# kngwyu/rogue-gym

Measured on AMD Instinct MI355X. Metric: env-steps/sec (whole node) at 65 536 envs, 32x16 mini-dungeon, higher is better.
Workload: dtype u8/u16 integer state, f32 observation; 1 GPU; config-mini.json 32x16, 65536 envs per GPU (65536 total), gray-image obs [N,1,16,32] f32, max_steps 1000, auto-reset; envs_per_gpu=65536, parallelism=env-sharded x1, no data-path collective

## Files before the change

### rogue-gym_amd/csrc/rg_api.cpp

```cpp
#include <hip/hip_runtime.h>
#include <dlfcn.h>

#include <cstdio>
#include <cstdlib>
#include <cstring>
#include <mutex>
#include <random>
#include <string>
#include <vector>

#include "../../include/rogue_gym_hip.h"
#include "rg_state.h"
#include "rg_state_io.h"

extern "C" {
typedef struct ncclComm *ncclComm_t;
typedef struct { char internal[128]; } ncclUniqueId;
typedef int ncclResult_t;
typedef int ncclDataType_t;
}
static const ncclResult_t ncclSuccess = 0;
static const ncclDataType_t ncclUint8 = 1;

extern "C" {
void rgk_build(const RgState *S, const RgConfig *c, hipStream_t st);
int rgk_step(const RgState *S, const RgState *SP_dev, const RgConfig *c, const uint8_t *keys, int use_spares, int parity, hipStream_t st, hipEvent_t ev0, hipEvent_t ev1);
void rgk_probe_clock(unsigned long long *out, int spin, hipStream_t st);
void rgk_regen(const RgState *SP, const RgConfig *c, int bulk, int spares, const uint32_t *mark, uint32_t target, uint32_t *err_any, hipStream_t st, hipEvent_t ev0, hipEvent_t ev1);
void rgk_regen_gate(const uint32_t *mark, uint32_t target, uint32_t *err_any, hipStream_t st);
void rgk_export(const RgState *S, uint32_t *err_any, void *o_screen, void *o_hist, void *o_status, void *o_flags, uint32_t *o_err, hipStream_t st);
int rgk_regen_lanes_supported(const RgConfig *c, int maze_cap);
int rgk_step_bound_capable(const RgConfig *c);
int rgk_regen_lanes(const RgState *SP, const RgConfig *c, uint32_t *q, int32_t *list, int bulk, int waves, int slots, hipStream_t st, hipEvent_t ev0, hipEvent_t ev1);
void rgk_debug_descend(const RgState *S, const RgConfig *c, hipStream_t st);
void rgk_render(const RgState *S, const RgConfig *c, hipStream_t st);
void rgk_encode(const uint8_t *screen, const uint8_t *hist, const int32_t *status, uint32_t *flags, uint32_t *err_any, int n, int hw, size_t rs, size_t rst,
                int symbols, int planes_sym, uint32_t sflag, int with_hist, int kind, float *out, const int32_t *ext, hipStream_t st);
void rgk_pack(const RgState *S, int with_hist, uint8_t *out, hipStream_t st);
void rgk_scatter_rows(const void *src, void *dst, const int32_t *ext, int n, int row_bytes, hipStream_t st);
void rgk_gather_keys(const uint8_t *keys, const int32_t *ext, uint8_t *dst, int n, hipStream_t st);
int rgk_obs(const RgState *S, const RgConfig *c, uint32_t sflag, int with_hist, int kind, float *out, uint32_t *err_any, int planes_sym, int bound, hipStream_t st, hipEvent_t ev0, hipEvent_t ev1);
int rgk_redraw(const RgState *S, const RgConfig *c, hipStream_t st);
int rgk_obs_typed(const RgState *S, const RgConfig *c, int kind, int dtype, uint32_t sflag, int with_hist, int planes_sym, void *out, uint32_t *err_any, hipStream_t st, hipEvent_t ev0,
                  hipEvent_t ev1);
int rgk_obs_crop(const RgState *S, const RgConfig *c, int kind, int ry, int rx, uint32_t sflag, int with_hist, int planes_sym, float *out, int32_t *centers,
                 uint32_t *err_any, hipStream_t st);
void rgk_state_save(const RgState *S, const RgIoLayout *L, const uint64_t *desc, const uint32_t *guard, const int32_t *ids, int k, uint8_t *out, hipStream_t st);
void rgk_state_load(const RgState *S, const RgIoLayout *L, const uint64_t *desc, const uint32_t *guard, const int32_t *ids, int k, const uint8_t *recs, uint32_t rec_bytes, uint8_t *ok,
                    uint8_t *mark, hipStream_t st);
}

#define RG_TIMED_KERNELS 5
struct rg_handle {
    RgParsed parsed;
    RgConfig cfg;
    RgState S;
    RgState SP;
    bool spares = false;
    uint32_t *lane_q = nullptr; int32_t *lane_list = nullptr;
    hipStream_t side3 = nullptr;
    hipStream_t side2 = nullptr;
    int lane_flip = 0;
    uint64_t lane_last = 0;
    uint8_t *pin_keys = nullptr;
    uint32_t *pin_err = nullptr;
    bool lane_regen = false;
    uint64_t step_count = 0;
    hipStream_t side = nullptr;
    int regen_idle_after = -1;
    int regen_bulk = 0;
    int device = 0;
    hipStream_t stream = nullptr;
    std::vector<void *> allocs;
    uint32_t *d_err = nullptr;
    uint8_t *d_keys = nullptr;
    bool render_pending = false;
    float *bound_out = nullptr; int bound_kind = 0; bool bound_valid = false;
    int32_t *obs_list_mem = nullptr; uint32_t *obs_cnt_mem = nullptr; float *gray_lut_mem = nullptr;
    int bound_steps = 0;
    int stair_gen = 0;
    float *obs_scratch = nullptr;
    size_t obs_scratch_cap = 0;
    std::vector<uint64_t> seed_lo, seed_hi;
    std::vector<uint8_t> reseed;
    std::vector<uint64_t> range_lo, range_span;
    unsigned long long *d_probe = nullptr;
    std::vector<rg_handle *> sub;
    std::vector<int> g_of, l_of;
    int32_t *d_ext = nullptr;
    std::vector<int32_t> ext;
    uint8_t *d_keys_sub = nullptr;
    int planes_sym = 0;
    bool screens_stale = true;
    bool mixed = false;
    std::vector<size_t> ragged_off;
    size_t stat_rows = 0;
    RgState *d_SP = nullptr;
    ncclComm_t comm = nullptr;
    int comm_rank = 0, comm_world = 1;
    std::string err;
    bool timing = false;
    std::vector<hipEvent_t> ev[RG_TIMED_KERNELS];
    size_t ev_used[RG_TIMED_KERNELS] = {0, 0, 0, 0, 0};
    uint64_t timing_seq[RG_TIMED_KERNELS] = {0, 0, 0, 0, 0};
    uint64_t timing_stride = 1;
    uint64_t state_fp = 0;
    uint64_t *io_desc = nullptr;
    uint32_t *io_guard = nullptr;
    uint32_t io_words = 0;
    int32_t *io_ids = nullptr; size_t io_ids_cap = 0;
    uint8_t *io_ok = nullptr; size_t io_ok_cap = 0;
    uint8_t *io_mark = nullptr;
};

#define RG_TIMING_MAX 4096
struct TimedLaunch {
    rg_handle *h; int k; bool on, ext_;
    TimedLaunch(rg_handle *h_, int k_, bool ext = false) : h(h_), k(k_), on(false), ext_(ext) {
        if (h->timing && (h->timing_seq[k]++ % h->timing_stride) == h->timing_stride / 2 && h->ev_used[k] + 2 <= h->ev[k].size()) {
            on = true;
            if (!ext_) (void)hipEventRecord(h->ev[k][h->ev_used[k]], h->stream);
        }
    }
    hipEvent_t start_ev() const { return on && ext_ ? h->ev[k][h->ev_used[k]] : nullptr; }
    hipEvent_t stop_ev() const { return on && ext_ ? h->ev[k][h->ev_used[k] + 1] : nullptr; }
    void cancel() { on = false; }
    void stop() { if (on) { if (!ext_) (void)hipEventRecord(h->ev[k][h->ev_used[k] + 1], h->stream); h->ev_used[k] += 2; on = false; } }
    ~TimedLaunch() { stop(); }
};

static thread_local std::string g_create_err;

#ifdef RG_DEV_KNOBS
#define RG_DEV_ENV(name) getenv(name)
#else
#define RG_DEV_ENV(name) ((const char *)nullptr)
#endif

#define HIPCHK(h, call)                                                                                  \
    do {                                                                                                 \
        hipError_t e_ = (call);                                                                          \
        if (e_ != hipSuccess) {                                                                          \
            (h)->err = std::string(#call) + ": " + hipGetErrorString(e_);                                \
            return 1;                                                                                    \
        }                                                                                                \
    } while (0)

template <typename T>
static bool dev_alloc(rg_handle *h, T **p, size_t count) {
    void *q = nullptr;
    size_t bytes = count * sizeof(T);
    if (bytes == 0) bytes = 16;
    if (hipMalloc(&q, bytes) != hipSuccess) { h->err = "hipMalloc failed (" + std::to_string(bytes) + " bytes)"; return false; }
    if (hipMemset(q, 0, bytes) != hipSuccess) { h->err = "hipMemset failed"; return false; }
    h->allocs.push_back(q);
    *p = (T *)q;
    return true;
}

static void free_all(rg_handle *h) {
    for (void *p : h->allocs) (void)hipFree(p);
    h->allocs.clear();
}

static int flush_render(rg_handle *h) {
    if (h->render_pending) {
        { TimedLaunch t(h, 1); rgk_render(&h->S, &h->cfg, h->stream); }
        HIPCHK(h, hipGetLastError());
        h->render_pending = false;
        h->bound_valid = false;
    }
    return 0;
}

static int upload_seeds(rg_handle *h, size_t n) {
    HIPCHK(h, hipMemcpyAsync(h->S.seed_lo, h->seed_lo.data(), n * 8, hipMemcpyHostToDevice, h->stream));
    HIPCHK(h, hipMemcpyAsync(h->S.seed_hi, h->seed_hi.data(), n * 8, hipMemcpyHostToDevice, h->stream));
    HIPCHK(h, hipMemcpyAsync(h->S.reseed, h->reseed.data(), n, hipMemcpyHostToDevice, h->stream));
    return 0;
}

extern "C" {

const char *rg_last_error(const rg_t *h) { return h ? h->err.c_str() : g_create_err.c_str(); }

#ifndef RG_BUILD_ID
#define RG_BUILD_ID "unstamped"
#endif
const char *rg_build_id(void) { static const char id[] = "RGBUILDID:" RG_BUILD_ID; return id + 10; }

static void destroy_handle(rg_handle *h);
struct EnvSeed { bool has_seed, has_range; uint64_t lo, hi; unsigned __int128 r0, r1; };

static int create_homog(const RgParsed &parsed, const EnvSeed *seeds, int n_env, uint64_t max_steps, int device, int auto_reset, rg_handle **out) {
    *out = nullptr;
    rg_handle *h = new rg_handle();
    std::random_device rd;
    std::mt19937_64 gen(((uint64_t)rd() << 32) ^ rd());
    h->seed_lo.resize(n_env); h->seed_hi.resize(n_env); h->reseed.resize(n_env);
    h->parsed = parsed;
    for (int i = 0; i < n_env; i++) {
        const EnvSeed &p = seeds[i];
        if (p.has_seed) { h->seed_lo[i] = p.lo; h->seed_hi[i] = p.hi; h->reseed[i] = 0; }
        else { h->seed_lo[i] = gen(); h->seed_hi[i] = gen(); h->reseed[i] = 1; }
        if (p.has_range) {
            if (!(p.r1 > p.r0)) {
                if (!p.has_seed) { g_create_err = "Invalid Setting: seed_range must satisfy start < end"; delete h; return 1; }
                continue;
            }
            if (h->range_lo.empty()) { h->range_lo.assign(2 * (size_t)n_env, 0); h->range_span.assign(2 * (size_t)n_env, 0); }
            const unsigned __int128 span = p.r1 - p.r0;
            h->range_lo[i] = (uint64_t)p.r0; h->range_lo[n_env + i] = (uint64_t)(p.r0 >> 64);
            h->range_span[i] = (uint64_t)span; h->range_span[n_env + i] = (uint64_t)(span >> 64);
            if (!p.has_seed) h->reseed[i] = 2;
        }
    }
    h->cfg = h->parsed.cfg;
    {
        RgParsed q = h->parsed;
        q.has_seed_range = false;
        const std::string js = rg_dump_config_json(q, 0, 0, false);
        uint64_t f = 0xcbf29ce484222325ull;
        for (unsigned char ch : js) { f ^= ch; f *= 0x100000001b3ull; }
        h->state_fp = f;
    }
    h->planes_sym = h->cfg.symbols;
    h->cfg.max_steps = max_steps > 0xfffffff0ull ? 0xfffffff0u : (uint32_t)max_steps;
    h->cfg.auto_reset = auto_reset ? 1 : 0;
    h->device = device;
    int ndev = 0;
    if (hipGetDeviceCount(&ndev) != hipSuccess || ndev <= 0) {
        g_create_err = "no HIP device available (librogue_gym_hip has no CPU fallback)"; delete h; return 1;
    }
    if (device < 0 || device >= ndev || hipSetDevice(device) != hipSuccess) { g_create_err = "invalid HIP device " + std::to_string(device); delete h; return 1; }

    RgState &S = h->S;
    memset(&S, 0, sizeof S);
    const size_t n = (size_t)n_env, hw = (size_t)h->cfg.width * h->cfg.height;
    S.n = n_env; S.hw = (int)hw; S.n_keys = n_env;
    const int maze_cap = ((h->cfg.width / h->cfg.room_num_x + 1) / 2) * ((h->cfg.height / h->cfg.room_num_y + 1) / 2) + 1;
    S.maze_cap = maze_cap;
    const size_t nr = (size_t)h->cfg.room_num_x * h->cfg.room_num_y, ne = 2 * nr;
    h->stat_rows = 2048 + (n + 15) / 16;
    bool ok = dev_alloc(h, &S.cell, n * hw) && dev_alloc(h, &S.screen, n * hw) && dev_alloc(h, &S.hist, n * hw) &&
              dev_alloc(h, &S.p_pos, n) && dev_alloc(h, &S.p_hp, n) && dev_alloc(h, &S.p_hpmax, n) && dev_alloc(h, &S.p_lvl, n) &&
              dev_alloc(h, &S.p_exp, n) && dev_alloc(h, &S.food, n) && dev_alloc(h, &S.quiet, n) && dev_alloc(h, &S.pack_gold, n) &&
              dev_alloc(h, &S.dlevel, n) && dev_alloc(h, &S.steps, n) && dev_alloc(h, &S.flags, n) && dev_alloc(h, &S.reward, n) && dev_alloc(h, &S.done, n) &&
              dev_alloc(h, &S.rng, 12 * n) && dev_alloc(h, &S.seed_lo, n) && dev_alloc(h, &S.seed_hi, n) && dev_alloc(h, &S.reseed, n) &&
              dev_alloc(h, &S.room_rect, nr * n) && dev_alloc(h, &S.room_meta, nr * n) &&
              dev_alloc(h, &S.mon_w0, nr * n) && dev_alloc(h, &S.mon_hp, nr * n) && dev_alloc(h, &S.mon_exp, nr * n) &&
              dev_alloc(h, &S.mon_cnt, n) && dev_alloc(h, &S.gold_pos, nr * n) && dev_alloc(h, &S.gold_amt, nr * n) &&
              dev_alloc(h, &S.edge_a, ne * n) && dev_alloc(h, &S.edge_b, ne * n) &&
              dev_alloc(h, &S.maze_stack, (size_t)maze_cap * n) && dev_alloc(h, &S.build_ctr, n) && dev_alloc(h, &S.stats, RG_STAT_COLS * h->stat_rows) && dev_alloc(h, &S.stair_list, 2 * n) && dev_alloc(h, &S.stair_cnt, 8) && dev_alloc(h, &S.stair_mark, 2 * n) &&
              dev_alloc(h, &S.dc_map, h->cfg.n_enemies > 0 ? n * RG_DIST_SLOTS * hw : 16) && dev_alloc(h, &S.dc_key, RG_DIST_SLOTS * n) &&
              dev_alloc(h, &S.dc_head, n) && dev_alloc(h, &S.dc_len, n) && dev_alloc(h, &S.dc_part, n) && dev_alloc(h, &S.dc_own, n) && dev_alloc(h, &S.status, n * 10) &&
              dev_alloc(h, &h->d_err, 4) && dev_alloc(h, &h->d_keys, n);
    if (ok && nr <= RG_OBS_MAX_ROOMS) ok = dev_alloc(h, &S.obs_rec, n * (size_t)RG_OBS_REC_WORDS(nr));
    if (ok && nr <= RG_OVL_MAX && getenv("ROGUE_GYM_HIP_NO_MIRROR_UPDATE") == nullptr)
        ok = dev_alloc(h, &S.ovl, (nr + 1) * n) && hipMemset(S.ovl, 0xff, (nr + 1) * n * 2) == hipSuccess;
    h->spares = auto_reset != 0 && getenv("ROGUE_GYM_HIP_NO_SPARES") == nullptr;
    h->lane_regen = h->spares && getenv("ROGUE_GYM_HIP_WAVE_REGEN") == nullptr && rgk_regen_lanes_supported(&h->cfg, maze_cap) > 0;
    const char *slots_env = getenv("ROGUE_GYM_HIP_SP_SLOTS");
    S.sp_slots = h->lane_regen ? (slots_env ? atoi(slots_env) : 4) : 1;
    if (S.sp_slots < 1 || S.sp_slots > 8) S.sp_slots = 4;
    const size_t ns = n * (size_t)S.sp_slots;
    ok = ok && dev_alloc(h, &S.sp_ready, ns) && dev_alloc(h, &h->d_probe, 4) && dev_alloc(h, &S.launch_mark, 4);
    if (ok && h->cfg.n_enemies > 0 && RG_PARTIAL_MAPS(h->cfg.width, h->cfg.height, (int)nr))
        ok = dev_alloc(h, &S.dc_walk, n * RG_DIST_SLOTS * h->cfg.height * RG_WALK_WORDS(h->cfg.width));
    S.full_bfs = getenv("ROGUE_GYM_HIP_FULL_BFS") != nullptr;
    S.keep_spares = getenv("ROGUE_GYM_HIP_KEEP_SPARES") != nullptr;
    S.err_any = h->d_err;
    if (ok && !h->range_lo.empty()) {
        ok = dev_alloc(h, &S.range_lo, 2 * n) && dev_alloc(h, &S.range_span, 2 * n) &&
             hipMemcpy(S.range_lo, h->range_lo.data(), 2 * n * 8, hipMemcpyHostToDevice) == hipSuccess &&
             hipMemcpy(S.range_span, h->range_span.data(), 2 * n * 8, hipMemcpyHostToDevice) == hipSuccess;
        if (!ok && h->err.empty()) h->err = "hipMemcpy failed";
    }
    if (ok && !h->parsed.init_draws.empty()) {
        uint32_t *d = nullptr;
        ok = dev_alloc(h, &d, h->parsed.init_draws.size()) &&
             hipMemcpy(d, h->parsed.init_draws.data(), h->parsed.init_draws.size() * 4, hipMemcpyHostToDevice) == hipSuccess;
        if (!ok && h->err.empty()) h->err = "hipMemcpy failed";
        S.init_draws = d;
    }
    if (ok && h->spares && nr <= 64 && getenv("ROGUE_GYM_HIP_NO_NEXT_LEVELS") == nullptr) {
        RgNext nx;
        memset(&nx, 0, sizeof nx);
        RgNext *d_nx = nullptr;
        ok = dev_alloc(h, &nx.cell, n * hw) && dev_alloc(h, &nx.room_rect, nr * n) && dev_alloc(h, &nx.room_meta, nr * n) &&
             dev_alloc(h, &nx.gold_pos, nr * n) && dev_alloc(h, &nx.gold_amt, nr * n) && dev_alloc(h, &nx.level, n) &&
             dev_alloc(h, &S.nx_rng, 12 * n) && dev_alloc(h, &S.nx_state, n) && dev_alloc(h, &d_nx, 1);
        ok = ok && hipMemcpy(d_nx, &nx, sizeof nx, hipMemcpyHostToDevice) == hipSuccess;
        S.nx = d_nx;
    }
    h->SP = S;
    if (ok && h->spares) {
        RgState &P = h->SP;
        ok = dev_alloc(h, &P.cell, ns * hw) && dev_alloc(h, &P.p_pos, ns) && dev_alloc(h, &P.p_hp, ns) && dev_alloc(h, &P.p_hpmax, ns) && dev_alloc(h, &P.p_lvl, ns) &&
             dev_alloc(h, &P.p_exp, ns) && dev_alloc(h, &P.food, ns) && dev_alloc(h, &P.quiet, ns) && dev_alloc(h, &P.pack_gold, ns) && dev_alloc(h, &P.dlevel, ns) &&
             dev_alloc(h, &P.rng, 12 * ns) && dev_alloc(h, &P.room_rect, nr * ns) && dev_alloc(h, &P.room_meta, nr * ns) &&
             dev_alloc(h, &P.mon_w0, nr * ns) && dev_alloc(h, &P.mon_hp, nr * ns) && dev_alloc(h, &P.mon_exp, nr * ns) &&
             dev_alloc(h, &P.mon_cnt, ns) && dev_alloc(h, &P.gold_pos, nr * ns) && dev_alloc(h, &P.gold_amt, nr * ns) &&
             dev_alloc(h, &P.edge_a, ne * n) && dev_alloc(h, &P.edge_b, ne * n) && dev_alloc(h, &P.maze_stack, (size_t)maze_cap * n) &&
             dev_alloc(h, &P.on_stairs, ns);
        P.prof = nullptr;
        int lo = 0, hi = 0;
        if (ok && (hipDeviceGetStreamPriorityRange(&lo, &hi) != hipSuccess || hipStreamCreateWithPriority(&h->side, hipStreamNonBlocking, RG_DEV_ENV("ROGUE_GYM_HIP_SIDE_HIPRIO") ? hi : lo) != hipSuccess)) {
            h->err = "failed to create the background generation stream"; ok = false;
        }
        static const bool lanes_low = RG_DEV_ENV("ROGUE_GYM_HIP_LANES_LOWPRIO") != nullptr;
        if (ok && (hipStreamCreateWithPriority(&h->side2, hipStreamNonBlocking, lanes_low ? lo : (lo + hi) / 2) != hipSuccess || hipStreamCreateWithPriority(&h->side3, hipStreamNonBlocking, lanes_low ? lo : (lo + hi) / 2) != hipSuccess)) { h->err = "failed to create the background generation stream"; ok = false; }
    }
    ok = ok && dev_alloc(h, &h->d_SP, 1) && hipMemcpy(h->d_SP, &h->SP, sizeof(RgState), hipMemcpyHostToDevice) == hipSuccess;
    if (!ok) { g_create_err = h->err.empty() ? "device allocation failed" : h->err; destroy_handle(h); return 1; }
    if (hipMemset(S.screen, ' ', n * hw) != hipSuccess) { g_create_err = "hipMemset failed"; destroy_handle(h); return 1; }
    if (upload_seeds(h, n)) { g_create_err = h->err; destroy_handle(h); return 1; }
    h->S.stair_gen = h->stair_gen++;
    rgk_build(&h->S, &h->cfg, h->stream);
    hipError_t e = hipGetLastError();
    if (e == hipSuccess) e = hipStreamSynchronize(h->stream);
    if (e != hipSuccess) { g_create_err = std::string("k_build: ") + hipGetErrorString(e); destroy_handle(h); return 1; }
    h->render_pending = true;
    if (h->spares) {
        if (h->lane_regen && !(dev_alloc(h, &h->lane_q, 8) && dev_alloc(h, &h->lane_list, 2 * ns))) { g_create_err = h->err; destroy_handle(h); return 1; }
        if (h->lane_regen) (void)rgk_regen_lanes(&h->SP, &h->cfg, h->lane_q, h->lane_list, 1, 0, h->S.sp_slots, h->side2, nullptr, nullptr);
        else rgk_regen(&h->SP, &h->cfg, 1, 1, nullptr, 0, h->d_err, h->side, nullptr, nullptr);
        e = hipGetLastError();
        if (e == hipSuccess && !RG_DEV_ENV("ROGUE_GYM_HIP_ASYNC_FIRST_SPARES")) { e = hipStreamSynchronize(h->side); if (e == hipSuccess) e = hipStreamSynchronize(h->side2); if (e == hipSuccess) e = hipStreamSynchronize(h->side3); }
        if (e != hipSuccess) { g_create_err = std::string("k_regen: ") + hipGetErrorString(e); destroy_handle(h); return 1; }
        h->regen_bulk = 1;
        bool all_fixed = true;
        for (uint8_t m : h->reseed) all_fixed = all_fixed && m == 0;
        if (h->S.keep_spares && all_fixed && !h->S.nx_state) h->regen_idle_after = 1;
    }
    *out = h;
    return 0;
}

#define SUBCHK(h, sh, call) do { if (call) { (h)->err = (sh)->err; return 1; } } while (0)

static void destroy_handle(rg_handle *h);
static int comm_release(rg_handle *h, bool teardown);

static int assemble_small(rg_handle *h) {
    for (rg_handle *sh : h->sub) {
        const int m = sh->S.n;
        rgk_scatter_rows(sh->S.status, h->S.status, sh->d_ext, m, 40, h->stream);
        rgk_scatter_rows(sh->S.reward, h->S.reward, sh->d_ext, m, 4, h->stream);
        rgk_scatter_rows(sh->S.done, h->S.done, sh->d_ext, m, 1, h->stream);
        rgk_scatter_rows(sh->S.flags, h->S.flags, sh->d_ext, m, 4, h->stream);
    }
    HIPCHK(h, hipGetLastError());
    return 0;
}
static int assemble_screens(rg_handle *h) {
    if (!h->screens_stale) return 0;
    for (rg_handle *sh : h->sub) {
        SUBCHK(h, sh, flush_render(sh));
        const int m = sh->S.n;
        if (!h->mixed) {
            rgk_scatter_rows(sh->S.screen, h->S.screen, sh->d_ext, m, h->S.hw, h->stream);
            rgk_scatter_rows(sh->S.hist, h->S.hist, sh->d_ext, m, h->S.hw, h->stream);
        }
        rgk_scatter_rows(sh->S.flags, h->S.flags, sh->d_ext, m, 4, h->stream);
    }
    HIPCHK(h, hipGetLastError());
    h->screens_stale = false;
    return 0;
}

int rg_create(const char *const *cfg_json, int n_env, uint64_t max_steps, int device, int auto_reset, rg_t **out) {
    if (!out || n_env <= 0) { g_create_err = "rg_create: invalid arguments"; return 1; }
    *out = nullptr;
    std::vector<RgParsed> reps;
    std::vector<EnvSeed> seeds(n_env);
    std::vector<int> g_of(n_env), l_of(n_env);
    std::vector<std::vector<int>> members;
    {
        const char *prev = nullptr; int prev_g = -1;
        RgParsed p;
        for (int i = 0; i < n_env; i++) {
            const char *js = cfg_json ? cfg_json[i] : nullptr;
            const bool same_text = i > 0 && ((js == nullptr && prev == nullptr) || (js && prev && strcmp(js, prev) == 0));
            int g = prev_g;
            if (!same_text) {
                std::string e = rg_parse_config(js, &p);
                if (!e.empty()) { g_create_err = "Failed to parse config: " + e; return 1; }
                g = -1;
                for (size_t k = 0; k < reps.size(); k++) if (rg_config_equal(reps[k], p)) { g = (int)k; break; }
                if (g < 0) { g = (int)reps.size(); reps.push_back(p); members.emplace_back(); }
                prev = js; prev_g = g;
            }
            seeds[i] = EnvSeed{p.has_seed, p.has_seed_range, p.seed_lo, p.seed_hi, p.seed_range[0], p.seed_range[1]};
            g_of[i] = g; l_of[i] = (int)members[g].size(); members[g].push_back(i);
        }
    }
    if (reps.size() == 1) return create_homog(reps[0], seeds.data(), n_env, max_steps, device, auto_reset, out);
    bool mixed = false;
    for (size_t k = 1; k < reps.size(); k++) mixed = mixed || reps[k].cfg.width != reps[0].cfg.width || reps[k].cfg.height != reps[0].cfg.height;
    rg_handle *h = new rg_handle();
    h->device = device;
    h->mixed = mixed;
    h->g_of = g_of; h->l_of = l_of;
    for (size_t k = 0; k < reps.size(); k++) {
        std::vector<EnvSeed> gs(members[k].size());
        for (size_t j = 0; j < members[k].size(); j++) gs[j] = seeds[members[k][j]];
        rg_handle *sh = nullptr;
        if (create_homog(reps[k], gs.data(), (int)gs.size(), max_steps, device, auto_reset, &sh)) { destroy_handle(h); return 1; }
        h->sub.push_back(sh);
        sh->ext.assign(members[k].begin(), members[k].end());
        bool ok = dev_alloc(sh, &sh->d_ext, gs.size()) && dev_alloc(sh, &sh->d_keys_sub, gs.size()) &&
                  hipMemcpy(sh->d_ext, sh->ext.data(), gs.size() * 4, hipMemcpyHostToDevice) == hipSuccess;
        if (!ok) { g_create_err = "device allocation failed"; destroy_handle(h); return 1; }
        sh->S.ext = sh->d_ext;
    }
    if (mixed) {
        h->ragged_off.assign((size_t)n_env + 1, 0);
        for (int i = 0; i < n_env; i++) h->ragged_off[i + 1] = h->ragged_off[i] + (size_t)reps[g_of[i]].cfg.width * reps[g_of[i]].cfg.height;
    }
    rg_handle *first = h->sub[g_of[0]];
    h->parsed = first->parsed; h->cfg = first->cfg;
    h->planes_sym = first->cfg.symbols;
    for (rg_handle *sh : h->sub) sh->planes_sym = h->planes_sym;
    RgState &S = h->S;
    memset(&S, 0, sizeof S);
    const size_t n = (size_t)n_env, hw = (size_t)h->cfg.width * h->cfg.height;
    S.n = n_env; S.hw = (int)hw; S.n_keys = n_env;
    bool ok = (mixed || (dev_alloc(h, &S.screen, n * hw) && dev_alloc(h, &S.hist, n * hw))) && dev_alloc(h, &S.status, n * 10) && dev_alloc(h, &S.flags, n) &&
              dev_alloc(h, &S.reward, n) && dev_alloc(h, &S.done, n) && dev_alloc(h, &h->d_err, 4) && dev_alloc(h, &h->d_probe, 4);
    if (!ok) { g_create_err = h->err; destroy_handle(h); return 1; }
    S.err_any = h->d_err;
    if (assemble_small(h) || hipStreamSynchronize(h->stream) != hipSuccess) { g_create_err = h->err.empty() ? "assemble failed" : h->err; destroy_handle(h); return 1; }
    *out = h;
    return 0;
}

static void destroy_handle(rg_handle *h) {
    if (!h) return;
    (void)hipSetDevice(h->device);
    for (rg_handle *sh : h->sub) destroy_handle(sh);
    h->sub.clear();
    (void)hipStreamSynchronize(h->stream);
    if (h->comm) (void)comm_release(h, true);
    if (h->side) { (void)hipStreamSynchronize(h->side); (void)hipStreamDestroy(h->side); }
    if (h->side2) { (void)hipStreamSynchronize(h->side2); (void)hipStreamDestroy(h->side2); }
    if (h->side3) { (void)hipStreamSynchronize(h->side3); (void)hipStreamDestroy(h->side3); }
    for (int k = 0; k < RG_TIMED_KERNELS; k++) for (auto &e : h->ev[k]) (void)hipEventDestroy(e);
    if (h->obs_scratch) (void)hipFree(h->obs_scratch);
    if (h->pin_keys) (void)hipHostFree(h->pin_keys);
    if (h->pin_err) (void)hipHostFree(h->pin_err);
    free_all(h);
    delete h;
}

void rg_destroy(rg_t *h) { destroy_handle(h); }

int rg_dims(const rg_t *h, int *height, int *width, int *symbols, int *n_env) {
    if (height) *height = h->cfg.height;
    if (width) *width = h->cfg.width;
    if (symbols) *symbols = h->planes_sym;
    if (n_env) *n_env = h->S.n;
    return 0;
}

int rg_env_dims(const rg_t *h, int32_t *heights, int32_t *widths) {
    for (int i = 0; i < h->S.n; i++) {
        const RgConfig &c = h->sub.empty() ? h->cfg : h->sub[h->g_of[i]]->cfg;
        if (heights) heights[i] = c.height;
        if (widths) widths[i] = c.width;
    }
    return 0;
}
static bool refuse_mixed(rg_handle *h, const char *what) {
    if (!h->mixed) return false;
    h->err = std::string(what) + ": the envs of this batch differ in width / height, so there is no [n_env][H][W] tensor (per-env sizes: rg_env_dims; "
             "ragged host copies: rg_fetch_states; or one handle per size)";
    return true;
}

int rg_env_symbols(const rg_t *h, int32_t *out_host) {
    if (h->sub.empty()) { for (int i = 0; i < h->S.n; i++) out_host[i] = h->cfg.symbols; return 0; }
    for (int i = 0; i < h->S.n; i++) out_host[i] = h->sub[h->g_of[i]]->cfg.symbols;
    return 0;
}

int rg_set_stream(rg_t *h, void *hip_stream) {
    for (rg_handle *sh : h->sub) SUBCHK(h, sh, rg_set_stream(sh, hip_stream));
    HIPCHK(h, hipStreamSynchronize(h->stream));
    if (h->side) { HIPCHK(h, hipStreamSynchronize(h->side)); HIPCHK(h, hipStreamSynchronize(h->side2)); HIPCHK(h, hipStreamSynchronize(h->side3)); }
    h->stream = (hipStream_t)hip_stream;
    return 0;
}

int rg_seed(rg_t *h, const uint64_t *seed_lo, const uint64_t *seed_hi, int n) {
    if (n > h->S.n) n = h->S.n;
    if (n <= 0) return 0;
    HIPCHK(h, hipSetDevice(h->device));
    if (!h->sub.empty()) {
        for (rg_handle *sh : h->sub) {
            std::vector<uint64_t> lo, hi;
            for (int l = 0; l < sh->S.n && sh->ext[l] < n; l++) { lo.push_back(seed_lo[sh->ext[l]]); hi.push_back(seed_hi ? seed_hi[sh->ext[l]] : 0); }
            if (!lo.empty()) SUBCHK(h, sh, rg_seed(sh, lo.data(), hi.data(), (int)lo.size()));
        }
        return 0;
    }
    for (int i = 0; i < n; i++) { h->seed_lo[i] = seed_lo[i]; h->seed_hi[i] = seed_hi ? seed_hi[i] : 0; h->reseed[i] = 0; }
    if (h->spares) {
        HIPCHK(h, hipStreamSynchronize(h->side));
        HIPCHK(h, hipStreamSynchronize(h->side2));
        HIPCHK(h, hipStreamSynchronize(h->side3));
        for (int sl = 0; sl < h->S.sp_slots; sl++) HIPCHK(h, hipMemsetAsync(h->S.sp_ready + (size_t)sl * h->S.n, 0, (size_t)n * 4, h->stream));
        if (h->regen_idle_after >= 0) h->regen_idle_after = 2;
        h->regen_bulk = 2;
    }
    return upload_seeds(h, (size_t)n);
}

int rg_reset(rg_t *h) {
    HIPCHK(h, hipSetDevice(h->device));
    if (!h->sub.empty()) {
        for (rg_handle *sh : h->sub) SUBCHK(h, sh, rg_reset(sh));
        h->screens_stale = true;
        return assemble_small(h);
    }
    h->S.stair_gen = h->stair_gen++;
    { TimedLaunch t(h, 3); rgk_build(&h->S, &h->cfg, h->stream); }
    HIPCHK(h, hipGetLastError());
    h->render_pending = true;
    h->bound_valid = false;
    return 0;
}

static int obs_common(rg_t *h, uint32_t status_flag, int with_hist, int kind, float *out_dev);
int rg_step(rg_t *h, const uint8_t *keys, int keys_on_device) { return rg_step_prefix(h, keys, h->S.n, keys_on_device); }
int rg_step_obs_gray(rg_t *h, const uint8_t *keys, int keys_on_device, uint32_t status_flag, int with_hist, float *out_dev) {
    return rg_step_prefix(h, keys, h->S.n, keys_on_device) ? 1 : obs_common(h, status_flag, with_hist, 0, out_dev);
}

int rg_step_prefix(rg_t *h, const uint8_t *keys, int n_keys, int keys_on_device) {
    HIPCHK(h, hipSetDevice(h->device));
    if (n_keys < 0) { h->err = "rg_step_prefix: negative key count"; return 1; }
    if (n_keys > h->S.n) n_keys = h->S.n;
    if (!h->sub.empty()) {
        const uint8_t *dkeys = keys;
        if (!keys_on_device) {
            if (!h->d_keys && !dev_alloc(h, &h->d_keys, (size_t)h->S.n)) return 1;
            HIPCHK(h, hipMemcpyAsync(h->d_keys, keys, (size_t)n_keys, hipMemcpyHostToDevice, h->stream));
            dkeys = h->d_keys;
        }
        for (rg_handle *sh : h->sub) {
            int m = 0;
            while (m < sh->S.n && sh->ext[m] < n_keys) m++;
            if (m) rgk_gather_keys(dkeys, sh->d_ext, sh->d_keys_sub, m, h->stream);
            SUBCHK(h, sh, rg_step_prefix(sh, sh->d_keys_sub, m, 1));
        }
        HIPCHK(h, hipGetLastError());
        h->screens_stale = true;
        return assemble_small(h);
    }
    if (flush_render(h)) return 1;
    const uint8_t *dk = keys;
    if (!keys_on_device) {
        HIPCHK(h, hipMemcpyAsync(h->d_keys, keys, (size_t)n_keys, hipMemcpyHostToDevice, h->stream));
        dk = h->d_keys;
    }
    h->S.n_keys = n_keys;
    static const int regen_every = RG_DEV_ENV("ROGUE_GYM_HIP_REGEN_EVERY") ? atoi(RG_DEV_ENV("ROGUE_GYM_HIP_REGEN_EVERY")) : 1;
    h->step_count++;
    bool regen = h->spares && (regen_every <= 1 || h->step_count % (uint64_t)regen_every == 0);
    if (regen && h->regen_idle_after >= 0) { if (h->regen_idle_after == 0) regen = false; else h->regen_idle_after--; }
    static const bool no_stair_waves = getenv("ROGUE_GYM_HIP_NO_STAIR_WAVES") != nullptr;
    {
        TimedLaunch t(h, 0, true);
        h->S.stair_gen = h->stair_gen++;
        h->S.obs_par = (int32_t)(h->step_count & 1); h->bound_steps++;
        (void)rgk_step(&h->S, h->d_SP, &h->cfg, dk, h->spares ? 1 : 0, no_stair_waves ? -1 : 0, h->stream, t.start_ev(), t.stop_ev());
    }
    HIPCHK(h, hipGetLastError());
    if (regen) {
        TimedLaunch t(h, 4, true);
        if (h->lane_regen) {
            static const int lane_waves = RG_DEV_ENV("ROGUE_GYM_HIP_LANE_WAVES") ? atoi(RG_DEV_ENV("ROGUE_GYM_HIP_LANE_WAVES")) : 256;
            static const int lane_every = RG_DEV_ENV("ROGUE_GYM_HIP_LANE_EVERY") ? atoi(RG_DEV_ENV("ROGUE_GYM_HIP_LANE_EVERY")) : 16;
            static const bool time_lanes = RG_DEV_ENV("ROGUE_GYM_HIP_TIME_LANES") != nullptr;
            const bool lanes_now = h->regen_bulk > 0 || h->step_count - h->lane_last >= (uint64_t)(lane_every > 0 ? lane_every : 1);
            static const int urgent_mode = RG_DEV_ENV("ROGUE_GYM_HIP_URGENT_AT0") ? 3 : 2;
            rgk_regen(&h->SP, &h->cfg, 0, urgent_mode, h->S.launch_mark, (uint32_t)h->S.stair_gen + 1u, h->d_err, h->side, time_lanes ? nullptr : t.start_ev(), time_lanes ? nullptr : t.stop_ev());
            if (time_lanes && !lanes_now) t.cancel();
            if (lanes_now) {
                h->lane_last = h->step_count;
                h->lane_flip ^= 1;
                rgk_regen_gate(h->S.launch_mark, (uint32_t)h->S.stair_gen + 1u, h->d_err, h->lane_flip ? h->side3 : h->side2);
                (void)rgk_regen_lanes(&h->SP, &h->cfg, h->lane_q + 4 * h->lane_flip, h->lane_list + (size_t)h->S.n * h->S.sp_slots * h->lane_flip, h->regen_bulk > 0 ? 1 : 0, lane_waves, h->S.sp_slots,
                                      h->lane_flip ? h->side3 : h->side2, time_lanes ? t.start_ev() : nullptr, time_lanes ? t.stop_ev() : nullptr);
            }
        } else rgk_regen(&h->SP, &h->cfg, h->regen_bulk > 0 ? 1 : 0, 1, h->S.launch_mark, (uint32_t)h->S.stair_gen + 1u, h->d_err, h->side, t.start_ev(), t.stop_ev());
        if (h->regen_bulk > 0) h->regen_bulk--;
    }
    HIPCHK(h, hipGetLastError());
    h->render_pending = true;
    return 0;
}

int rg_sync(rg_t *h) {
    HIPCHK(h, hipSetDevice(h->device));
    if (!h->sub.empty()) {
        int rc = 0;
        for (rg_handle *sh : h->sub)
            if (rg_sync(sh) && !rc) { rc = 1; h->err = sh->err; }
        if (rc) return rc;
    }
    uint32_t err = 0;
    HIPCHK(h, hipMemcpyAsync(&err, h->d_err, 4, hipMemcpyDeviceToHost, h->stream));
    HIPCHK(h, hipStreamSynchronize(h->stream));
    if (h->side) { HIPCHK(h, hipStreamSynchronize(h->side)); HIPCHK(h, hipStreamSynchronize(h->side2)); HIPCHK(h, hipStreamSynchronize(h->side3)); }
    if (err) {
        HIPCHK(h, hipMemsetAsync(h->d_err, 0, 4, h->stream));
        if (err & RG_FLAG_ERR_INTERNAL) h->err = "internal capacity guard of the HIP stepper tripped (please report the config)";
        else if (err & RG_FLAG_ERR_STATE) h->err = "state record refused: it does not fit this env (magic / version / config fingerprint / geometry), the env is unchanged";
        else if (err & RG_FLAG_ERR_KEY) h->err = "Invalid input (key is not in the ai keymap)";
        else if (err & RG_FLAG_ERR_DEAD) h->err = "Ignored input (action while the player is dead)";
        else h->err = "Invalid tile in symbol image (symbol >= symbols - 1)";
        return 1;
    }
    return 0;
}

static int flush_mirrors(rg_handle *h) { return h->sub.empty() ? flush_render(h) : assemble_screens(h); }
int rg_screen(rg_t *h, uint8_t **dev) { if (refuse_mixed(h, "rg_screen")) return 1; HIPCHK(h, hipSetDevice(h->device)); if (flush_mirrors(h)) return 1; *dev = h->S.screen; return 0; }
int rg_hist(rg_t *h, uint8_t **dev) { if (refuse_mixed(h, "rg_hist")) return 1; HIPCHK(h, hipSetDevice(h->device)); if (flush_mirrors(h)) return 1; *dev = h->S.hist; return 0; }
int rg_status(rg_t *h, int32_t **dev) { *dev = h->S.status; return 0; }
int rg_flags(rg_t *h, uint32_t **dev) { HIPCHK(h, hipSetDevice(h->device)); if (flush_mirrors(h)) return 1; *dev = h->S.flags; return 0; }
int rg_reward(rg_t *h, float **dev) { *dev = h->S.reward; return 0; }
int rg_done(rg_t *h, uint8_t **dev) { *dev = h->S.done; return 0; }
int rg_set_stair_reward(rg_t *h, float bonus) {
    if (!(bonus == bonus) || bonus < 0.f) { h->err = "rg_set_stair_reward: the bonus must be a number >= 0"; return 1; }
    h->S.stair_reward = bonus;
    for (rg_handle *sh : h->sub) sh->S.stair_reward = bonus;
    return 0;
}

int rg_obs_channels(const rg_t *h, int symbol, uint32_t status_flag, int with_hist) {
    return (symbol ? h->planes_sym : 1) + __builtin_popcount(status_flag & 0x1ffu) + (with_hist ? 1 : 0);
}

static int obs_common(rg_t *h, uint32_t status_flag, int with_hist, int kind, float *out_dev) {
    if (refuse_mixed(h, kind ? "rg_obs_symbol" : "rg_obs_gray")) return 1;
    HIPCHK(h, hipSetDevice(h->device));
    if (!h->sub.empty()) {
        for (rg_handle *sh : h->sub) {
            if (kind && sh->cfg.symbols > h->planes_sym) {
                h->err = "symbol image: a config of the batch has more symbols (" + std::to_string(sh->cfg.symbols) + ") than env 0's (" + std::to_string(h->planes_sym) +
                         "), which sets the channel count (python/src/lib.rs:281-285)";
                return 1;
            }
            SUBCHK(h, sh, obs_common(sh, status_flag, with_hist, kind, out_dev));
        }
        return 0;
    }
    {
        TimedLaunch t(h, 2, true);
        const bool bound = h->bound_out && out_dev == h->bound_out && kind == h->bound_kind && (status_flag & 0x1ffu) == 0 && !with_hist;
        if (rgk_obs(&h->S, &h->cfg, status_flag & 0x1ffu, with_hist ? 1 : 0, kind, out_dev, h->d_err, h->planes_sym, bound && h->S.obs_list && h->bound_valid && h->bound_steps == 1, h->stream, t.start_ev(), t.stop_ev())) {
            HIPCHK(h, hipGetLastError());
            h->render_pending = false;
            h->bound_valid = bound;
            h->bound_steps = 0;
            return 0;
        }
        t.cancel();
    }
    h->bound_valid = false;
    if (flush_render(h)) return 1;
    {
        TimedLaunch t(h, 2);
        rgk_encode(h->S.screen, h->S.hist, h->S.status, h->S.flags, h->d_err, h->S.n, h->S.hw, (size_t)h->S.hw, 10, h->cfg.symbols, h->planes_sym,
                   status_flag & 0x1ffu, with_hist ? 1 : 0, kind, out_dev, h->S.ext, h->stream);
    }
    HIPCHK(h, hipGetLastError());
    return 0;
}
static uint32_t host_tile_to_sym(uint32_t t) {
    switch (t) {
    case ' ': return 0; case '@': return 1; case '#': return 2; case '.': return 3; case '-': case '|': return 4;
    case '%': return 5; case '+': return 6; case '^': return 7; case '!': return 8; case '?': return 9; case ']': return 10;
    case ')': return 11; case '/': return 12; case '*': return 13; case ':': return 14; case '=': return 15; case ',': return 16;
    default: return (t >= 'A' && t <= 'Z') ? t - 'A' + 17 : 255u;
    }
}
int rg_obs_bind(rg_t *h, int kind, uint32_t status_flag, int with_hist, float *out_dev) {
    if (!h->sub.empty()) { h->err = "rg_obs_bind: not for a handle with config groups"; return 1; }
    if (out_dev && ((status_flag & 0x1ffu) || with_hist || (kind != 0 && kind != 1))) { h->err = "rg_obs_bind: gray or symbol image without status planes and history plane"; return 1; }
    HIPCHK(h, hipSetDevice(h->device));
    const bool capable = rgk_step_bound_capable(&h->cfg) != 0;
    if (!capable) { h->S.obs_list = nullptr; h->S.obs_cnt = nullptr; h->S.bound_gray = nullptr; h->bound_out = out_dev; h->bound_kind = kind; h->bound_valid = false; h->bound_steps = 0; return 0; }
    if (out_dev && !h->obs_list_mem) {
        if (!dev_alloc(h, &h->obs_list_mem, 2 * (size_t)h->S.n) || !dev_alloc(h, &h->obs_cnt_mem, 2)) return 1;
    }
    if (out_dev) HIPCHK(h, hipMemsetAsync(h->obs_cnt_mem, 0, 8, h->stream));
    h->S.obs_list = out_dev ? h->obs_list_mem : nullptr; h->S.obs_cnt = out_dev ? h->obs_cnt_mem : nullptr;
    h->S.bound_gray = (out_dev && kind == 0) ? out_dev : nullptr;
    if (h->S.bound_gray && !h->gray_lut_mem) {
        float lut[128];
        for (uint32_t g = 0; g < 128; g++) lut[g] = (float)(uint8_t)host_tile_to_sym(g) / (float)(uint8_t)h->cfg.symbols;
        if (!dev_alloc(h, &h->gray_lut_mem, 128)) return 1;
        HIPCHK(h, hipMemcpy(h->gray_lut_mem, lut, sizeof lut, hipMemcpyHostToDevice));
    }
    h->S.gray_lut = h->gray_lut_mem;
    h->bound_out = out_dev; h->bound_kind = kind; h->bound_valid = false; h->bound_steps = 0;
    return 0;
}
int rg_obs_crop(rg_t *h, int kind, int radius_y, int radius_x, uint32_t status_flag, int with_hist, float *out_dev, int32_t *centers_dev) {
    if (kind != 0 && kind != 1) { h->err = "rg_obs_crop: kind must be 0 (gray) or 1 (symbol), got " + std::to_string(kind); return 1; }
    if (radius_y < 0 || radius_y > RG_MAX_H - 1 || radius_x < 0 || radius_x > RG_MAX_W - 1) {
        h->err = "rg_obs_crop: radii must satisfy 0 <= radius_y <= " + std::to_string(RG_MAX_H - 1) + " and 0 <= radius_x <= " + std::to_string(RG_MAX_W - 1) +
                 ", got (" + std::to_string(radius_y) + ", " + std::to_string(radius_x) + ")";
        return 1;
    }
    if (!out_dev || ((uintptr_t)out_dev & 15)) { h->err = "rg_obs_crop: out_dev must be a non-null, 16-byte aligned device pointer"; return 1; }
    HIPCHK(h, hipSetDevice(h->device));
    if (!h->sub.empty()) {
        for (rg_handle *sh : h->sub)
            if (kind && sh->cfg.symbols > h->planes_sym) {
                h->err = "symbol image: a config of the batch has more symbols (" + std::to_string(sh->cfg.symbols) + ") than env 0's (" + std::to_string(h->planes_sym) +
                         "), which sets the channel count (python/src/lib.rs:281-285)";
                return 1;
            }
        for (rg_handle *sh : h->sub) SUBCHK(h, sh, rg_obs_crop(sh, kind, radius_y, radius_x, status_flag, with_hist, out_dev, centers_dev));
        return 0;
    }
    if (flush_render(h)) return 1;
    if (!rgk_obs_crop(&h->S, &h->cfg, kind, radius_y, radius_x, status_flag & 0x1ffu, with_hist ? 1 : 0, h->planes_sym, out_dev, centers_dev, h->d_err, h->stream)) {
        h->err = "rg_obs_crop: window too large";
        return 1;
    }
    HIPCHK(h, hipGetLastError());
    return 0;
}
int rg_obs_dtype_bytes(int dtype) { return dtype == RG_OBS_F32 ? 4 : (dtype == RG_OBS_F16 || dtype == RG_OBS_BF16) ? 2 : dtype == RG_OBS_U8 ? 1 : -1; }
static int typed_check(rg_t *h, const char *what, int kind, int dtype, uint32_t status_flag, const void *out_dev) {
    const std::string w = std::string(what) + ": ";
    if (kind < 0 || kind > 2) { h->err = w + "kind must be 0 (gray), 1 (symbol) or 2 (symbol ids), got " + std::to_string(kind); return 1; }
    if (rg_obs_dtype_bytes(dtype) < 0) { h->err = w + "dtype must be RG_OBS_F32 (0), RG_OBS_F16 (1), RG_OBS_BF16 (2) or RG_OBS_U8 (3), got " + std::to_string(dtype); return 1; }
    if (kind == 2 && dtype != RG_OBS_U8) { h->err = w + "kind 2 (symbol ids) takes dtype RG_OBS_U8 only, got dtype " + std::to_string(dtype); return 1; }
    if (kind != 2 && dtype == RG_OBS_U8) { h->err = w + "dtype RG_OBS_U8 is for kind 2 (symbol ids) only, got kind " + std::to_string(kind); return 1; }
    if (kind == 2 && (status_flag & 0x1ffu)) { h->err = w + "status_flag must be 0 for kind 2 (status values do not fit a byte; read the status mirror)"; return 1; }
    if (!out_dev || ((uintptr_t)out_dev & 15)) { h->err = w + "out_dev must be a non-null, 16-byte aligned device pointer"; return 1; }
    if (dtype == RG_OBS_F32) return 0;
    if (!h->sub.empty() || h->mixed) { h->err = w + "not for a handle with config groups or mixed sizes"; return 1; }
    const int cells = dtype == RG_OBS_U8 ? 16 : 8;
    if (h->S.hw % cells) {
        h->err = w + "H*W must be a multiple of " + std::to_string(cells) + " for this dtype (a lane writes whole 16-byte pieces of a plane), got " + std::to_string(h->cfg.height) +
                 " x " + std::to_string(h->cfg.width);
        return 1;
    }
    return 0;
}
static int obs_typed_checked(rg_t *h, int kind, int dtype, uint32_t status_flag, int with_hist, void *out_dev) {
    if (dtype == RG_OBS_F32) return obs_common(h, status_flag, with_hist, kind, static_cast<float *>(out_dev));
    HIPCHK(h, hipSetDevice(h->device));
    if (h->render_pending) {
        bool swept;
        { TimedLaunch t(h, 1); swept = rgk_redraw(&h->S, &h->cfg, h->stream) != 0; if (!swept) t.cancel(); }
        if (swept) {
            HIPCHK(h, hipGetLastError());
            h->render_pending = false;
            h->bound_valid = false;
        } else if (flush_render(h)) return 1;
    }
    {
        TimedLaunch t(h, 2, true);
        if (!rgk_obs_typed(&h->S, &h->cfg, kind, dtype, status_flag & 0x1ffu, with_hist ? 1 : 0, h->planes_sym, out_dev, h->d_err, h->stream, t.start_ev(), t.stop_ev())) {
            t.cancel();
            h->err = "rg_obs_typed: grid not supported";
            return 1;
        }
    }
    HIPCHK(h, hipGetLastError());
    return 0;
}
int rg_obs_typed(rg_t *h, int kind, int dtype, uint32_t status_flag, int with_hist, void *out_dev) {
    return typed_check(h, "rg_obs_typed", kind, dtype, status_flag, out_dev) ? 1 : obs_typed_checked(h, kind, dtype, status_flag, with_hist, out_dev);
}
int rg_step_obs_typed(rg_t *h, const uint8_t *keys, int keys_on_device, int kind, int dtype, uint32_t status_flag, int with_hist, void *out_dev) {
    if (typed_check(h, "rg_step_obs_typed", kind, dtype, status_flag, out_dev)) return 1;
    return rg_step_prefix(h, keys, h->S.n, keys_on_device) ? 1 : obs_typed_checked(h, kind, dtype, status_flag, with_hist, out_dev);
}
int rg_obs_gray(rg_t *h, uint32_t status_flag, int with_hist, float *out_dev) { return obs_common(h, status_flag, with_hist, 0, out_dev); }
int rg_obs_symbol(rg_t *h, uint32_t status_flag, int with_hist, float *out_dev) { return obs_common(h, status_flag, with_hist, 1, out_dev); }

int rg_fetch_states(rg_t *h, uint8_t *screen, uint8_t *hist, int32_t *status, uint32_t *flags) {
    HIPCHK(h, hipSetDevice(h->device));
    if (flush_mirrors(h)) return 1;
    size_t n = (size_t)h->S.n, hw = (size_t)h->S.hw;
    if (h->mixed) {
        std::vector<uint8_t> tmp;
        for (rg_handle *sh : h->sub) {
            const size_t m = (size_t)sh->S.n, ghw = (size_t)sh->S.hw;
            for (int which = 0; which < 2; which++) {
                uint8_t *dst = which ? hist : screen;
                if (!dst) continue;
                tmp.resize(m * ghw);
                HIPCHK(h, hipMemcpyAsync(tmp.data(), which ? sh->S.hist : sh->S.screen, m * ghw, hipMemcpyDeviceToHost, h->stream));
                HIPCHK(h, hipStreamSynchronize(h->stream));
                for (size_t l = 0; l < m; l++) memcpy(dst + h->ragged_off[sh->ext[l]], tmp.data() + l * ghw, ghw);
            }
        }
        screen = hist = nullptr;
    }
    if (screen) HIPCHK(h, hipMemcpyAsync(screen, h->S.screen, n * hw, hipMemcpyDeviceToHost, h->stream));
    if (hist) HIPCHK(h, hipMemcpyAsync(hist, h->S.hist, n * hw, hipMemcpyDeviceToHost, h->stream));
    if (status) HIPCHK(h, hipMemcpyAsync(status, h->S.status, n * 40, hipMemcpyDeviceToHost, h->stream));
    if (flags) HIPCHK(h, hipMemcpyAsync(flags, h->S.flags, n * 4, hipMemcpyDeviceToHost, h->stream));
    HIPCHK(h, hipStreamSynchronize(h->stream));
    return 0;
}

int rg_step_fetch(rg_t *h, const uint8_t *keys_host, int n_keys, uint8_t *screen, uint8_t *hist, int32_t *status, uint32_t *flags) {
    if (refuse_mixed(h, "rg_step_fetch")) return 1;
    if (!h->sub.empty()) { h->err = "rg_step_fetch: not for a handle with config groups (rg_step_prefix + rg_fetch_states)"; return 1; }
    if (!status || !flags || (screen == nullptr) != (hist == nullptr)) { h->err = "rg_step_fetch: status and flags are required, screen and hist come together"; return 1; }
    if (h->S.hw & 3) { h->err = "rg_step_fetch needs H*W divisible by 4"; return 1; }
    HIPCHK(h, hipSetDevice(h->device));
    if (n_keys < 0) { h->err = "rg_step_fetch: negative key count"; return 1; }
    if (n_keys > h->S.n) n_keys = h->S.n;
    if (!h->pin_keys) HIPCHK(h, hipHostMalloc((void **)&h->pin_keys, (size_t)h->S.n + 16, hipHostMallocDefault));
    if (!h->pin_err) HIPCHK(h, hipHostMalloc((void **)&h->pin_err, 16, hipHostMallocDefault));
    memcpy(h->pin_keys, keys_host, (size_t)n_keys);
    if (rg_step_prefix(h, h->pin_keys, n_keys, 1)) return 1;
    if (flush_render(h)) return 1;
    rgk_export(&h->S, h->d_err, screen, hist, status, flags, h->pin_err, h->stream);
    HIPCHK(h, hipGetLastError());
    HIPCHK(h, hipStreamSynchronize(h->stream));
    const uint32_t err = h->pin_err[0];
    if (err) {
        if (err & RG_FLAG_ERR_INTERNAL) h->err = "internal capacity guard of the HIP stepper tripped (please report the config)";
        else if (err & RG_FLAG_ERR_STATE) h->err = "state record refused: it does not fit this env (magic / version / config fingerprint / geometry), the env is unchanged";
        else if (err & RG_FLAG_ERR_KEY) h->err = "Invalid input (key is not in the ai keymap)";
        else if (err & RG_FLAG_ERR_DEAD) h->err = "Ignored input (action while the player is dead)";
        else h->err = "Invalid tile in symbol image (symbol >= symbols - 1)";
        return 1;
    }
    return 0;
}

int rg_dev_alloc(int device, size_t bytes, void **out) {
    if (hipSetDevice(device) != hipSuccess || hipMalloc(out, bytes ? bytes : 16) != hipSuccess) { g_create_err = "hipMalloc failed (" + std::to_string(bytes) + " bytes)"; return 1; }
    return 0;
}
void rg_dev_free(int device, void *p) { if (p && hipSetDevice(device) == hipSuccess) (void)hipFree(p); }
int rg_snapshot_take(rg_t *h, void *dev) {
    if (refuse_mixed(h, "rg_snapshot_take")) return 1;
    HIPCHK(h, hipSetDevice(h->device));
    if (flush_mirrors(h)) return 1;
    const size_t bytes = (size_t)h->S.n * (size_t)h->S.hw;
    HIPCHK(h, hipMemcpyAsync(dev, h->S.screen, bytes, hipMemcpyDeviceToDevice, h->stream));
    HIPCHK(h, hipMemcpyAsync(static_cast<uint8_t *>(dev) + bytes, h->S.hist, bytes, hipMemcpyDeviceToDevice, h->stream));
    return 0;
}
int rg_dev_read_rows(rg_t *h, const void *dev_src, size_t src_pitch, void *host_dst, size_t row_bytes, int rows) {
    HIPCHK(h, hipSetDevice(h->device));
// ... 664 lines not shown
```

### rogue-gym_amd/csrc/rg_kernels.hip

```cpp


#include "rg_device.h"


#include "rg_gen.h"


#ifdef RG_FINE_PROF
#define PFM(id) pf.mark(id)
#else
#define PFM(id) ((void)0)
#endif
struct Prof {
    unsigned long long *p; unsigned long long t, t0, r0; int k;
    __device__ __forceinline__ void start(unsigned long long *pp) { p = pp ? pp + (size_t)blockIdx.x * 64 : nullptr; k = 0; if (p) { r0 = __builtin_amdgcn_s_memrealtime(); t = t0 = __builtin_amdgcn_s_memtime(); } }
    __device__ __forceinline__ void rec(int phase, unsigned long long v) {
        if (p && threadIdx.x == 0 && k < 61) p[1 + k++] = ((unsigned long long)phase << 48) | (v & 0xffffffffffffull);
    }
    __device__ __forceinline__ void mark(int phase) {
        if (!p) return;
        unsigned long long now = __builtin_amdgcn_s_memtime();
        rec(phase, now - t);
        t = now;
    }
    __device__ __forceinline__ void finish() {
        if (p && threadIdx.x == 0) { p[0] = (unsigned long long)k; p[63] = __builtin_amdgcn_s_memtime() - t0; p[62] = (r0 << 32) | (__builtin_amdgcn_s_memrealtime() & 0xffffffffull); }
    }
};

typedef __attribute__((address_space(3))) uint16_t lds_u16;
typedef __attribute__((address_space(3))) uint32_t lds_u32;
struct Env {
    int e;
    int n;
    uint16_t *cell;
    uint16_t *gcell;
    Rng rd, ri, re;
    int px, py;
    int hp, hpmax, plvl;
    uint32_t exp, food, quiet, gold, dlevel;
    uint32_t mon_alive, mon_active;
    lds_u16 *lc;
    uint16_t *stk_lds;
    lds_u32 *mc;
    uint32_t err;
    uint32_t on_stairs;
#ifdef RG_FINE_PROF
    Prof *pfp;
#endif
    uint32_t g_rect, g_meta;
    uint32_t g_ea, g_eb;
};
template <int GM> __device__ __forceinline__ uint32_t gen_rect(const RgState &S, const Env &E, int i) { return GM < 2 ? lane_get(E.g_rect, i) : uni(S.room_rect[i]); }
template <int GM> __device__ __forceinline__ uint32_t gen_meta(const RgState &S, const Env &E, int i) { return GM < 2 ? lane_get(E.g_meta, i) : uni((uint32_t)S.room_meta[i]); }
template <int GM> __device__ __forceinline__ void gen_set_rect(const RgState &S, Env &E, int i, uint32_t v) {
    if (GM < 2) E.g_rect = (int)threadIdx.x == i ? v : E.g_rect; else S.room_rect[i] = v;
}
template <int GM> __device__ __forceinline__ void gen_set_meta(const RgState &S, Env &E, int i, uint32_t v) {
    if (GM < 2) E.g_meta = (int)threadIdx.x == i ? v : E.g_meta; else S.room_meta[i] = (uint8_t)v;
}

template <bool MC> __device__ __forceinline__ uint32_t mon_rd(const RgState &S, const Env &E, int s) { return MC ? E.mc[s * WAVE] : uni(S.mon_w0[s * E.n + E.e]); }
template <bool MC> __device__ __forceinline__ void mon_wr(const RgState &S, const Env &E, int s, uint32_t w) {
    S.mon_w0[s * E.n + E.e] = w;
    if (MC) E.mc[s * WAVE] = w;
}

__device__ __forceinline__ int mon_find(const RgState &S, const Env &E, int nrooms, uint32_t pos) {
    if (E.mon_alive == 0) return -1;
    int found = -1;
    for (int s = 0; s < nrooms; s++) {
        uint32_t w = mon_rd<true>(S, E, s);
        uint32_t fl = w >> 24;
        if ((fl & MF_ALIVE) && (w & 0xffff) == pos) found = s;
    }
    return found;
}

template <bool MC>
__device__ __forceinline__ void activate_room(const RgState &S, const RgConfig &c, Env &E, int rid) {
    if (E.mon_alive == E.mon_active) return;
    int nrooms = c.room_num_x * c.room_num_y;
    for (int s = 0; s < nrooms; s++) {
        uint32_t w = mon_rd<MC>(S, E, s);
        uint32_t fl = w >> 24;
        if (!(fl & MF_ALIVE) || (fl & MF_ACTIVE)) continue;
        if (!(c.mon[(w >> 16) & 0xff].attr & EA_MEAN)) continue;
        if (room_id_of(c, POS_X(w), POS_Y(w)) != rid) continue;
        mon_wr<MC>(S, E, s, w | (MF_ACTIVE << 24));
        E.mon_active++;
    }
}

template <int GM>
__device__ __forceinline__ void player_in_init(const RgState &S, const RgConfig &c, Env &E, int x, int y) {
    lds_u16 *cell = E.lc;
    int W = c.width;
    int rid = room_id_of(c, x, y);
    if (rid >= 0) {
        uint32_t meta = gen_meta<GM>(S, E, rid);
        if (!(meta & RM_VISITED)) {
            gen_set_meta<GM>(S, E, rid, meta | RM_VISITED);
            if ((meta & RM_KIND_MASK) == RK_NORMAL && !(meta & RM_DARK)) {
                int x0, y0, x1, y1;
                unpack_rect(gen_rect<GM>(S, E, rid), x0, y0, x1, y1);
                const int rw = x1 - x0, area = rw * (y1 - y0);
                for (int t = threadIdx.x; t < area; t += WAVE) {
                    const int yy = small_div(t, rw), xx = t - yy * rw;
                    cell[(y0 + yy) * W + x0 + xx] |= C_DRAWN | C_VISIBLE;
                }
                __builtin_amdgcn_fence(__ATOMIC_RELEASE, "workgroup");
                __builtin_amdgcn_wave_barrier();
            }
        }
        activate_room<false>(S, c, E, rid);
    }
    cell[y * W + x] |= C_VISITED;
    for (int d = 0; d < 9; d++) {
        int cx = x + dir_dx(d), cy = y + dir_dy(d);
        if (!in_bounds(c, cx, cy)) continue;
        uint32_t v = uni(cell[cy * W + cx]);
        bool diag = d >= 4 && d < 8;
        if (diag && (v & C_SURF_MASK) == S_PASSAGE) continue;
        if (v & C_HIDDEN) continue;
        cell[cy * W + cx] = (uint16_t)(v | C_DRAWN | C_VISIBLE);
    }
}

__device__ __forceinline__ uint64_t rect_ballot(const RgConfig &c, const Env &E, int x0, int y0, int rw, int area, int base, uint32_t bits, uint32_t excl) {
    const int t = base + (int)threadIdx.x;
    bool in = false;
    if (t < area) {
        const int yy = small_div(t, rw), xx = t - yy * rw;
        in = (E.lc[(y0 + yy) * c.width + x0 + xx] & bits) && POS(x0 + xx, y0 + yy) != excl;
    }
    return __ballot(in);
}
__device__ __forceinline__ int nth_set64(uint64_t m, int nth) {
    const int lane = threadIdx.x;
    const bool mine = ((m >> lane) & 1ull) && lanes_below(m) == nth;
    return __ffsll((long long)__ballot(mine)) - 1;
}
__device__ __forceinline__ uint32_t rect_nth(const RgConfig &c, const Env &E, int x0, int y0, int rw, int area, uint32_t bits, uint32_t excl, int nth) {
    for (int base = 0; base < area; base += WAVE) {
        const uint64_t m = rect_ballot(c, E, x0, y0, rw, area, base, bits, excl);
        const int cnt = __popcll(m);
        if (nth < cnt) {
            const int t = base + nth_set64(m, nth);
            const int yy = small_div(t, rw);
            return POS(x0 + t - yy * rw, y0 + yy);
        }
        nth -= cnt;
    }
    return POS(x0, y0);
}
// ... 1901 lines not shown
    const __attribute__((address_space(3))) uint8_t *mt = (const __attribute__((address_space(3))) uint8_t *)(ovl_l - ln + (RG_OVL_MAX + 6) * WAVE);
    uint32_t actp = 0;
    bool far = false;
#pragma nounroll
    for (int s0 = 0; s0 < nrooms; s0++) {
        const uint32_t p = ovl_l[(1 + s0) * WAVE], m = mc[s0 * WAVE];
        const bool alive = (m >> 24) & MF_ALIVE, had = p != OVL_NONE;
        const uint32_t pp = p & 0xff3fu, pn = m & 0xffffu;
        bool show = false;
        if (alive) {
            const int x = POS_X(pn), y = POS_Y(pn), dx = px - x, dy = py - y;
            show = dx * dx + dy * dy <= 2;
            if (!show && rid >= 0 && room_id_of(c, x, y) == rid) {
                if ((r_meta & RM_KIND_MASK) == RK_EMPTY) show = true;
                else {
                    int x0, y0, x1, y1;
                    unpack_rect(r_rect, x0, y0, x1, y1);
                    const bool ina = px >= x0 && px < x1 && py >= y0 && py < y1, inb = x >= x0 && x < x1 && y >= y0 && y < y1;
                    show = ina == inb;
                }
            }
        }
        const bool unknown = had && (p & OVL_UNKNOWN), showed = had && (p & OVL_SHOW);
        const bool same = had && alive && pp == pn && !unknown && !dirty_at(POS_X(pn), POS_Y(pn));
        uint32_t a = 0;
        if (same) { if (showed && !show) a = 1u; else if (!showed && show) a = 2u; }
        else { if (had && (showed || unknown)) a |= 1u; if (show) a |= 2u; }
        a |= show ? 4u : 0u;
        actp |= a << (3 * s0);
        if (((a & 1u) && !in_win(POS_X(pp), POS_Y(pp))) || ((a & 2u) && !in_win(POS_X(pn), POS_Y(pn)))) far = true;
        const uint32_t now = alive ? (pn | (show ? OVL_SHOW : 0u)) : OVL_NONE;
        if (now != p) S.ovl[(size_t)s0 * n + e] = (uint16_t)now;
    }
    const uint32_t pl = ovl_l[(1 + nrooms) * WAVE];
    const uint32_t plp = pl & 0xff3fu;
    const bool pl_moved = pl == OVL_NONE || (pl & OVL_UNKNOWN) || plp != POS(px, py) || dirty_at(px, py);
    if (pl_moved) S.ovl[(size_t)nrooms * n + e] = (uint16_t)POS(px, py);
    if (far || (pl_moved && pl != OVL_NONE && !in_win(POS_X(plp), POS_Y(plp)))) return false;
    for (uint32_t d = ds; d;) {
        const int k = __ffs((int)d) - 1;
        d &= d - 1;
        const int j = k / 5, i = k - j * 5, x = w.ox + i - 2, y = w.oy + j - 2;
        put(y * W + x, base_glyph(c, WV(w, k), y) & 0x7fu);
    }
    if (react & R_HIST_CHANGED) S.hist[(size_t)e * S.hw + py * W + px] = 1;
    if (pl_moved && pl != OVL_NONE) {
        const int x = POS_X(plp), y = POS_Y(plp);
        put(y * W + x, base_glyph(c, WV(w, WIN_K(x - w.ox, y - w.oy)), y) & 0x7fu);
    }
#pragma nounroll
    for (int s0 = 0; s0 < nrooms; s0++)
        if ((actp >> (3 * s0)) & 1u) {
            const uint32_t pp = ovl_l[(1 + s0) * WAVE] & 0xff3fu;
            const int x = POS_X(pp), y = POS_Y(pp);
            put(y * W + x, base_glyph(c, WV(w, WIN_K(x - w.ox, y - w.oy)), y) & 0x7fu);
        }
#pragma nounroll
    for (int s0 = 0; s0 < nrooms; s0++)
        if ((actp >> (3 * s0)) & 2u) {
            const uint32_t m = mc[s0 * WAVE];
            const int x = POS_X(m), y = POS_Y(m);
            const uint32_t under = base_glyph(c, WV(w, WIN_K(x - w.ox, y - w.oy)), y);
            if ((under & 0x80u) && under != (0x80u | '*')) put(y * W + x, mt[(m >> 16) & 0xff]);
        }
    if (pl_moved && (base_glyph(c, WV(w, WIN_K(px - w.ox, py - w.oy)), py) & 0x80u)) put(py * W + px, '@');
    return true;
}

__device__ __forceinline__ void take_spares(const RgState &S, const RgState *__restrict__ SPd, const RgConfig &c, int lane, int e, bool taken, bool &on_stairs) {
    const uint64_t tm = __ballot(taken);
    if (!tm) return;
    const RgState &SP = *SPd;
    const int HW = S.hw, n = S.n, nrooms = c.room_num_x * c.room_num_y;
    const size_t ns = (size_t)n * S.sp_slots;
    int es = e;
    if (taken)
        for (int sl = S.sp_slots - 1; sl >= 0; sl--)
            if (__hip_atomic_load(&S.sp_ready[(size_t)sl * n + e], __ATOMIC_RELAXED, __HIP_MEMORY_SCOPE_AGENT) == 1u) es = sl * n + e;
    __builtin_amdgcn_fence(__ATOMIC_ACQUIRE, "agent");
    if ((HW & 7) == 0) {
        const int q = HW / 8;
        uint64_t mm = tm;
        while (mm) {
            const int s0 = __ffsll((long long)mm) - 1; mm &= mm - 1;
            const int s1 = mm ? __ffsll((long long)mm) - 1 : -1; if (mm) mm &= mm - 1;
            const int s2 = mm ? __ffsll((long long)mm) - 1 : -1; if (mm) mm &= mm - 1;
            const int s3 = mm ? __ffsll((long long)mm) - 1 : -1; if (mm) mm &= mm - 1;
            const int e0 = __shfl(e, s0), e1 = __shfl(e, s1 >= 0 ? s1 : s0), e2 = __shfl(e, s2 >= 0 ? s2 : s0), e3 = __shfl(e, s3 >= 0 ? s3 : s0);
            const int q0 = __shfl(es, s0), q1 = __shfl(es, s1 >= 0 ? s1 : s0), q2 = __shfl(es, s2 >= 0 ? s2 : s0), q3 = __shfl(es, s3 >= 0 ? s3 : s0);
            const uint4 *a0 = reinterpret_cast<const uint4 *>(SP.cell + (size_t)q0 * HW), *a1 = reinterpret_cast<const uint4 *>(SP.cell + (size_t)q1 * HW);
            const uint4 *a2 = reinterpret_cast<const uint4 *>(SP.cell + (size_t)q2 * HW), *a3 = reinterpret_cast<const uint4 *>(SP.cell + (size_t)q3 * HW);
            uint4 *d0 = reinterpret_cast<uint4 *>(S.cell + (size_t)e0 * HW), *d1 = reinterpret_cast<uint4 *>(S.cell + (size_t)e1 * HW);
            uint4 *d2 = reinterpret_cast<uint4 *>(S.cell + (size_t)e2 * HW), *d3 = reinterpret_cast<uint4 *>(S.cell + (size_t)e3 * HW);
            for (int i = lane; i < q; i += WAVE) {
                const uint4 v0 = a0[i];
                uint4 v1 = v0, v2 = v0, v3 = v0;
                if (s1 >= 0) v1 = a1[i];
                if (s2 >= 0) v2 = a2[i];
                if (s3 >= 0) v3 = a3[i];
                d0[i] = v0;
                if (s1 >= 0) d1[i] = v1;
                if (s2 >= 0) d2[i] = v2;
                if (s3 >= 0) d3[i] = v3;
            }
        }
    } else {
        uint64_t mm = tm;
        while (mm) {
            const int src = __ffsll((long long)mm) - 1; mm &= mm - 1;
            const int env_s = __shfl(e, src);
            const uint16_t *sp = SP.cell + (size_t)__shfl(es, src) * HW;
            uint16_t *dp = S.cell + (size_t)env_s * HW;
            for (int i = lane; i < HW; i += WAVE) dp[i] = sp[i];
        }
    }
    if (taken) {
        uint32_t r[12];
#pragma unroll
        for (int k = 0; k < 12; k++) r[k] = SP.rng[k * ns + es];
        const uint16_t pp = SP.p_pos[es];
        const int32_t hp = SP.p_hp[es], hpm = SP.p_hpmax[es], lv = SP.p_lvl[es];
        const uint32_t ex = SP.p_exp[es], fd = SP.food[es], qu = SP.quiet[es], pg = SP.pack_gold[es], dl = SP.dlevel[es], mc = SP.mon_cnt[es];
        on_stairs = SP.on_stairs[es] != 0;
#pragma unroll
        for (int k = 0; k < 12; k++) S.rng[k * n + e] = r[k];
        S.p_pos[e] = pp; S.p_hp[e] = hp; S.p_hpmax[e] = hpm; S.p_lvl[e] = lv;
        if (S.obs_rec) S.obs_rec[(size_t)e * RG_OBS_REC_WORDS(nrooms) + nrooms] = pp;
        if (S.ovl) S.ovl[(size_t)nrooms * n + e] = (uint16_t)(pp | 0x40u);
        S.p_exp[e] = ex; S.food[e] = fd; S.quiet[e] = qu; S.pack_gold[e] = pg; S.dlevel[e] = dl; S.mon_cnt[e] = mc;
        for (int s0 = 0; s0 < nrooms; s0 += 4) {
            uint32_t rr[4], mw[4], me[4], gp[4], ga[4]; int32_t mh[4]; uint8_t rm[4];
#pragma unroll
            for (int k = 0; k < 4; k++) {
                const size_t g = (size_t)(s0 + k < nrooms ? s0 + k : s0) * ns + es;
                rr[k] = SP.room_rect[g]; rm[k] = SP.room_meta[g]; mw[k] = SP.mon_w0[g]; mh[k] = SP.mon_hp[g]; me[k] = SP.mon_exp[g]; gp[k] = SP.gold_pos[g]; ga[k] = SP.gold_amt[g];
            }
#pragma unroll
            for (int k = 0; k < 4; k++)
                if (s0 + k < nrooms) {
                    const size_t g = (size_t)(s0 + k) * n + e;
                    S.room_rect[g] = rr[k]; S.room_meta[g] = rm[k]; S.mon_w0[g] = mw[k]; S.mon_hp[g] = mh[k]; S.mon_exp[g] = me[k]; S.gold_pos[g] = gp[k]; S.gold_amt[g] = ga[k];
                    if (S.obs_rec) {
                        uint32_t *rec = S.obs_rec + (size_t)e * RG_OBS_REC_WORDS(nrooms);
                        rec[s0 + k] = mw[k]; rec[nrooms + 1 + s0 + k] = rr[k]; reinterpret_cast<uint8_t *>(&rec[2 * nrooms + 1])[s0 + k] = rm[k];
                    }
                    if (S.ovl) S.ovl[(size_t)(s0 + k) * n + e] = (uint16_t)(((mw[k] >> 24) & MF_ALIVE) ? ((mw[k] & 0xffffu) | 0x40u) : 0xffffu);
                }
        }
    }
    __syncthreads();
    if (taken && !(S.keep_spares && S.reseed[e] == 0)) __hip_atomic_store(&S.sp_ready[es], 0u, __ATOMIC_RELAXED, __HIP_MEMORY_SCOPE_AGENT);
}

template <int BW, int GM, bool BND = false>
__device__ __forceinline__ void step_wave(const RgState &S, const RgState *__restrict__ SPd, const RgConfig &c, const uint8_t *__restrict__ keys, int use_spares, int stage_off,
                                          const int e, const bool valid_in, const int stair_role) {
    uint16_t *lds_grid = reinterpret_cast<uint16_t *>(g_smem + stage_off);
    const int lane = threadIdx.x;
    Prof pf; pf.start(S.prof);
    Env E;
    E.err = 0; E.on_stairs = 0;
    uint32_t react = 0, err = 0, old_flags = 0, steps = 0, flags = 0;
    int act = ACT_NOOP, dir = 0;
    int gold0 = 0;
    bool live = false;
    bool ui_dead = false, terminal = false;
    bool inc_done = false;
    bool taken = false;
    uint32_t n_bfs = 0, n_inline = 0, n_taken = 0, n_cont = 0;
    uint32_t key = 0, nxs = RG_NX_NONE;
    bool listed = false;
    const int nrooms_k = c.room_num_x * c.room_num_y;
    E.mc = (lds_u32 *)(g_smem + STEP_LDS_MC) + lane;
    const uint32_t glyph_r = S.ovl ? c.mon[lane & 31].tile : 0u;
    if (valid_in) {
        listed = S.stair_mark[(size_t)(S.stair_gen & 1) * S.n + e] != 0;
        uint32_t nxk = 0;
        if (S.nx_state) {
            nxs = __hip_atomic_load(&S.nx_state[e], __ATOMIC_RELAXED, __HIP_MEMORY_SCOPE_AGENT);
            nxk = __hip_atomic_load(&S.nx_rng[(size_t)3 * S.n + e], __ATOMIC_RELAXED, __HIP_MEMORY_SCOPE_AGENT);
        }
        old_flags = S.flags[e];
        steps = S.steps[e];
        gold0 = S.status[(size_t)e * 10 + 1];
        if (e < S.n_keys) key = keys[e];
        load_env(S, E, e);
        if (nxs == RG_NX_READY && nxk != E.rd.w) nxs = RG_NX_STALE;
        for (int s0 = 0; s0 < nrooms_k; s0 += 4) {
            uint32_t m4[4];
#pragma unroll
            for (int k = 0; k < 4; k++) m4[k] = S.mon_w0[(size_t)(s0 + k < nrooms_k ? s0 + k : s0) * S.n + e];
#pragma unroll
            for (int k = 0; k < 4; k++)
                if (s0 + k < nrooms_k) E.mc[(s0 + k) * WAVE] = m4[k];
        }
    }
    const bool to_stair_wave = listed && key == '>';
    const bool valid = valid_in && (stair_role == 0 || (stair_role == 1) == to_stair_wave);
    const bool has_key = valid && e < S.n_keys;
    if (valid) {
        if (has_key && !(steps > c.max_steps)) {
            act = decode_key(key, dir);
            if (act == ACT_INVALID) err = RG_FLAG_ERR_KEY;
            else {
                klog_push(S, e, key);
                if (old_flags & RG_FLAG_DEAD) err = RG_FLAG_ERR_DEAD;
                else live = true;
            }
        }
    }
    pf.mark(0);
    bool need_gen = false, descends = false;
    Win w;
    w.v = (lds_u16 *)(g_smem + STEP_LDS_WIN) + lane;
    lds_u32 *ovl_l = (lds_u32 *)(g_smem + STEP_LDS_OVL) + lane;
    ovl_l[0] = 0;
    if (BND && S.bound_gray) {
        typedef const __attribute__((address_space(1))) void *gptr;
        typedef __attribute__((address_space(3))) void *lptr;
        __builtin_amdgcn_global_load_lds((gptr)(S.gray_lut + lane), (lptr)(g_smem + STEP_LDS_LUT), 4, 0, 0);
        __builtin_amdgcn_global_load_lds((gptr)(S.gray_lut + 64 + lane), (lptr)(g_smem + STEP_LDS_LUT + 256), 4, 0, 0);
    }
    if (S.ovl && lane < RG_MAX_ENEMY_KINDS + 6)
        ((__attribute__((address_space(3))) uint8_t *)(g_smem + STEP_LDS_OVL + (RG_OVL_MAX + 6) * WAVE * 4))[lane] = (uint8_t)glyph_r;
    if (S.ovl) {
        typedef const __attribute__((address_space(1))) void *gptr;
        typedef __attribute__((address_space(3))) void *lptr;
        lds_u32 *base = (lds_u32 *)(g_smem + STEP_LDS_OVL);
        const size_t es = valid_in ? (size_t)e : 0;
#pragma unroll
        for (int s0 = 0; s0 <= RG_OVL_MAX; s0++)
            __builtin_amdgcn_global_load_lds((gptr)(S.ovl + (size_t)(s0 <= nrooms_k ? s0 : 0) * S.n + es), (lptr)(base + (1 + s0) * WAVE), 2, 0, 0);
    }
    w.inb = 0;
    if (S.ovl) {
        typedef const __attribute__((address_space(1))) void *gptr;
        typedef __attribute__((address_space(3))) void *lptr;
        lds_u32 *base = (lds_u32 *)(g_smem + STEP_LDS_OVL);
        const size_t es = valid_in ? (size_t)e : 0;
        const bool mv = live && (act == ACT_MOVE || act == ACT_MOVE_UNTIL);
        const int ra = room_id_of(c, E.px, E.py), rb = mv ? room_id_of(c, E.px + dir_dx(dir), E.py + dir_dy(dir)) : ra;
        const size_t aa = (size_t)(ra >= 0 ? ra : 0) * S.n + es, ab = (size_t)(rb >= 0 ? rb : 0) * S.n + es;
        __builtin_amdgcn_global_load_lds((gptr)(S.room_rect + aa), (lptr)(base + (RG_OVL_MAX + 2) * WAVE), 4, 0, 0);
        __builtin_amdgcn_global_load_lds((gptr)(S.room_meta + aa), (lptr)(base + (RG_OVL_MAX + 3) * WAVE), 1, 0, 0);
        __builtin_amdgcn_global_load_lds((gptr)(S.room_rect + ab), (lptr)(base + (RG_OVL_MAX + 4) * WAVE), 4, 0, 0);
        __builtin_amdgcn_global_load_lds((gptr)(S.room_meta + ab), (lptr)(base + (RG_OVL_MAX + 5) * WAVE), 1, 0, 0);
    }
    if (live && stair_role != 1) win_load(c, E.cell, w, E.px, E.py);
    else { w.inb = 0; w.dirty = 0; w.ox = w.oy = 0; }
    pf.mark(26);
    if (live && act == ACT_DOWNSTAIR) {
        if (stair_role == 1 || (WV(w, WIN_K(0, 0)) & C_SURF_MASK) == S_STAIR) {
            need_gen = descends = true;
            react |= R_REDRAW | R_STATUS | R_HIST_STALE;
        } else react |= MSG_NO_DOWNSTAIR;
    }
    if (S.nx_state) {
        if (descends && nxs == RG_NX_READY) {
            const uint32_t *q = S.nx_rng + e;
            const size_t n = (size_t)S.n;
            const uint32_t k0 = q[0], k1 = q[n], k2 = q[2 * n], kl = S.nx->level[e];
            if (k0 == E.rd.x && k1 == E.rd.y && k2 == E.rd.z && kl == E.dlevel) nxs = RG_NX_HIT;
        }
        if (__any(nxs == RG_NX_HIT)) __builtin_amdgcn_fence(__ATOMIC_ACQUIRE, "agent");
    }
    {
        uint64_t lag = __ballot(descends && ((old_flags & RG_FLAG_HIST_LAG) || ((old_flags & RG_FLAG_REDRAW) && (old_flags & RG_FLAG_HIST_STALE))));
        while (lag) {
            const int src = __ffsll((long long)lag) - 1;
            lag &= lag - 1;
            const int env_s = __shfl(e, src);
            const uint16_t *cp = S.cell + (size_t)env_s * S.hw;
            uint8_t *hp = S.hist + (size_t)env_s * S.hw;
            for (int i = lane; i < S.hw; i += WAVE) hp[i] = (cp[i] & C_VISITED) ? 1 : 0;
        }
    }
#pragma nounroll
    for (int pass = 0; pass < 2; ++pass) {
        pf.mark(1);
        if (pass == 1 && use_spares) {
            if (need_gen) {
                bool rdy = false;
                for (int sl = 0; sl < S.sp_slots; sl++) rdy = rdy || __hip_atomic_load(&S.sp_ready[(size_t)sl * S.n + e], __ATOMIC_RELAXED, __HIP_MEMORY_SCOPE_AGENT) == 1u;
                if (rdy) { taken = true; need_gen = false; n_taken++; }
            }
        }
        const bool regenerated = descends && pass == 0;
        if constexpr (BW == 1 || BW == 2) { if (pass == 0 && S.dc_walk) snapshot_walk_service(S, c, lane, e, descends); }
        const uint64_t nx_now = pass == 0 ? __ballot(need_gen && nxs == RG_NX_HIT) : 0ull;
        if (need_gen) n_inline++;
        gen_service<GM>(S, c, E, lane, e, need_gen, pass == 1, lds_grid, pf, nx_now);
        (void)regenerated;
        pf.mark(2);
        need_gen = false;
        if (pass == 1) break;

        bool running = live && act != ACT_NOOP;
        int iter = 0;
        while (__any(running)) {
            bool do_turn = false, need_bfs = false, opened = false, own_req = false;
            int map_slot = -1;
            FillReq fr; fr.leave = fr.enter = 0;
            if (running) {
                switch (act) {
                case ACT_DOWNSTAIR:
                    do_turn = true; running = false;
                    break;
                case ACT_MOVE:
                case ACT_MOVE_UNTIL: {
                    bool done = move_player(S, c, E, w, dir, react, fr, (S.ovl && iter == 0) ? (const lds_u32 *)ovl_l : nullptr);
                    if (act == ACT_MOVE) { do_turn = true; running = false; break; }
                    uint32_t v = win_get(w, WIN_K(E.px - w.ox, E.py - w.oy));
                    uint32_t tile = (v & C_VISIBLE) ? glyph_of(v) : ' ';
                    if (done || (tile != '.' && tile != '#')) running = false;
                    else do_turn = true;
                    break;
                }
                case ACT_SEARCH:
                    opened = do_search(c, E, w, react);
                    do_turn = true; running = false;
                    break;
                }
            }
            if constexpr (BW == 1 || BW == 2) { if (__any(opened) && S.dc_walk) snapshot_walk_service(S, c, lane, e, opened); }
            pf.mark(28);
            if (do_turn) turn_passed(c, E, react);
            pf.mark(29);
            bool need_map = false;
            if (do_turn && E.mon_active > 0) need_map = monsters_prepass(S, c, E);
            pf.mark(30);
            if (need_map) {
                uint32_t part_bits = 0, own_bits = 0;
                if constexpr (BW == 1 || BW == 2) { part_bits = S.dc_part[e]; own_bits = S.dc_own[e]; }
                need_bfs = !dist_cache_lookup(S, E, POS(E.px, E.py), map_slot);
                if constexpr (BW == 1 || BW == 2) {
                    if (!need_bfs && ((part_bits >> map_slot) & 1u) && !dist_map_sufficient(S, c, E, map_slot)) {
                        need_bfs = true;
                        own_req = (own_bits >> map_slot) & 1u;
                        if (own_req) n_cont++;
                    }
                }
            }
            pf.mark(3);
            if (iter == 0) ovl_l[0] = w.dirty | ((fr.leave | fr.enter) ? 0x80000000u : 0u);
            fill_service(S, c, lane, e, fr);
            win_flush(c, E.cell, w);
            pf.mark(27);
#ifdef RG_EXP_NO_BFS
            need_bfs = false;
#endif
            uint64_t m = __ballot(need_bfs);
            if (need_bfs) n_bfs++;
            if (m) {
                unsigned long long tb0 = pf.p ? __builtin_amdgcn_s_memtime() : 0;
                const bool complete = bfs_service<BW>(S, c, reinterpret_cast<uint64_t *>(lds_grid), m, e, E.px, E.py, map_slot, lane, E.mc - lane, __ballot(own_req));
                if constexpr (BW == 1 || BW == 2) {
                    if (need_bfs) {
                        const uint32_t bit = 1u << map_slot;
                        const uint32_t part = S.dc_part[e], own = S.dc_own[e];
                        S.dc_part[e] = (uint16_t)(complete ? part & ~bit : part | bit);
                        S.dc_own[e] = (uint16_t)((own_req && !complete) ? own : own & ~bit);
                    }
                } else (void)complete;
                if (pf.p) { pf.rec(24, __builtin_amdgcn_s_memtime() - tb0); pf.rec(25, (unsigned long long)__popcll(m)); }
            }
            pf.mark(4);
            if (do_turn && E.mon_active > 0) ui_dead = monsters_move(S, c, E, map_slot, react);
            else if (do_turn) ui_dead = false;
            pf.mark(5);
            if (++iter > RG_MAX_W + RG_MAX_H && running) { running = false; E.err |= RG_FLAG_ERR_INTERNAL; }
            if (running) win_load(c, E.cell, w, E.px, E.py);
        }
        if (live) {
            flags = (react & 0x7f00u);
            if (react & R_REDRAW) flags |= RG_FLAG_REDRAW | ((react & R_HIST_STALE) ? RG_FLAG_HIST_STALE : 0);
            else flags |= old_flags & (RG_FLAG_REDRAW | RG_FLAG_HIST_STALE);
            flags |= old_flags & (RG_FLAG_HIST_LAG | RG_FLAG_HIST_DIRTY | (BND ? RG_FLAG_SCR_CHANGED : 0u));
            if ((react & R_HIST_CHANGED) || descends) flags |= RG_FLAG_HIST_DIRTY;
            if (react & R_STATUS) write_status(S, c, E);
            if (ui_dead) flags |= RG_FLAG_DEAD;
            steps += 1;
            terminal = (react & R_GRAVE) || steps >= c.max_steps;
            need_gen = terminal && c.auto_reset;
            if (S.ovl && (react & R_REDRAW) && !descends && !need_gen && act != ACT_MOVE_UNTIL &&
                !(old_flags & (RG_FLAG_REDRAW | RG_FLAG_HIST_STALE | RG_FLAG_HIST_LAG | RG_FLAG_HIST_DIRTY)) && !(ovl_l[0] >> 31)) {
                if (mirror_update<BND>(S, c, E, w, react, room_id_of(c, w.ox, w.oy))) flags = (flags & ~(RG_FLAG_REDRAW | RG_FLAG_HIST_DIRTY)) | ((!BND || S.bound_gray) ? 0u : RG_FLAG_SCR_CHANGED);
                inc_done = true;
            }
        }
    }
    pf.mark(6);
    int et = e;
    asm volatile("" : "+v"(et));
    E.e = et;
    bool pend = false; uint64_t pm = 0; uint32_t lbase = 0;
    if (BND && S.obs_list) {
        const uint32_t fw = (live ? ((terminal && c.auto_reset) ? RG_FLAG_REDRAW : flags) : old_flags);
        pend = valid && (fw & (RG_FLAG_REDRAW | RG_FLAG_SCR_CHANGED));
        pm = __ballot(pend);
        if (pm && lane == 0) lbase = atomicAdd(&S.obs_cnt[S.obs_par], (uint32_t)__popcll(pm));
    }
    if (S.stats) {
        const uint32_t cnt[8] = {(uint32_t)__popcll(__ballot(live && terminal && c.auto_reset)), (uint32_t)__popcll(__ballot(descends)),
                                 wave_sum(n_bfs), wave_sum(n_inline), wave_sum(n_taken), (uint32_t)__popcll(__ballot(live && (react & R_REDRAW))),
                                 (uint32_t)__popcll(__ballot(live)), (BW == 1 || BW == 2) ? wave_sum(n_cont) : 0u};
        const uint32_t n_nx = (uint32_t)__popcll(__ballot(descends && nxs == RG_NX_HIT));
        int ln = threadIdx.x;
        asm volatile("" : "+v"(ln));
        if (ln < RG_STAT_COLS) {
            uint32_t mine = ln == 8 ? n_nx : 0u;
#pragma unroll
            for (int k = 0; k < 8; k++) mine = ln == k ? cnt[k] : mine;
            if (mine) atomicAdd(&S.stats[(size_t)blockIdx.x * RG_STAT_COLS + ln], (unsigned long long)mine);
        }
    }
    if (valid && err) {
        S.flags[et] = (old_flags & ~RG_FLAG_ERR_MASK) | err;
        S.reward[et] = 0.f;
        S.done[et] = (old_flags & RG_FLAG_TERMINAL) ? 1 : 0;
        atomicOr(S.err_any, err);
    } else if (valid && !live) {
        S.reward[et] = 0.f; S.done[et] = (old_flags & RG_FLAG_TERMINAL) ? 1 : 0;
    } else if (valid) {
        if (terminal && c.auto_reset) {
            if (taken) {
                E.dlevel = 1; E.gold = c.init_gold; E.hp = E.hpmax = c.init_hp; E.plvl = 1; E.exp = 0; E.food = c.hunger_time;
            }
            write_status(S, c, E);
            S.dc_len[et] = 0; S.dc_head[et] = 0; S.dc_part[et] = 0; S.dc_own[et] = 0;
            steps = 0;
            flags = RG_FLAG_REDRAW | RG_FLAG_HIST_DIRTY;
            klog_new_episode(S, et);
        }
        if (E.err) { flags |= E.err; atomicOr(S.err_any, E.err); }
        if (terminal) flags |= RG_FLAG_TERMINAL;
        if (!taken) store_env(S, E);
        S.steps[et] = steps;
        S.flags[et] = flags;
        S.done[et] = terminal ? 1 : 0;
        if (S.ovl && !taken && !inc_done && ((react & R_REDRAW) || descends || (terminal && c.auto_reset))) {
            for (int s0 = 0; s0 < nrooms_k; s0++) {
                const uint32_t mw = E.mc[s0 * WAVE];
                S.ovl[(size_t)s0 * S.n + et] = (uint16_t)(((mw >> 24) & MF_ALIVE) ? ((mw & 0xffffu) | OVL_UNKNOWN) : OVL_NONE);
            }
            S.ovl[(size_t)nrooms_k * S.n + et] = (uint16_t)(POS(E.px, E.py) | OVL_UNKNOWN);
        }
        if (S.obs_rec && (flags & RG_FLAG_REDRAW) && !taken) {
            uint32_t *rec = S.obs_rec + (size_t)et * RG_OBS_REC_WORDS(nrooms_k);
            for (int s0 = 0; s0 < nrooms_k; s0 += 4) {
                uint32_t m4[4];
#pragma unroll
                for (int k = 0; k < 4; k++) m4[k] = E.mc[(s0 + k < nrooms_k ? s0 + k : s0) * WAVE];
                if (s0 + 4 <= nrooms_k) *reinterpret_cast<uint4 *>(rec + s0) = make_uint4(m4[0], m4[1], m4[2], m4[3]);
                else
                    for (int k = 0; k < 4 && s0 + k < nrooms_k; k++) rec[s0 + k] = m4[k];
            }
            rec[nrooms_k] = POS(E.px, E.py);
        }
        const int gold_before = gold0;
        const int gold_after = ((terminal && c.auto_reset) || (react & R_STATUS)) ? (int)E.gold : gold_before;
        const float bonus = (descends && !(terminal && c.auto_reset)) ? S.stair_reward : 0.f;
        S.reward[et] = (float)(gold_after - gold_before > 0 ? gold_after - gold_before : 0) + bonus;
    }
    bool on_next = false;
    if (valid && !live) on_next = S.stair_mark[(size_t)(S.stair_gen & 1) * S.n + et] != 0;
    if (live) on_next = ((descends || (terminal && c.auto_reset && !taken)) ? E.on_stairs != 0
                                                                              : (win_get(w, WIN_K(E.px - w.ox, E.py - w.oy)) & C_SURF_MASK) == S_STAIR);
    if (S.nx_state) {
        const bool fresh = live && (descends || (terminal && c.auto_reset));
        const bool ask = live && !fresh && (w.inb & WIN_STAIR) && (nxs == RG_NX_NONE || nxs == RG_NX_STALE);
        if (fresh && nxs != RG_NX_NONE) (void)__hip_atomic_fetch_and(&S.nx_state[et], RG_NX_DROP, __ATOMIC_RELAXED, __HIP_MEMORY_SCOPE_AGENT);
        if (__any(ask)) {
            if (ask) {
                uint32_t *q = S.nx_rng + et;
                const size_t n = (size_t)S.n;
                st_pub<true>(&q[0], E.rd.x); st_pub<true>(&q[n], E.rd.y); st_pub<true>(&q[2 * n], E.rd.z); st_pub<true>(&q[3 * n], E.rd.w);
                st_pub<true>(&q[8 * n], E.ri.x); st_pub<true>(&q[9 * n], E.ri.y); st_pub<true>(&q[10 * n], E.ri.z); st_pub<true>(&q[11 * n], E.ri.w);
                st_pub<true>(&S.nx->level[et], E.dlevel);
            }
            asm volatile("s_waitcnt vmcnt(0)" ::: "memory");
            if (ask) __hip_atomic_store(&S.nx_state[et], RG_NX_ASKED, __ATOMIC_RELAXED, __HIP_MEMORY_SCOPE_AGENT);
        }
    }
    if (BND && pm) {
        const uint32_t lb = uni(lbase);
        if (pend) S.obs_list[(size_t)S.obs_par * S.n + lb + lanes_below(pm)] = et;
    }
    take_spares(S, SPd, c, lane, et, taken, on_next);
    stair_publish(S, lane, et, valid, on_next);
    pf.mark(7);
    pf.finish();
}

#define STAIR_BLOCKS 256

#define RG_STEP_BLOCK_BODY(BWV, GMV, BNDV) \
    __builtin_amdgcn_s_setprio(3); \
    const int lane = threadIdx.x; \
    if (blockIdx.x == 0 && lane == 0) { \
        stair_recycle(S); \
        if (BNDV && S.obs_cnt) S.obs_cnt[S.obs_par ^ 1] = 0;   \
        __hip_atomic_store(S.launch_mark, (uint32_t)S.stair_gen + 1u, __ATOMIC_RELAXED, __HIP_MEMORY_SCOPE_AGENT);   \
    } \
    const bool stair = parity >= 0 && (int)blockIdx.x < STAIR_BLOCKS; \
    const int32_t *list = S.stair_list + (size_t)(S.stair_gen & 1) * S.n; \
    const int items = stair ? (int)S.stair_cnt[S.stair_gen % 3] : S.n; \
    const int first = stair ? (int)blockIdx.x : ((int)blockIdx.x - (parity >= 0 ? STAIR_BLOCKS : 0)) * epw; \
    uint32_t *next = S.stair_cnt + 4 + S.stair_gen % 3; \
    for (int i0 = first; i0 < items;) { \
        bool v; int e; \
        if (stair) { e = list[i0]; v = lane == 0 && e < S.n_keys && keys[e] == '>'; } \
        else { v = lane < epw && i0 + lane < items; e = v ? i0 + lane : 0; } \
        if (!stair || __any(v)) step_wave<BWV, GMV, BNDV>(S, SPd, c, keys, use_spares, stage_off, e, v, parity >= 0 ? (stair ? 1 : 2) : 0); \
        if (!stair || items <= STAIR_BLOCKS) break; \
        __syncthreads(); \
        uint32_t t = 0; \
        if (lane == 0) t = atomicAdd(next, 1u); \
        i0 = STAIR_BLOCKS + (int)uni(t); \
    }
template <int BW, bool BND = false>
__global__ void __launch_bounds__(WAVE) k_step(RgState S, const RgState *__restrict__ SPd, RgConfig c, const uint8_t *__restrict__ keys, int use_spares, int stage_off, int epw,
                                               int parity) {
    RG_STEP_BLOCK_BODY(BW, (BW != 0 ? 1 : 0), BND)
}
template <bool BND>
__global__ void __launch_bounds__(WAVE) __attribute__((amdgpu_waves_per_eu(2, 2)))
k_step_w32(RgState S, const RgState *__restrict__ SPd, RgConfig c, const uint8_t *__restrict__ keys, int use_spares, int stage_off, int epw, int parity) {
    RG_STEP_BLOCK_BODY(0, 0, BND)
}
__global__ void __launch_bounds__(WAVE) k_step_huge(RgState S, const RgState *__restrict__ SPd, RgConfig c, const uint8_t *__restrict__ keys, int use_spares, int stage_off,
                                                    int epw, int parity) {
    RG_STEP_BLOCK_BODY(4, 2, false)
}
#undef RG_STEP_BLOCK_BODY

static int gen_mode_of(const RgConfig *c) { const int nr = c->room_num_x * c->room_num_y; return nr <= 32 ? 0 : (nr <= 64 ? 1 : 2); }
extern "C" {
void rgk_build(const RgState *S, const RgConfig *c, hipStream_t st) {
    int hw = c->width * c->height;
    size_t smem = GEN_SLOT_BYTES(hw, c->room_num_x * c->room_num_y);
    const dim3 grid((S->n + BUILD_EPB - 1) / BUILD_EPB);
    switch (gen_mode_of(c)) {
    case 0: hipLaunchKernelGGL(k_build<0>, grid, dim3(WAVE), smem, st, *S, *c); break;
    case 1: hipLaunchKernelGGL(k_build<1>, grid, dim3(WAVE), smem, st, *S, *c); break;
    default: hipLaunchKernelGGL(k_build<2>, grid, dim3(WAVE), smem, st, *S, *c);
    }
}
int rgk_step_epw(int n, int slots_per_simd) {
    static const int epw_env = getenv("ROGUE_GYM_HIP_EPW") ? atoi(getenv("ROGUE_GYM_HIP_EPW")) : 0;
    int epw = WAVE;
    while (epw > 16 && (n + epw - 1) / epw < 1024) epw >>= 1;
    if (slots_per_simd < 2 && epw < WAVE && (n + epw - 1) / epw > 1008) { epw = (n + 1007) / 1008; if (epw > WAVE) epw = WAVE; }
    if (epw_env >= 16 && epw_env <= 64) epw = epw_env;
    return epw;
}
static size_t step_lds(const RgConfig *c, int *stage_off_out) {
    const int hw = c->width * c->height;
    size_t stage = GEN_SLOT_BYTES(hw, c->room_num_x * c->room_num_y);
    const bool n32 = c->width <= 96 && hw <= 4096;
    const size_t bfs_hi = n32 ? 0 : (size_t)10 * ((c->width + 63) / 64) * WAVE * 8;
    if (bfs_hi > stage) stage = bfs_hi;
    stage = (stage + 15) & ~(size_t)15;
    const int stage_off = STEP_LDS_MC + c->room_num_x * c->room_num_y * WAVE * 4;
    if (stage_off_out) *stage_off_out = stage_off;
    return (size_t)stage_off + stage;
}
size_t rgk_step_lds_per_cu(const RgConfig *c) { return step_lds(c, nullptr) * ((c->width <= 32 && gen_mode_of(c) == 0) ? 8 : 4); }
int rgk_step_bound_capable(const RgConfig *c) {
    const int hw = c->width * c->height;
    if (gen_mode_of(c) == 2) return 0;
    if (c->width <= 32 && gen_mode_of(c) == 0) return 1;
    return (c->width <= 96 && hw <= 4096 && c->width > 64) ? 1 : 0;
}
int rgk_step(const RgState *S, const RgState *SP_dev, const RgConfig *c, const uint8_t *keys, int use_spares, int parity, hipStream_t st, hipEvent_t ev0, hipEvent_t ev1) {
    const bool bnd = S->obs_list != nullptr && rgk_step_bound_capable(c);
    int hw = c->width * c->height;
    const bool n32 = c->width <= 96 && hw <= 4096;
    int stage_off = 0;
    const size_t smem = step_lds(c, &stage_off);
    const int epw = rgk_step_epw(S->n, (c->width <= 32 && gen_mode_of(c) == 0) ? 2 : 1);
    const int nb = (S->n + epw - 1) / epw;
    const dim3 grid(parity >= 0 ? STAIR_BLOCKS + nb : nb), block(WAVE);
#define RG_LAUNCH_STEP(K) do { if (ev0 || ev1) hipExtLaunchKernelGGL(K, grid, block, (uint32_t)smem, st, ev0, ev1, 0, *S, SP_dev, *c, keys, use_spares, stage_off, epw, parity); \
                               else hipLaunchKernelGGL(K, grid, block, smem, st, *S, SP_dev, *c, keys, use_spares, stage_off, epw, parity); } while (0)
    if (gen_mode_of(c) == 2) {
        static size_t raised[64] = {0};
        int dev = 0;
        (void)hipGetDevice(&dev);
        if (dev < 0 || dev >= 64 || smem > raised[dev]) {
            if (hipFuncSetAttribute(reinterpret_cast<const void *>(k_step_huge), hipFuncAttributeMaxDynamicSharedMemorySize, (int)smem) == hipSuccess && dev >= 0 && dev < 64) raised[dev] = smem;
        }
        RG_LAUNCH_STEP(k_step_huge);
    } else if (c->width <= 32 && gen_mode_of(c) == 0) { if (bnd) RG_LAUNCH_STEP(k_step_w32<true>); else RG_LAUNCH_STEP(k_step_w32<false>); }
    else if (n32 && c->width <= 64) RG_LAUNCH_STEP(k_step<1>);
    else if (n32) { if (bnd) RG_LAUNCH_STEP((k_step<2, true>)); else RG_LAUNCH_STEP(k_step<2>); }
    else if (c->width <= 128) RG_LAUNCH_STEP(k_step<3>);
    else RG_LAUNCH_STEP(k_step<4>);
#undef RG_LAUNCH_STEP
    return (int)grid.x;
}
void rgk_debug_descend(const RgState *S, const RgConfig *c, hipStream_t st) {
    int hw = c->width * c->height;
    const size_t smem = GEN_SLOT_BYTES(hw, c->room_num_x * c->room_num_y);
    const dim3 grid((S->n + BUILD_EPB - 1) / BUILD_EPB);
    switch (gen_mode_of(c)) {
    case 0: hipLaunchKernelGGL(k_debug_descend<0>, grid, dim3(WAVE), smem, st, *S, *c); break;
    case 1: hipLaunchKernelGGL(k_debug_descend<1>, grid, dim3(WAVE), smem, st, *S, *c); break;
    default: hipLaunchKernelGGL(k_debug_descend<2>, grid, dim3(WAVE), smem, st, *S, *c);
    }
}
void rgk_regen_gate(const uint32_t *mark, uint32_t target, uint32_t *err_any, hipStream_t st) { hipLaunchKernelGGL(k_regen_gate, dim3(1), dim3(WAVE), 0, st, mark, target, err_any); }
void rgk_regen(const RgState *SP, const RgConfig *c, int bulk, int spares, const uint32_t *mark, uint32_t target, uint32_t *err_any, hipStream_t st, hipEvent_t ev0, hipEvent_t ev1) {
    if (mark) rgk_regen_gate(mark, target, err_any, st);
    int hw = c->width * c->height;
    size_t smem = GEN_SLOT_BYTES(hw, c->room_num_x * c->room_num_y);
#ifdef RG_DEV_KNOBS
    static const int epb_env = getenv("ROGUE_GYM_HIP_REGEN_EPB") ? atoi(getenv("ROGUE_GYM_HIP_REGEN_EPB")) : 0;
    const int epb = (epb_env >= 4 && epb_env <= WAVE) ? epb_env : (spares == 1 ? 8 : WAVE);
    static const int claims_env = getenv("ROGUE_GYM_HIP_REGEN_CLAIMS") ? atoi(getenv("ROGUE_GYM_HIP_REGEN_CLAIMS")) : 1;
    const int max_claims = bulk ? WAVE : claims_env;
#else
    const int epb = spares == 1 ? 8 : WAVE, max_claims = bulk ? WAVE : 1;
#endif
    const dim3 grid((SP->n + epb - 1) / epb);
#define RG_LAUNCH_REGEN(K) do { if (ev0 || ev1) hipExtLaunchKernelGGL(K, grid, dim3(WAVE), (uint32_t)smem, st, ev0, ev1, 0, *SP, *c, epb, max_claims, spares); \
                                else hipLaunchKernelGGL(K, grid, dim3(WAVE), smem, st, *SP, *c, epb, max_claims, spares); } while (0)
    switch (gen_mode_of(c)) {
    case 0: RG_LAUNCH_REGEN(k_regen<0>); break;
    case 1: RG_LAUNCH_REGEN(k_regen<1>); break;
    default: RG_LAUNCH_REGEN(k_regen_huge);
    }
#undef RG_LAUNCH_REGEN
}
}
```

### rogue-gym_amd/csrc/rg_obs.hip

```cpp
#include <cstdlib>
#include "rg_device.h"

#define RENDER_THREADS 256
__device__ __forceinline__ bool in_same_room(const RgState &S, const RgConfig &c, int e, int ax, int ay, int bx, int by) {
    int id = room_id_of(c, ax, ay);
    if (id < 0 || room_id_of(c, bx, by) != id) return false;
    uint8_t meta = S.room_meta[id * S.n + e];
    if ((meta & RM_KIND_MASK) == RK_EMPTY) return true;
    int x0, y0, x1, y1;
    unpack_rect(S.room_rect[id * S.n + e], x0, y0, x1, y1);
    bool ina = ax >= x0 && ax < x1 && ay >= y0 && ay < y1, inb = bx >= x0 && bx < x1 && by >= y0 && by < y1;
    return ina == inb;
}

__global__ void __launch_bounds__(RENDER_THREADS) k_render(RgState S, RgConfig c) {
    __shared__ uint8_t s_scr[RG_MAX_W * RG_MAX_H];
    const int tid = threadIdx.x, W = c.width, H = c.height, HW = W * H, n = S.n;
    const int nrooms = c.room_num_x * c.room_num_y;
    for (int e = blockIdx.x; e < n; e += gridDim.x) {
        const uint32_t fl = S.flags[e];
        if (!(fl & RG_FLAG_REDRAW)) continue;
        const uint16_t *cell = S.cell + (size_t)e * HW;
        const bool upd_hist = !(fl & RG_FLAG_HIST_STALE);
        uint8_t *hist = S.hist + (size_t)e * HW;
        for (int i = tid; i < HW; i += RENDER_THREADS) {
            uint32_t v = cell[i];
            int y = i / W;
            uint8_t g = ' ';
            if (y >= 1 && y < H - 1 && (v & C_VISIBLE)) g = glyph_of(v);
            s_scr[i] = g;
            if (upd_hist) hist[i] = (v & C_VISITED) ? 1 : 0;
        }
        __syncthreads();
        const uint32_t ppos = S.p_pos[e];
        const int px = POS_X(ppos), py = POS_Y(ppos);
        for (int r = tid; r < nrooms; r += RENDER_THREADS) {
            uint32_t w = S.mon_w0[r * n + e];
            if ((w >> 24) & MF_ALIVE) {
                int x = POS_X(w), y = POS_Y(w);
                uint32_t v = cell[y * W + x];
                int dx = px - x, dy = py - y;
                if ((v & (C_VISIBLE | C_DRAWN)) && y >= 1 && y < H - 1 && (dx * dx + dy * dy <= 2 || in_same_room(S, c, e, px, py, x, y)))
                    s_scr[y * W + x] = c.mon[(w >> 16) & 0xff].tile;
            }
        }
        __syncthreads();
        for (int r = tid; r < nrooms; r += RENDER_THREADS) {
            uint32_t g = S.gold_pos[r * n + e];
            if (g & 0x10000u) {
                int x = POS_X(g), y = POS_Y(g);
                if ((cell[y * W + x] & (C_VISIBLE | C_DRAWN)) && y >= 1 && y < H - 1) s_scr[y * W + x] = '*';
            }
        }
        __syncthreads();
        if (tid == 0 && (cell[py * W + px] & (C_VISIBLE | C_DRAWN)) && py >= 1 && py < H - 1) s_scr[py * W + px] = '@';
        __syncthreads();
        uint8_t *scr = S.screen + (size_t)e * HW;
        if ((HW & 3) == 0) {
            uint32_t *d4 = reinterpret_cast<uint32_t *>(scr);
            const uint32_t *s4 = reinterpret_cast<const uint32_t *>(s_scr);
            for (int i = tid; i < HW / 4; i += RENDER_THREADS) d4[i] = s4[i];
        } else
            for (int i = tid; i < HW; i += RENDER_THREADS) scr[i] = s_scr[i];
        if (tid == 0)
            S.flags[e] = (fl & ~(RG_FLAG_REDRAW | RG_FLAG_HIST_STALE | RG_FLAG_HIST_LAG | (upd_hist ? RG_FLAG_HIST_DIRTY : 0u))) | ((fl & RG_FLAG_HIST_STALE) ? RG_FLAG_HIST_LAG : 0u);
        __syncthreads();
    }
}

__device__ __constant__ uint8_t kStatusIdx[9] = {0, 2, 3, 4, 5, 6, 7, 8, 9};

__global__ void __launch_bounds__(256) k_gray(const uint8_t *__restrict__ screen, const uint8_t *__restrict__ hist, const int32_t *__restrict__ status,
                                              int n, int hw, size_t rs, size_t rst, int symbols, uint32_t sflag, int with_hist, float *__restrict__ out,
                                              const int32_t *__restrict__ ext) {
    const int q = hw >> 2;
    const size_t total = (size_t)n * q;
    const int nplanes = 1 + __popc(sflag) + (with_hist ? 1 : 0);
    const float fsym = (float)(uint8_t)symbols;
    for (size_t g = (size_t)blockIdx.x * blockDim.x + threadIdx.x; g < total; g += (size_t)gridDim.x * blockDim.x) {
        int e = (int)(g / q), i = (int)(g - (size_t)e * q);
        uint32_t s4 = reinterpret_cast<const uint32_t *>(screen + (size_t)e * rs)[i];
        float4 v;
        v.x = (float)(uint8_t)tile_to_sym(s4 & 0xff) / fsym;
        v.y = (float)(uint8_t)tile_to_sym((s4 >> 8) & 0xff) / fsym;
        v.z = (float)(uint8_t)tile_to_sym((s4 >> 16) & 0xff) / fsym;
        v.w = (float)(uint8_t)tile_to_sym(s4 >> 24) / fsym;
        float4 *o = reinterpret_cast<float4 *>(out + (size_t)(ext ? ext[e] : e) * nplanes * hw) + i;
        o[0] = v;
        int p = 1;
        for (int b = 0; b < 9; b++)
            if (sflag & (1u << b)) {
                float f = (float)status[(size_t)e * rst + kStatusIdx[b]];
                float4 sv; sv.x = sv.y = sv.z = sv.w = f;
                o[(size_t)p * q] = sv;
                p++;
            }
        if (with_hist) {
            uint32_t h4 = reinterpret_cast<const uint32_t *>(hist + (size_t)e * rs)[i];
            float4 hv;
            hv.x = (h4 & 0xff) ? 1.f : 0.f; hv.y = (h4 & 0xff00) ? 1.f : 0.f; hv.z = (h4 & 0xff0000) ? 1.f : 0.f; hv.w = (h4 >> 24) ? 1.f : 0.f;
            o[(size_t)p * q] = hv;
        }
    }
}

__global__ void __launch_bounds__(256) k_symbol(const uint8_t *__restrict__ screen, const uint8_t *__restrict__ hist, const int32_t *__restrict__ status,
                                                uint32_t *__restrict__ flags, uint32_t *__restrict__ err_any,
                                                int n, int hw, size_t rs, size_t rst, int symbols, int planes_sym, uint32_t sflag, int with_hist, float *__restrict__ out,
                                                const int32_t *__restrict__ ext) {
    const int q = hw >> 2;
    const size_t total = (size_t)n * q;
    const int nplanes = planes_sym + __popc(sflag) + (with_hist ? 1 : 0);
    const uint32_t symbol_max = (uint32_t)symbols - 1;
    for (size_t g = (size_t)blockIdx.x * blockDim.x + threadIdx.x; g < total; g += (size_t)gridDim.x * blockDim.x) {
        int e = (int)(g / q), i = (int)(g - (size_t)e * q);
        uint32_t s4 = reinterpret_cast<const uint32_t *>(screen + (size_t)e * rs)[i];
        uint32_t a = tile_to_sym(s4 & 0xff), b = tile_to_sym((s4 >> 8) & 0xff), cc = tile_to_sym((s4 >> 16) & 0xff), d = tile_to_sym(s4 >> 24);
        if (a >= symbol_max || b >= symbol_max || cc >= symbol_max || d >= symbol_max) {
            if (flags) atomicOr(&flags[e], RG_FLAG_ERR_TILE);
            atomicOr(err_any, RG_FLAG_ERR_TILE);
        }
        float4 *o = reinterpret_cast<float4 *>(out + (size_t)(ext ? ext[e] : e) * nplanes * hw) + i;
        for (uint32_t ch = 0; ch < (uint32_t)planes_sym; ch++) {
            float4 v;
            v.x = a == ch ? 1.f : 0.f; v.y = b == ch ? 1.f : 0.f; v.z = cc == ch ? 1.f : 0.f; v.w = d == ch ? 1.f : 0.f;
            if (ch >= symbol_max) v.x = v.y = v.z = v.w = 0.f;
            o[(size_t)ch * q] = v;
        }
        int p = planes_sym;
        for (int bb = 0; bb < 9; bb++)
            if (sflag & (1u << bb)) {
                float f = (float)status[(size_t)e * rst + kStatusIdx[bb]];
                float4 sv; sv.x = sv.y = sv.z = sv.w = f;
                o[(size_t)p * q] = sv;
                p++;
            }
        if (with_hist) {
            uint32_t h4 = reinterpret_cast<const uint32_t *>(hist + (size_t)e * rs)[i];
            float4 hv;
            hv.x = (h4 & 0xff) ? 1.f : 0.f; hv.y = (h4 & 0xff00) ? 1.f : 0.f; hv.z = (h4 & 0xff0000) ? 1.f : 0.f; hv.w = (h4 >> 24) ? 1.f : 0.f;
            o[(size_t)p * q] = hv;
        }
    }
}

#define OBS_THREADS 256
__device__ __forceinline__ void store_obs(float4 *p, float4 v) {
    typedef float f4v __attribute__((ext_vector_type(4)));
    f4v nv = {v.x, v.y, v.z, v.w};
#ifdef RG_EXP_OBS_PLAIN_STORES
    *reinterpret_cast<f4v *>(p) = nv;
#else
    __builtin_nontemporal_store(nv, reinterpret_cast<f4v *>(p));
#endif
}
struct ObsTabs { uint32_t w[RG_OBS_REC_WORDS(RG_OBS_MAX_ROOMS)]; };
#define OBS_ENV_BYTES(hw) ((((size_t)(hw) + sizeof(ObsTabs)) + 15) & ~(size_t)15)

__device__ __forceinline__ void draw_cells8(uint4 v, int i, int W, int HW, uint32_t g[2], uint32_t hb[2]) {
    const uint32_t q[4] = {v.x, v.y, v.z, v.w};
    g[0] = g[1] = hb[0] = hb[1] = 0;
#pragma unroll
    for (int t = 0; t < 8; t++) {
        uint32_t cw = (q[t >> 1] >> ((t & 1) * 16)) & 0xffff;
        int idx = i * 8 + t;
        bool inner = idx >= W && idx < HW - W;
        uint32_t gl = ' ';
        if (inner && (cw & C_VISIBLE)) gl = glyph_of(cw);
        if (inner && (cw & (C_VISIBLE | C_DRAWN))) gl = ((cw & C_GOLD) ? (uint32_t)'*' : gl) | 0x80u;
        g[t >> 2] |= gl << ((t & 3) * 8);
        hb[t >> 2] |= ((cw & C_VISITED) ? 1u : 0u) << ((t & 3) * 8);
    }
}
__device__ __forceinline__ bool monster_shown(const RgConfig &c, const ObsTabs *tb, int nrooms, int px, int py, int x, int y) {
    int dx = px - x, dy = py - y;
    bool show = dx * dx + dy * dy <= 2;
    if (!show) {
        int id = room_id_of(c, px, py);
        if (id >= 0 && room_id_of(c, x, y) == id) {
            if ((reinterpret_cast<const uint8_t *>(&tb->w[2 * nrooms + 1])[id] & RM_KIND_MASK) == RK_EMPTY) show = true;
            else {
                int x0, y0, x1, y1;
                unpack_rect(tb->w[nrooms + 1 + id], x0, y0, x1, y1);
                bool ina = px >= x0 && px < x1 && py >= y0 && py < y1, inb = x >= x0 && x < x1 && y >= y0 && y < y1;
                show = ina == inb;
            }
        }
    }
    return show;
}

__device__ __forceinline__ void lds_barrier() { asm volatile("s_waitcnt lgkmcnt(0)\n\ts_barrier" ::: "memory"); }

template <int KIND, bool GROUPS, bool BOUND = false>
__global__ void __launch_bounds__(OBS_THREADS) k_obs(RgState S, RgConfig c, uint32_t sflag, int with_hist, float *__restrict__ out,
                                                    uint32_t *__restrict__ err_any, int tpe, int epb, int planes_sym, int hi_prio) {
    if (hi_prio) __builtin_amdgcn_s_setprio(3);
    extern __shared__ __align__(16) uint8_t smem[];
    float *lutf = reinterpret_cast<float *>(smem);
    uint8_t *luts = smem + 512;
    uint8_t *mtile = smem + 512 + 128;
    uint8_t *envs = smem + 512 + 128 + 64;
    const int tid = threadIdx.x, W = c.width, H = c.height, HW = W * H, Q8 = HW >> 3;
    const int32_t *list = BOUND ? S.obs_list + (size_t)S.obs_par * S.n : nullptr;
    const int n = BOUND ? (int)S.obs_cnt[S.obs_par] : S.n;
    const int nrooms = c.room_num_x * c.room_num_y;
    const int symbols = c.symbols;
    for (int g = tid; g < 128; g += blockDim.x) {
        uint32_t sy = tile_to_sym((uint32_t)g);
        luts[g] = (uint8_t)sy;
        lutf[g] = (float)(uint8_t)sy / (float)(uint8_t)symbols;
    }
    for (int g = tid; g < RG_MAX_ENEMY_KINDS + 6; g += blockDim.x) mtile[g] = c.mon[g].tile;
    const int le = tid / tpe, lt = tid - le * tpe;
    const int base_planes = KIND ? (GROUPS ? planes_sym : symbols) : 1;
    const int nplanes = base_planes + __popc(sflag) + (with_hist ? 1 : 0);
    uint8_t *scr = envs + (size_t)le * OBS_ENV_BYTES(HW);
    ObsTabs *tb = reinterpret_cast<ObsTabs *>(scr + HW);
    struct Pre { uint4 v0; uint32_t rec; };
    const int rec_words = RG_OBS_REC_WORDS(nrooms);
    const uint32_t *rec_all = S.obs_rec;
    const int stride = gridDim.x * epb;
    const int Q4 = HW >> 2;
    const bool one_wave = blockDim.x == WAVE;
    const bool fast_ok = (epb == 1 || one_wave) && Q4 <= 4 * tpe && sflag == 0 && !with_hist;
    auto load_env = [&](int base) -> int {
        const int i = base + le;
        if (!BOUND) return i;
        return (le < epb && i < n) ? list[i] : 0;
    };
    auto load_flag = [&](int base, int e) -> uint32_t {
        return (le < epb && base + le < n) ? S.flags[e] : 0u;
    };
    auto prefetch = [&](int base, int e, uint32_t fl) {
        Pre p; p.v0 = make_uint4(0, 0, 0, 0); p.rec = 0;
        if (le < epb && base + le < n) {
            if (fl & RG_FLAG_REDRAW) {
                if (lt < Q8) p.v0 = reinterpret_cast<const uint4 *>(S.cell + (size_t)e * HW)[lt];
                if (lt < rec_words) p.rec = rec_all[(size_t)e * rec_words + lt];
            } else if (fast_ok) {
                const uint32_t *m4 = reinterpret_cast<const uint32_t *>(S.screen + (size_t)e * HW);
                if (lt < Q4) p.v0.x = m4[lt];
                if (lt + tpe < Q4) p.v0.y = m4[lt + tpe];
                if (lt + 2 * tpe < Q4) p.v0.z = m4[lt + 2 * tpe];
                if (lt + 3 * tpe < Q4) p.v0.w = m4[lt + 3 * tpe];
            } else if (lt < Q8) {
                const uint2 m = reinterpret_cast<const uint2 *>(S.screen + (size_t)e * HW)[lt];
                p.v0.x = m.x; p.v0.y = m.y;
            }
        }
        return p;
    };
    const uint32_t smax = (uint32_t)symbols - 1;
    auto emit_glyphs = [&](float4 *o, int q, uint32_t g, bool &bad) {
        const int q4 = Q4;
        const uint32_t b0 = g & 0x7f, b1 = (g >> 8) & 0x7f, b2 = (g >> 16) & 0x7f, b3 = g >> 24;
        if (KIND == 0) {
            float4 v; v.x = lutf[b0]; v.y = lutf[b1]; v.z = lutf[b2]; v.w = lutf[b3];
            store_obs(&o[q], v);
        } else {
            const uint32_t s0 = luts[b0], s1 = luts[b1], s2 = luts[b2], s3 = luts[b3];
            bad = bad || s0 >= smax || s1 >= smax || s2 >= smax || s3 >= smax;
            for (uint32_t ch = 0; ch < smax; ch++) {
                float4 v;
                v.x = s0 == ch ? 1.f : 0.f; v.y = s1 == ch ? 1.f : 0.f; v.z = s2 == ch ? 1.f : 0.f; v.w = s3 == ch ? 1.f : 0.f;
                store_obs(&o[(size_t)ch * q4 + q], v);
            }
            float4 z; z.x = z.y = z.z = z.w = 0.f;
            for (uint32_t ch = smax; ch < (uint32_t)base_planes; ch++) store_obs(&o[(size_t)ch * q4 + q], z);
        }
    };
    auto emit = [&](float4 *o, int q, uint32_t g, const float *stf, int nst, const uint32_t *hist4, bool &bad) {
        const int q4 = Q4;
        emit_glyphs(o, q, g, bad);
        int p = base_planes;
        for (int b = 0; b < nst; b++, p++) {
            float4 sv; sv.x = sv.y = sv.z = sv.w = stf[b];
            store_obs(&o[(size_t)p * q4 + q], sv);
        }
        if (with_hist) {
            const uint32_t h4 = hist4[q];
            float4 a;
            a.x = (h4 & 0xff) ? 1.f : 0.f; a.y = (h4 & 0xff00) ? 1.f : 0.f; a.z = (h4 & 0xff0000) ? 1.f : 0.f; a.w = (h4 >> 24) ? 1.f : 0.f;
            store_obs(&o[(size_t)p * q4 + q], a);
        }
    };
    lds_barrier();
    const int base0 = blockIdx.x * epb;
    int e_cur = load_env(base0), e_nxt = load_env(base0 + stride), e_nn = load_env(base0 + 2 * stride);
    uint32_t fl_cur = load_flag(base0, e_cur), fl_nxt = load_flag(base0 + stride, e_nxt);
    Pre nxt = prefetch(base0, e_cur, fl_cur);
    for (int base = base0; base < n; base += stride) {
        const int e = e_cur;
        const bool valid = le < epb && base + le < n;
        const Pre cur = nxt;
        const uint32_t fl = fl_cur;
        e_cur = e_nxt; e_nxt = e_nn;
        fl_cur = fl_nxt;
        fl_nxt = load_flag(base + 2 * stride, e_nxt);
        e_nn = load_env(base + 3 * stride);
        if (base + stride < n) nxt = prefetch(base + stride, e_cur, fl_cur);
        const uint4 *cell4 = reinterpret_cast<const uint4 *>(S.cell + (size_t)e * HW);
        const uint4 v0 = cur.v0;
        const uint32_t t_rec = cur.rec;
        const bool my_fast = fast_ok && valid && !(fl & RG_FLAG_REDRAW);
        if (my_fast) {
            const int xe = GROUPS ? __builtin_amdgcn_readfirstlane(S.ext[e]) : e;
            float4 *o = reinterpret_cast<float4 *>(out + (size_t)xe * nplanes * HW);
            bool bad = false;
            if (lt < Q4) emit_glyphs(o, lt, v0.x & 0x7f7f7f7fu, bad);
            if (lt + tpe < Q4) emit_glyphs(o, lt + tpe, v0.y & 0x7f7f7f7fu, bad);
            if (lt + 2 * tpe < Q4) emit_glyphs(o, lt + 2 * tpe, v0.z & 0x7f7f7f7fu, bad);
            if (lt + 3 * tpe < Q4) emit_glyphs(o, lt + 3 * tpe, v0.w & 0x7f7f7f7fu, bad);
            if (KIND == 1 && bad) { atomicOr(&S.flags[e], RG_FLAG_ERR_TILE); atomicOr(err_any, RG_FLAG_ERR_TILE); }
            if (BOUND && lt == 0) atomicAnd(&S.flags[e], ~RG_FLAG_SCR_CHANGED);
        }
        const bool staged = valid && !my_fast;
        if (fast_ok && !(one_wave ? __any(staged) : staged)) continue;
        const bool redraw = staged && (fl & RG_FLAG_REDRAW);
        lds_barrier();
        if (staged) {
            if (redraw) {
                if (lt < rec_words) tb->w[lt] = t_rec;
                const bool upd_hist = !(fl & RG_FLAG_HIST_STALE) && (fl & RG_FLAG_HIST_DIRTY);
                uint2 *hist8 = reinterpret_cast<uint2 *>(S.hist + (size_t)e * HW);
                for (int i = lt; i < Q8; i += tpe) {
                    uint4 v = i == lt ? v0 : cell4[i];
                    uint32_t g[2], hb[2];
                    draw_cells8(v, i, W, HW, g, hb);
                    reinterpret_cast<uint2 *>(scr)[i] = make_uint2(g[0], g[1]);
                    if (upd_hist) hist8[i] = make_uint2(hb[0], hb[1]);
                }
            } else {
                const uint2 *m8 = reinterpret_cast<const uint2 *>(S.screen + (size_t)e * HW);
                for (int i = lt; i < Q8; i += tpe) reinterpret_cast<uint2 *>(scr)[i] = i == lt ? make_uint2(v0.x, v0.y) : m8[i];
            }
        }
        lds_barrier();
        const uint32_t ppos = redraw ? tb->w[nrooms] : 0;
        const int px = POS_X(ppos), py = POS_Y(ppos);
        if (redraw && lt < nrooms) {
            uint32_t w = tb->w[lt];
            if ((w >> 24) & MF_ALIVE) {
                int x = POS_X(w), y = POS_Y(w);
                const bool show = monster_shown(c, tb, nrooms, px, py, x, y);
                const uint32_t under = scr[y * W + x];
                if (show && (under & 0x80u) && under != (0x80u | '*')) scr[y * W + x] = (uint8_t)(0x80u | mtile[(w >> 16) & 0xff]);
            }
        }
        lds_barrier();
        if (redraw && lt == 0 && (scr[py * W + px] & 0x80u)) scr[py * W + px] = (uint8_t)(0x80u | '@');
        lds_barrier();
        if (with_hist) __syncthreads();
        if (staged) {
            uint32_t *m4 = reinterpret_cast<uint32_t *>(S.screen + (size_t)e * HW);
            const uint32_t *scr4 = reinterpret_cast<const uint32_t *>(scr);
            const uint32_t *hist4 = reinterpret_cast<const uint32_t *>(S.hist + (size_t)e * HW);
            const int xe = GROUPS ? __builtin_amdgcn_readfirstlane(S.ext[e]) : e;
            float4 *o = reinterpret_cast<float4 *>(out + (size_t)xe * nplanes * HW);
            float stf[9];
            int nst = 0;
            for (int b = 0; b < 9; b++)
                if (sflag & (1u << b)) stf[nst++] = (float)S.status[(size_t)e * 10 + kStatusIdx[b]];
            bool bad = false;
            for (int q = lt; q < Q4; q += tpe) {
                const uint32_t g = scr4[q] & 0x7f7f7f7fu;
                if (redraw) m4[q] = g;
                emit(o, q, g, stf, nst, hist4, bad);
            }
            if (KIND == 1 && bad) { atomicOr(&S.flags[e], RG_FLAG_ERR_TILE); atomicOr(err_any, RG_FLAG_ERR_TILE); }
            const uint32_t seen = BOUND ? RG_FLAG_SCR_CHANGED : 0u;
            if (redraw && lt == 0) {
                const uint32_t clr = seen | RG_FLAG_REDRAW | RG_FLAG_HIST_STALE | RG_FLAG_HIST_LAG | ((fl & RG_FLAG_HIST_STALE) ? 0u : RG_FLAG_HIST_DIRTY);
                const uint32_t set = (fl & RG_FLAG_HIST_STALE) ? RG_FLAG_HIST_LAG : 0u;
                if (KIND == 1) {
                    atomicAnd(&S.flags[e], ~clr);
                    if (set) atomicOr(&S.flags[e], set);
                } else S.flags[e] = (fl & ~clr) | set;
            } else if (BOUND && !redraw && lt == 0) atomicAnd(&S.flags[e], ~RG_FLAG_SCR_CHANGED);
        }
    }
}

#ifndef OBS_RUN
#define OBS_RUN 4
#endif
#ifndef OBS_STREAM_WAVES
#define OBS_STREAM_WAVES 16384
#endif
__global__ void __launch_bounds__(WAVE) k_obs_stream(RgState S, RgConfig c, float *__restrict__ out, int hi_prio) {
    if (hi_prio) __builtin_amdgcn_s_setprio(3);
    __shared__ float lutf[128];
    __shared__ uint8_t mtile[RG_MAX_ENEMY_KINDS + 6];
    __shared__ __align__(16) uint8_t scr[512];
    __shared__ ObsTabs tb;
    const int lane = threadIdx.x, W = c.width, HW = W * c.height, Q4 = HW >> 2, Q8 = HW >> 3, n = S.n;
    const int nrooms = c.room_num_x * c.room_num_y, rec_words = RG_OBS_REC_WORDS(nrooms);
    for (int g = lane; g < 128; g += WAVE) lutf[g] = (float)(uint8_t)tile_to_sym((uint32_t)g) / (float)(uint8_t)c.symbols;
    for (int g = lane; g < RG_MAX_ENEMY_KINDS + 6; g += WAVE) mtile[g] = c.mon[g].tile;
    lds_barrier();
    auto gray4 = [&](uint32_t w) {
        w &= 0x7f7f7f7fu;
        float4 v; v.x = lutf[w & 0xff]; v.y = lutf[(w >> 8) & 0xff]; v.z = lutf[(w >> 16) & 0xff]; v.w = lutf[w >> 24];
        return v;
    };
    struct Run { uint32_t fl, w0[OBS_RUN], w1[OBS_RUN]; };
    auto load_run = [&](int r, Run &R) {
        const int base = r * OBS_RUN, cnt = n - base;
        R.fl = lane < cnt && lane < OBS_RUN ? S.flags[base + lane] : 0u;
        const uint32_t *m = reinterpret_cast<const uint32_t *>(S.screen) + (size_t)base * Q4;
#pragma unroll
        for (int i = 0; i < OBS_RUN; i++) {
            R.w0[i] = i < cnt && lane < Q4 ? m[i * Q4 + lane] : 0u;
            R.w1[i] = i < cnt && lane + WAVE < Q4 ? m[i * Q4 + lane + WAVE] : 0u;
        }
    };
    const int nruns = (n + OBS_RUN - 1) / OBS_RUN;
    Run cur;
    load_run(blockIdx.x, cur);
    for (int r = blockIdx.x; r < nruns; r += gridDim.x) {
        const int base = r * OBS_RUN, cnt = n - base < OBS_RUN ? n - base : OBS_RUN;
        Run nxt;
        load_run(r + gridDim.x, nxt);
        const uint32_t fl = cur.fl;
#ifdef RG_EXP_OBS_STREAM_BOUND
        uint64_t rmask = 0;
#else
        uint64_t rmask = __ballot(fl & RG_FLAG_REDRAW);
#endif
        auto load_tiles = [&](int e, uint4 &v, uint32_t &rec) {
            v = lane < Q8 ? reinterpret_cast<const uint4 *>(S.cell + (size_t)e * HW)[lane] : make_uint4(0, 0, 0, 0);
            rec = lane < rec_words ? S.obs_rec[(size_t)e * rec_words + lane] : 0u;
        };
        uint4 tv = make_uint4(0, 0, 0, 0);
        uint32_t trec = 0;
        if (rmask) load_tiles(base + __builtin_ctzll(rmask), tv, trec);
        float4 *o = reinterpret_cast<float4 *>(out) + (size_t)base * Q4;
#pragma unroll
        for (int i = 0; i < OBS_RUN; i++) {
            if (i >= cnt || ((rmask >> i) & 1)) continue;
            if (lane < Q4) store_obs(&o[i * Q4 + lane], gray4(cur.w0[i]));
            if (lane + WAVE < Q4) store_obs(&o[i * Q4 + lane + WAVE], gray4(cur.w1[i]));
        }
        while (rmask) {
            const int i = __builtin_ctzll(rmask);
            rmask &= rmask - 1;
            const int e = base + i;
            const uint32_t fle = __builtin_amdgcn_readlane(fl, i);
            const uint4 v = tv;
            const uint32_t t_rec = trec;
            if (rmask) load_tiles(base + __builtin_ctzll(rmask), tv, trec);
            lds_barrier();
            if (lane < rec_words) tb.w[lane] = t_rec;
            const bool upd_hist = !(fle & RG_FLAG_HIST_STALE) && (fle & RG_FLAG_HIST_DIRTY);
            if (lane < Q8) {
                uint32_t g[2], hb[2];
                draw_cells8(v, lane, W, HW, g, hb);
                reinterpret_cast<uint2 *>(scr)[lane] = make_uint2(g[0], g[1]);
                if (upd_hist) reinterpret_cast<uint2 *>(S.hist + (size_t)e * HW)[lane] = make_uint2(hb[0], hb[1]);
            }
            lds_barrier();
            const uint32_t ppos = tb.w[nrooms];
            const int px = POS_X(ppos), py = POS_Y(ppos);
            if (lane < nrooms) {
                const uint32_t mw = tb.w[lane];
                if ((mw >> 24) & MF_ALIVE) {
                    const int x = POS_X(mw), y = POS_Y(mw);
                    const uint32_t under = scr[y * W + x];
                    if (monster_shown(c, &tb, nrooms, px, py, x, y) && (under & 0x80u) && under != (0x80u | '*')) scr[y * W + x] = (uint8_t)(0x80u | mtile[(mw >> 16) & 0xff]);
                }
            }
            lds_barrier();
            if (lane == 0 && (scr[py * W + px] & 0x80u)) scr[py * W + px] = (uint8_t)(0x80u | '@');
            lds_barrier();
            uint32_t *m4 = reinterpret_cast<uint32_t *>(S.screen + (size_t)e * HW);
            float4 *oe = reinterpret_cast<float4 *>(out) + (size_t)e * Q4;
            for (int q = lane; q < Q4; q += WAVE) {
                const uint32_t g = reinterpret_cast<const uint32_t *>(scr)[q] & 0x7f7f7f7fu;
                m4[q] = g;
                store_obs(&oe[q], gray4(g));
            }
            if (lane == 0)
                S.flags[e] = (fle & ~(RG_FLAG_REDRAW | RG_FLAG_HIST_STALE | RG_FLAG_HIST_LAG | ((fle & RG_FLAG_HIST_STALE) ? 0u : RG_FLAG_HIST_DIRTY))) |
                             ((fle & RG_FLAG_HIST_STALE) ? RG_FLAG_HIST_LAG : 0u);
        }
        cur = nxt;
    }
}

#define RG_PUBLIC_FLAGS (RG_FLAG_TERMINAL | RG_FLAG_DEAD | RG_FLAG_MSG_MASK | RG_FLAG_ERR_MASK)
__global__ void __launch_bounds__(256) k_pack(const uint8_t *__restrict__ screen, const uint8_t *__restrict__ hist, const int32_t *__restrict__ status,
                                              const float *__restrict__ reward, const uint32_t *__restrict__ flags, int n, int hw, int with_hist, uint32_t *__restrict__ out) {
    const int qs = hw >> 2, qr = qs + 12 + (with_hist ? qs : 0);
    const size_t total = (size_t)n * qr;
    for (size_t g = (size_t)blockIdx.x * blockDim.x + threadIdx.x; g < total; g += (size_t)gridDim.x * blockDim.x) {
        const int e = (int)(g / qr), i = (int)(g - (size_t)e * qr);
        uint32_t v;
        if (i < qs) v = reinterpret_cast<const uint32_t *>(screen + (size_t)e * hw)[i];
        else if (i < qs + 10) v = (uint32_t)status[(size_t)e * 10 + (i - qs)];
        else if (i == qs + 10) v = __float_as_uint(reward[e]);
        else if (i == qs + 11) v = flags[e] & RG_PUBLIC_FLAGS;
        else v = reinterpret_cast<const uint32_t *>(hist + (size_t)e * hw)[i - qs - 12];
        out[g] = v;
    }
}

__global__ void __launch_bounds__(256) k_export(const uint32_t *__restrict__ screen, const uint32_t *__restrict__ hist, const uint32_t *__restrict__ status,
                                                const uint32_t *__restrict__ flags, uint32_t *__restrict__ err_any, size_t w_scr, size_t w_status, size_t w_flags,
                                                uint32_t *__restrict__ o_screen, uint32_t *__restrict__ o_hist, uint32_t *__restrict__ o_status,
                                                uint32_t *__restrict__ o_flags, uint32_t *__restrict__ o_err) {
    const size_t total = (o_screen ? 2 * w_scr : 0) + w_status + w_flags;
    const size_t base = o_screen ? 2 * w_scr : 0;
    for (size_t g = (size_t)blockIdx.x * blockDim.x + threadIdx.x; g < total; g += (size_t)gridDim.x * blockDim.x) {
        if (g < base) { if (g < w_scr) o_screen[g] = screen[g]; else o_hist[g - w_scr] = hist[g - w_scr]; }
        else if (g < base + w_status) o_status[g - base] = status[g - base];
        else o_flags[g - base - w_status] = flags[g - base - w_status];
    }
    if (blockIdx.x == 0 && threadIdx.x == 0) {
        const uint32_t e = atomicExch(err_any, 0u);
        *o_err = e;
    }
}
__global__ void __launch_bounds__(256) k_scatter_rows(const uint8_t *__restrict__ src, uint8_t *__restrict__ dst, const int32_t *__restrict__ ext, int n, int row_bytes) {
    if ((row_bytes & 3) == 0) {
        const int rw = row_bytes >> 2;
        const size_t total = (size_t)n * rw;
        for (size_t g = (size_t)blockIdx.x * blockDim.x + threadIdx.x; g < total; g += (size_t)gridDim.x * blockDim.x) {
            const int e = (int)(g / rw), i = (int)(g - (size_t)e * rw);
            reinterpret_cast<uint32_t *>(dst)[(size_t)ext[e] * rw + i] = reinterpret_cast<const uint32_t *>(src)[g];
        }
    } else {
        const size_t total = (size_t)n * row_bytes;
        for (size_t g = (size_t)blockIdx.x * blockDim.x + threadIdx.x; g < total; g += (size_t)gridDim.x * blockDim.x) {
            const int e = (int)(g / row_bytes), i = (int)(g - (size_t)e * row_bytes);
            dst[(size_t)ext[e] * row_bytes + i] = src[g];
        }
    }
}
__global__ void __launch_bounds__(256) k_gather_keys(const uint8_t *__restrict__ keys, const int32_t *__restrict__ ext, uint8_t *__restrict__ dst, int n) {
    const int e = blockIdx.x * 256 + threadIdx.x;
    if (e < n) dst[e] = keys[ext[e]];
}

__global__ void k_probe_clock(unsigned long long *out, int spin) {
    const unsigned long long c0 = __builtin_amdgcn_s_memtime(), r0 = __builtin_amdgcn_s_memrealtime();
    uint32_t x = threadIdx.x + 1u;
    for (int i = 0; i < spin; i++) x = x * 1664525u + 1013904223u;
    const unsigned long long c1 = __builtin_amdgcn_s_memtime(), r1 = __builtin_amdgcn_s_memrealtime();
    if (threadIdx.x == 0) { out[0] = c1 - c0; out[1] = r1 - r0; out[2] = x; out[3] = (unsigned long long)spin; }
}

__global__ void __launch_bounds__(256) k_encode_scalar(const uint8_t *__restrict__ screen, const uint8_t *__restrict__ hist, const int32_t *__restrict__ status,
                                                       uint32_t *__restrict__ flags, uint32_t *__restrict__ err_any, int n, int hw, size_t rs, size_t rst, int symbols,
                                                       int planes_sym, uint32_t sflag, int with_hist, int kind, float *__restrict__ out, const int32_t *__restrict__ ext) {
    const size_t total = (size_t)n * hw;
    const int base = kind ? planes_sym : 1;
    const int nplanes = base + __popc(sflag) + (with_hist ? 1 : 0);
    for (size_t g = (size_t)blockIdx.x * blockDim.x + threadIdx.x; g < total; g += (size_t)gridDim.x * blockDim.x) {
        int e = (int)(g / hw), i = (int)(g - (size_t)e * hw);
        uint32_t sym = tile_to_sym(screen[(size_t)e * rs + i]);
        float *o = out + (size_t)(ext ? ext[e] : e) * nplanes * hw + i;
        if (!kind) o[0] = (float)(uint8_t)sym / (float)(uint8_t)symbols;
        else {
            if (sym >= (uint32_t)symbols - 1) { if (flags) atomicOr(&flags[e], RG_FLAG_ERR_TILE); atomicOr(err_any, RG_FLAG_ERR_TILE); }
            for (int ch = 0; ch < planes_sym; ch++) o[(size_t)ch * hw] = (sym == (uint32_t)ch && ch < symbols - 1) ? 1.f : 0.f;
        }
        int p = base;
        for (int b = 0; b < 9; b++)
            if (sflag & (1u << b)) { o[(size_t)p * hw] = (float)status[(size_t)e * rst + kStatusIdx[b]]; p++; }
        if (with_hist) o[(size_t)p * hw] = hist[(size_t)e * rs + i] ? 1.f : 0.f;
    }
}

enum { CROP_D_CA, CROP_D_AREA, CROP_D_WC, CROP_D_BB, CROP_D_BW };
__device__ __forceinline__ uint32_t mdiv(uint32_t x, uint32_t m, uint32_t shifts, int which) {
    return (uint32_t)(((uint64_t)x * m) >> ((shifts >> (6 * which)) & 63));
}
struct RgCropArgs {
    int ry, rx, hc, wc, area, ca;
    int run, bh, bw, bb;
    int planes, nst, with_hist, nplanes;
    uint32_t sflag;
    uint32_t m[5], shifts;
};
#define CROP_UNROLL 8
template <int KIND>
__global__ void __launch_bounds__(WAVE) k_obs_crop(const uint16_t *__restrict__ p_pos, const int32_t *__restrict__ status, const uint8_t *__restrict__ screen,
                                                  const uint8_t *__restrict__ hist, uint32_t *__restrict__ flags, const int32_t *__restrict__ ext, int n, int W, int H,
                                                  int symbols, RgCropArgs a, float *__restrict__ out, int32_t *__restrict__ centers, uint32_t *__restrict__ err_any) {
    extern __shared__ __align__(16) uint8_t smem[];
    float *lutf = reinterpret_cast<float *>(smem);
    uint8_t *luts = smem + 512;
    int4 *geo = reinterpret_cast<int4 *>(smem + 640);
    float *stf = reinterpret_cast<float *>(smem + 640 + 16 * a.run);
    uint8_t *box = smem + 640 + 52 * a.run;
    uint8_t *hbox = box + (size_t)a.run * a.bb;
    const int lane = threadIdx.x, HW = W * H, R = a.run;
    for (int g = lane; g < 128; g += WAVE) {
        const uint32_t sy = tile_to_sym((uint32_t)g);
        luts[g] = (uint8_t)sy;
        lutf[g] = (float)(uint8_t)sy / (float)(uint8_t)symbols;
    }
    const uint32_t smax = (uint32_t)symbols - 1;
    const int nruns = (n + R - 1) / R;
    for (int run = blockIdx.x; run < nruns; run += gridDim.x) {
        const int base = run * R, cnt = n - base < R ? n - base : R;
        lds_barrier();
        if (lane < cnt) {
            const int e = base + lane;
            const uint32_t pos = p_pos[e];
            const int cx = POS_X(pos), cy = POS_Y(pos);
            const int oy = min(max(cy - a.ry, 0), H - a.bh), ox = min(max(cx - a.rx, 0), W - a.bw);
            geo[lane] = make_int4(cy, cx, oy, ox);
            int p = 0;
            for (int b = 0; b < 9; b++)
                if (a.sflag & (1u << b)) stf[lane * 9 + p++] = (float)status[(size_t)e * 10 + kStatusIdx[b]];
            if (centers) {
                const int xe = ext ? ext[e] : e;
                centers[2 * (size_t)xe] = cy;
                centers[2 * (size_t)xe + 1] = cx;
            }
        }
        lds_barrier();
        const int tot = cnt * a.bb;
        auto box_cell = [&](int k, int &r, int &y, int &x) {
            r = (int)mdiv((uint32_t)k, a.m[CROP_D_BB], a.shifts, CROP_D_BB);
            const int t = k - r * a.bb, j = (int)mdiv((uint32_t)t, a.m[CROP_D_BW], a.shifts, CROP_D_BW);
            const int4 gg = geo[r];
            y = gg.z + j; x = gg.w + (t - j * a.bw);
        };
        for (int k0 = 0; k0 < tot; k0 += WAVE * CROP_UNROLL) {
            uint32_t gv[CROP_UNROLL], hv[CROP_UNROLL];
#pragma unroll
            for (int u = 0; u < CROP_UNROLL; u++) {
                const int kk = k0 + u * WAVE + lane;
                gv[u] = hv[u] = 0;
                if (KIND == 0 || kk < tot) {
                    int r, y, x;
                    box_cell(min(kk, tot - 1), r, y, x);
                    const size_t off = (size_t)(base + r) * HW + y * W + x;
                    gv[u] = screen[off];
// ... 110 lines not shown
            const uint32_t ppos = tb.w[nrooms];
            const int px = POS_X(ppos), py = POS_Y(ppos);
            for (int rm = tid; rm < nrooms; rm += B) {
                const uint32_t mw = tb.w[rm];
                if ((mw >> 24) & MF_ALIVE) {
                    const int x = POS_X(mw), y = POS_Y(mw);
                    const uint32_t under = scr[y * W + x];
                    if (monster_shown(c, &tb, nrooms, px, py, x, y) && (under & 0x80u) && under != (0x80u | '*')) scr[y * W + x] = (uint8_t)(0x80u | mtile[(mw >> 16) & 0xff]);
                }
            }
            lds_barrier();
            if (tid == 0 && (scr[py * W + px] & 0x80u)) scr[py * W + px] = (uint8_t)(0x80u | '@');
            lds_barrier();
            uint2 *m8 = reinterpret_cast<uint2 *>(S.screen + (size_t)e * HW);
            for (int j = tid; j < (HW >> 3); j += B) {
                const uint2 g = reinterpret_cast<const uint2 *>(scr)[j];
                m8[j] = make_uint2(g.x & 0x7f7f7f7fu, g.y & 0x7f7f7f7fu);
            }
            if (tid == 0)
                S.flags[e] = (fle & ~(RG_FLAG_REDRAW | RG_FLAG_HIST_STALE | RG_FLAG_HIST_LAG | ((fle & RG_FLAG_HIST_STALE) ? 0u : RG_FLAG_HIST_DIRTY))) |
                             ((fle & RG_FLAG_HIST_STALE) ? RG_FLAG_HIST_LAG : 0u);
        }
        fl = fl_nxt;
    }
}

#define OBS_T_ITEMS 4
typedef uint32_t u4v __attribute__((ext_vector_type(4)));
__device__ __forceinline__ void store_obs16(u4v *p, uint32_t a, uint32_t b, uint32_t c, uint32_t d) {
    u4v v = {a, b, c, d};
    __builtin_nontemporal_store(v, p);
}
template <int DT>
__device__ __forceinline__ uint32_t cvt16(float f) {
    if (DT == RG_OBS_F16) return (uint32_t)__builtin_bit_cast(uint16_t, (_Float16)f);
    const uint32_t u = __float_as_uint(f);
    return (u + 0x7fffu + ((u >> 16) & 1u)) >> 16;
}
__device__ __forceinline__ uint32_t nonzero_bytes(uint32_t w) { return ((w | ((w & 0x7f7f7f7fu) + 0x7f7f7f7fu)) >> 7) & 0x01010101u; }

template <int KIND, int DT>
__global__ void __launch_bounds__(OBS_THREADS) k_obs_typed(const uint8_t *__restrict__ screen, const uint8_t *__restrict__ hist, const int32_t *__restrict__ status,
                                                          uint32_t *__restrict__ flags, uint32_t *__restrict__ err_any, int n, int hw, int symbols, int planes,
                                                          uint32_t sflag, int with_hist, int run, u4v *__restrict__ out) {
    constexpr int CW = DT == RG_OBS_U8 ? 4 : 2;
    typedef uint32_t wv __attribute__((ext_vector_type(CW)));
    constexpr uint32_t ONE = DT == RG_OBS_F16 ? 0x3C00u : 0x3F80u;
    __shared__ uint16_t lut16[128];
    __shared__ uint8_t luts[128];
    const int tid = threadIdx.x, B = blockDim.x, Q = hw / (4 * CW);
    for (int g = tid; g < 128; g += B) {
        const uint32_t sy = tile_to_sym((uint32_t)g);
        luts[g] = (uint8_t)sy;
        if (KIND == 0) lut16[g] = (uint16_t)cvt16<DT>((float)(uint8_t)sy / (float)(uint8_t)symbols);
    }
    const int nplanes = planes + __popc(sflag) + (with_hist ? 1 : 0);
    const uint32_t smax = (uint32_t)symbols - 1;
    const int per_run = run * Q;
    int el[OBS_T_ITEMS], ql[OBS_T_ITEMS];
#pragma unroll
    for (int k = 0; k < OBS_T_ITEMS; k++) {
        const int j = tid + k * B;
        el[k] = j < per_run ? j / Q : -1;
        ql[k] = el[k] < 0 ? 0 : j - el[k] * Q;
    }
    struct Run { wv w[OBS_T_ITEMS], h[OBS_T_ITEMS]; };
    auto load_run = [&](int r, Run &R) {
        const int base = r * run;
        const wv *m = reinterpret_cast<const wv *>(screen + (size_t)base * hw), *hm = reinterpret_cast<const wv *>(hist + (size_t)base * hw);
#pragma unroll
        for (int k = 0; k < OBS_T_ITEMS; k++) {
            const bool ok = el[k] >= 0 && base + el[k] < n;
            R.w[k] = ok ? m[tid + k * B] : (wv)0u;
            R.h[k] = ok && with_hist ? hm[tid + k * B] : (wv)0u;
        }
    };
    auto gray2 = [&](uint32_t w, int hi) -> uint32_t {
        return (uint32_t)lut16[(w >> (16 * hi)) & 0x7f] | ((uint32_t)lut16[(w >> (16 * hi + 8)) & 0x7f] << 16);
    };
    auto one2 = [&](bool a, bool b) -> uint32_t { return (a ? ONE : 0u) | (b ? ONE << 16 : 0u); };
    lds_barrier();
    const int nruns = (n + run - 1) / run;
    Run cur;
    load_run(blockIdx.x, cur);
    for (int r = blockIdx.x; r < nruns; r += gridDim.x) {
        Run nxt;
        load_run(r + gridDim.x, nxt);
        const int base = r * run;
#pragma unroll
        for (int k = 0; k < OBS_T_ITEMS; k++) {
            const int e = base + el[k];
            if (el[k] < 0 || e >= n) continue;
            u4v *o = out + (size_t)e * nplanes * Q + ql[k];
            uint32_t w[CW], h[CW];
#pragma unroll
            for (int t = 0; t < CW; t++) { w[t] = cur.w[k][t]; h[t] = cur.h[k][t]; }
            bool bad = false;
            if (KIND == 0) {
                store_obs16(o, gray2(w[0], 0), gray2(w[0], 1), gray2(w[1], 0), gray2(w[1], 1));
            } else if (KIND == 1) {
                uint32_t s[8];
#pragma unroll
                for (int t = 0; t < 8; t++) {
                    s[t] = luts[(w[t >> 2] >> ((t & 3) * 8)) & 0x7f];
                    bad = bad || s[t] >= smax;
                }
                for (uint32_t ch = 0; ch < smax; ch++)
                    store_obs16(o + (size_t)ch * Q, one2(s[0] == ch, s[1] == ch), one2(s[2] == ch, s[3] == ch), one2(s[4] == ch, s[5] == ch), one2(s[6] == ch, s[7] == ch));
                for (uint32_t ch = smax; ch < (uint32_t)planes; ch++) store_obs16(o + (size_t)ch * Q, 0u, 0u, 0u, 0u);
            } else {
                uint32_t id[CW];
#pragma unroll
                for (int t = 0; t < CW; t++) {
                    const uint32_t a = luts[w[t] & 0x7f], b = luts[(w[t] >> 8) & 0x7f], c = luts[(w[t] >> 16) & 0x7f], d = luts[(w[t] >> 24) & 0x7f];
                    bad = bad || a >= smax || b >= smax || c >= smax || d >= smax;
                    id[t] = a | (b << 8) | (c << 16) | (d << 24);
                }
                store_obs16(o, id[0], id[1], id[CW - 2], id[CW - 1]);
            }
            int p = planes;
            if (KIND != 2 && sflag) {
                const int eu = __builtin_amdgcn_readfirstlane(e);
                for (int b = 0; b < 9; b++)
                    if (sflag & (1u << b)) {
                        const uint32_t v = cvt16<DT>((float)status[(size_t)eu * 10 + kStatusIdx[b]]) * 0x10001u;
                        store_obs16(o + (size_t)p * Q, v, v, v, v);
                        p++;
                    }
            }
            if (with_hist) {
                if (KIND == 2) store_obs16(o + (size_t)p * Q, nonzero_bytes(h[0]), nonzero_bytes(h[1]), nonzero_bytes(h[CW - 2]), nonzero_bytes(h[CW - 1]));
                else
                    store_obs16(o + (size_t)p * Q, one2(h[0] & 0xffu, h[0] & 0xff00u), one2(h[0] & 0xff0000u, h[0] >> 24), one2(h[1] & 0xffu, h[1] & 0xff00u),
                                one2(h[1] & 0xff0000u, h[1] >> 24));
            }
            if (KIND != 0 && bad) { atomicOr(&flags[e], RG_FLAG_ERR_TILE); atomicOr(err_any, RG_FLAG_ERR_TILE); }
        }
        cur = nxt;
    }
}

static void host_magic(RgCropArgs &a, int which, uint32_t d) {
    uint32_t l = 0;
    while ((1u << l) < d) l++;
    const uint32_t s = 30 + l;
    a.m[which] = (uint32_t)(((1ull << s) + d - 1) / d);
    a.shifts |= s << (6 * which);
}
extern "C" {
void rgk_render(const RgState *S, const RgConfig *c, hipStream_t st) {
    int blocks = S->n < 8192 ? S->n : 8192;
    hipLaunchKernelGGL(k_render, dim3(blocks), dim3(RENDER_THREADS), 0, st, *S, *c);
}
int rgk_obs(const RgState *S, const RgConfig *c, uint32_t sflag, int with_hist, int kind, float *out, uint32_t *err_any, int planes_sym, int bound, hipStream_t st, hipEvent_t ev0, hipEvent_t ev1) {
    int hw = c->width * c->height;
    if (hw & 7) return 0;
    if (c->room_num_x * c->room_num_y > RG_OBS_MAX_ROOMS || !S->obs_rec) return 0;
    int q8 = hw / 8;
    int tpe = q8 >= OBS_THREADS ? OBS_THREADS : ((q8 + 63) / 64) * 64;
    if (tpe > OBS_THREADS) tpe = OBS_THREADS;
    if (RG_OBS_REC_WORDS(c->room_num_x * c->room_num_y) > tpe) return 0;
    const int bthreads = tpe, epb = 1;
    const bool groups = S->ext != nullptr;
    size_t smem = 512 + 128 + 64 + (size_t)epb * OBS_ENV_BYTES(hw);
    int blocks = (S->n + epb - 1) / epb;
    {
        int cap = bthreads <= 64 ? 16384 : 8192;
#ifdef RG_DEV_KNOBS
        if (const char *ev = getenv("RG_OBS_BLOCKS")) cap = atoi(ev);
#endif
        if (blocks > cap) blocks = cap;
    }
    const int hi_prio = !(c->width <= 32 && c->room_num_x * c->room_num_y <= 32);
    bool stream = !kind && !groups && !bound && sflag == 0 && !with_hist && tpe == WAVE;
#ifdef RG_DEV_KNOBS
    if (const char *ev = getenv("RG_OBS_STREAM")) stream = stream && atoi(ev) != 0;
#endif
    if (stream) {
        int sblocks = (S->n + OBS_RUN - 1) / OBS_RUN, cap = OBS_STREAM_WAVES;
#ifdef RG_DEV_KNOBS
        if (const char *ev = getenv("RG_OBS_BLOCKS")) if (atoi(ev) > 0) cap = atoi(ev);
#endif
        if (sblocks > cap) sblocks = cap;
        if (ev0 || ev1) hipExtLaunchKernelGGL(k_obs_stream, dim3(sblocks), dim3(WAVE), 0, st, ev0, ev1, 0, *S, *c, out, hi_prio);
        else hipLaunchKernelGGL(k_obs_stream, dim3(sblocks), dim3(WAVE), 0, st, *S, *c, out, hi_prio);
        return 1;
    }
#define RG_LAUNCH_OBS(...) do { if (ev0 || ev1) hipExtLaunchKernelGGL((__VA_ARGS__), dim3(blocks), dim3(bthreads), (uint32_t)smem, st, ev0, ev1, 0, *S, *c, sflag, with_hist, out, err_any, tpe, epb, planes_sym, hi_prio); \
                               else hipLaunchKernelGGL((__VA_ARGS__), dim3(blocks), dim3(bthreads), smem, st, *S, *c, sflag, with_hist, out, err_any, tpe, epb, planes_sym, hi_prio); } while (0)
    if (bound && !groups && !kind) RG_LAUNCH_OBS(k_obs<0, false, true>);
    else if (bound && !groups) RG_LAUNCH_OBS(k_obs<1, false, true>);
    else if (!kind && !groups) RG_LAUNCH_OBS(k_obs<0, false>);
    else if (!kind) RG_LAUNCH_OBS(k_obs<0, true>);
    else if (!groups) RG_LAUNCH_OBS(k_obs<1, false>);
    else RG_LAUNCH_OBS(k_obs<1, true>);
#undef RG_LAUNCH_OBS
    return 1;
}
void rgk_encode(const uint8_t *screen, const uint8_t *hist, const int32_t *status, uint32_t *flags, uint32_t *err_any, int n, int hw, size_t rs, size_t rst,
                int symbols, int planes_sym, uint32_t sflag, int with_hist, int kind, float *out, const int32_t *ext, hipStream_t st) {
    if ((hw & 3) == 0 && (rs & 3) == 0) {
        size_t total = (size_t)n * (hw >> 2);
        int blocks = (int)((total + 255) / 256 < 16384 ? (total + 255) / 256 : 16384);
        if (blocks < 1) blocks = 1;
        if (!kind) hipLaunchKernelGGL(k_gray, dim3(blocks), dim3(256), 0, st, screen, hist, status, n, hw, rs, rst, symbols, sflag, with_hist, out, ext);
        else hipLaunchKernelGGL(k_symbol, dim3(blocks), dim3(256), 0, st, screen, hist, status, flags, err_any, n, hw, rs, rst, symbols, planes_sym, sflag, with_hist, out, ext);
    } else {
        size_t total = (size_t)n * hw;
        int blocks = (int)((total + 255) / 256 < 16384 ? (total + 255) / 256 : 16384);
        hipLaunchKernelGGL(k_encode_scalar, dim3(blocks), dim3(256), 0, st, screen, hist, status, flags, err_any, n, hw, rs, rst, symbols, planes_sym, sflag, with_hist, kind, out, ext);
    }
}
void rgk_export(const RgState *S, uint32_t *err_any, void *o_screen, void *o_hist, void *o_status, void *o_flags, uint32_t *o_err, hipStream_t st) {
    const size_t n = (size_t)S->n, w_scr = n * (size_t)S->hw / 4, w_status = n * 10, w_flags = n;
    const size_t total = (o_screen ? 2 * w_scr : 0) + w_status + w_flags;
    int blocks = (int)((total + 255) / 256 < 1024 ? (total + 255) / 256 : 1024);
    hipLaunchKernelGGL(k_export, dim3(blocks < 1 ? 1 : blocks), dim3(256), 0, st, reinterpret_cast<const uint32_t *>(S->screen), reinterpret_cast<const uint32_t *>(S->hist),
                       reinterpret_cast<const uint32_t *>(S->status), S->flags, err_any, w_scr, w_status, w_flags, static_cast<uint32_t *>(o_screen), static_cast<uint32_t *>(o_hist),
                       static_cast<uint32_t *>(o_status), static_cast<uint32_t *>(o_flags), o_err);
}
void rgk_pack(const RgState *S, int with_hist, uint8_t *out, hipStream_t st) {
    const int hw = S->hw;
    const size_t rec = (size_t)hw + RG_COMPACT_FIXED_BYTES + (with_hist ? hw : 0);
    const size_t total = (size_t)S->n * (rec / 4);
    int blocks = (int)((total + 255) / 256 < 16384 ? (total + 255) / 256 : 16384);
    if (blocks < 1) blocks = 1;
    hipLaunchKernelGGL(k_pack, dim3(blocks), dim3(256), 0, st, S->screen, S->hist, S->status, S->reward, S->flags, S->n, hw, with_hist, reinterpret_cast<uint32_t *>(out));
}
void rgk_scatter_rows(const void *src, void *dst, const int32_t *ext, int n, int row_bytes, hipStream_t st) {
    const size_t total = (size_t)n * row_bytes;
    int blocks = (int)((total + 255) / 256 < 8192 ? (total + 255) / 256 : 8192);
    if (blocks < 1) blocks = 1;
    hipLaunchKernelGGL(k_scatter_rows, dim3(blocks), dim3(256), 0, st, (const uint8_t *)src, (uint8_t *)dst, ext, n, row_bytes);
}
void rgk_gather_keys(const uint8_t *keys, const int32_t *ext, uint8_t *dst, int n, hipStream_t st) {
    hipLaunchKernelGGL(k_gather_keys, dim3((n + 255) / 256), dim3(256), 0, st, keys, ext, dst, n);
}
int rgk_obs_crop(const RgState *S, const RgConfig *c, int kind, int ry, int rx, uint32_t sflag, int with_hist, int planes_sym, float *out, int32_t *centers,
                 uint32_t *err_any, hipStream_t st) {
    RgCropArgs a;
    const int hc = 2 * ry + 1;
    a.ry = ry; a.rx = rx; a.hc = hc; a.wc = 2 * rx + 1; a.area = hc * a.wc;
    a.planes = kind ? planes_sym : 1; a.nst = __builtin_popcount(sflag); a.with_hist = with_hist ? 1 : 0; a.sflag = sflag;
    a.nplanes = a.planes + a.nst + a.with_hist;
    a.ca = a.nplanes * a.area;
    a.bh = hc < c->height ? hc : c->height; a.bw = a.wc < c->width ? a.wc : c->width; a.bb = a.bh * a.bw;
    a.run = 4;
    const size_t stage = (size_t)a.bb * (1 + a.with_hist);
    while (a.run < 64 && (size_t)a.run * a.ca * 4 < 4096 && (size_t)a.run * 2 * stage <= 16384) a.run *= 2;
    if ((uint64_t)a.run * a.ca >= (1ull << 30) || (uint64_t)a.run * a.bb >= (1ull << 30)) return 0;
    a.shifts = 0;
    host_magic(a, CROP_D_CA, (uint32_t)a.ca); host_magic(a, CROP_D_AREA, (uint32_t)a.area); host_magic(a, CROP_D_WC, (uint32_t)a.wc);
    host_magic(a, CROP_D_BB, (uint32_t)a.bb); host_magic(a, CROP_D_BW, (uint32_t)a.bw);
    const size_t smem = 640 + 52 * (size_t)a.run + (size_t)a.run * stage;
    const int nruns = (S->n + a.run - 1) / a.run;
    const int blocks = nruns < OBS_STREAM_WAVES ? nruns : OBS_STREAM_WAVES;
    if (kind) hipLaunchKernelGGL(k_obs_crop<1>, dim3(blocks), dim3(WAVE), smem, st, S->p_pos, S->status, S->screen, S->hist, S->flags, S->ext, S->n, c->width, c->height,
                                 c->symbols, a, out, centers, err_any);
    else hipLaunchKernelGGL(k_obs_crop<0>, dim3(blocks), dim3(WAVE), smem, st, S->p_pos, S->status, S->screen, S->hist, S->flags, S->ext, S->n, c->width, c->height,
                            c->symbols, a, out, centers, err_any);
    return 1;
}
int rgk_redraw(const RgState *S, const RgConfig *c, hipStream_t st) {
    const int hw = c->width * c->height;
    if ((hw & 7) || c->room_num_x * c->room_num_y > RG_OBS_MAX_ROOMS || !S->obs_rec) return 0;
    int B = ((hw / 8 + WAVE - 1) / WAVE) * WAVE;
    if (B > OBS_THREADS) B = OBS_THREADS;
    const int nruns = (S->n + REDRAW_RUN - 1) / REDRAW_RUN;
    hipLaunchKernelGGL(k_redraw, dim3(nruns < 8192 ? nruns : 8192), dim3(B), (size_t)hw, st, *S, *c);
    return 1;
}
int rgk_obs_typed(const RgState *S, const RgConfig *c, int kind, int dtype, uint32_t sflag, int with_hist, int planes_sym, void *out, uint32_t *err_any,
                  hipStream_t st, hipEvent_t ev0, hipEvent_t ev1) {
    const int hw = c->width * c->height, cells = dtype == RG_OBS_U8 ? 16 : 8;
    if (hw % cells) return 0;
    const int Q = hw / cells;
    int B = ((Q + WAVE - 1) / WAVE) * WAVE;
    if (B > OBS_THREADS) B = OBS_THREADS;
    if (Q > OBS_T_ITEMS * B) return 0;
    int run = sflag ? 1 : OBS_T_ITEMS * B / Q;
    if (run < 1) run = 1;
    const int nruns = (S->n + run - 1) / run, cap = B <= WAVE ? OBS_STREAM_WAVES : 4096;
    const int blocks = nruns < cap ? nruns : cap;
    const int planes = kind == 1 ? planes_sym : 1;
#define RG_LAUNCH_TYPED(...) do { if (ev0 || ev1) hipExtLaunchKernelGGL((__VA_ARGS__), dim3(blocks), dim3(B), 0, st, ev0, ev1, 0, S->screen, S->hist, S->status, S->flags, err_any, S->n, hw, \
                                                                        (int)c->symbols, planes, sflag, with_hist, run, static_cast<u4v *>(out)); \
                                  else hipLaunchKernelGGL((__VA_ARGS__), dim3(blocks), dim3(B), 0, st, S->screen, S->hist, S->status, S->flags, err_any, S->n, hw, (int)c->symbols, planes, sflag, \
                                                          with_hist, run, static_cast<u4v *>(out)); } while (0)
    if (kind == 2) RG_LAUNCH_TYPED(k_obs_typed<2, RG_OBS_U8>);
    else if (kind == 0 && dtype == RG_OBS_F16) RG_LAUNCH_TYPED(k_obs_typed<0, RG_OBS_F16>);
    else if (kind == 0) RG_LAUNCH_TYPED(k_obs_typed<0, RG_OBS_BF16>);
    else if (dtype == RG_OBS_F16) RG_LAUNCH_TYPED(k_obs_typed<1, RG_OBS_F16>);
    else RG_LAUNCH_TYPED(k_obs_typed<1, RG_OBS_BF16>);
#undef RG_LAUNCH_TYPED
    return 1;
}
void rgk_probe_clock(unsigned long long *out, int spin, hipStream_t st) { hipLaunchKernelGGL(k_probe_clock, dim3(1), dim3(64), 0, st, out, spin); }
}
```

### rogue-gym_amd/csrc/rg_state.h

```cpp
#pragma once
#include <cstdint>

#include "rg_config.h"

#define C_SURF_MASK 0x0007u
#define C_DOOR      0x0008u
#define C_ATTR_SHIFT 4
#define C_VISITED   0x0010u
#define C_HIDDEN    0x0020u
#define C_VISIBLE   0x0040u
#define C_DRAWN     0x0080u
#define C_LOCKED    0x0100u
#define C_DARK      0x0200u
#define C_ATTR_MASK 0x03f0u
#define C_MAZE      0x0400u
#define C_GOLD      0x0800u

enum { S_PASSAGE = 0, S_FLOOR, S_WALLX, S_WALLY, S_STAIR, S_DOOR, S_TRAP, S_NONE };

#define RM_KIND_MASK 0x03u
#define RM_DARK      0x04u
#define RM_VISITED   0x08u
#define RM_HAS_GOLD  0x10u
enum { RK_NORMAL = 0, RK_MAZE = 1, RK_EMPTY = 2 };

#define MF_ALIVE   0x01u
#define MF_ACTIVE  0x02u
#define MF_PENDING 0x04u
#define MF_RANDOM 0x08u
#define MF_DIR_SHIFT 4
#define MF_REACH 0x80u
#define MF_TURN_BITS (MF_PENDING | MF_RANDOM | (7u << MF_DIR_SHIFT) | MF_REACH)

#define RG_MAX_EDGES (2 * RG_MAX_ROOMS)
#define RG_WALK_WORDS(w) ((w) <= 64 ? 2 : 3)
#define RG_PARTIAL_MAPS(w, h, rooms) ((w) <= 96 && (w) * (h) <= 4096 && (rooms) <= 64 && !((w) <= 32 && (rooms) <= 32))

#define RG_STAT_COLS 16
#define RG_NX_ASKED 1u
#define RG_NX_CLAIMED 6u
#define RG_NX_READY 3u
#define RG_NX_NONE 0u
#define RG_NX_DROP 4u
#define RG_NX_STALE 8u
#define RG_NX_HIT 9u
struct RgNext {
    uint16_t *cell;
    uint32_t *room_rect, *gold_pos, *gold_amt;
    uint8_t *room_meta;
    uint32_t *level;
};
struct RgState {
    int32_t n;
    int32_t hw;
    uint16_t *cell;
    uint8_t *screen;
    uint8_t *hist;
    uint16_t *p_pos;
    int32_t *p_hp, *p_hpmax, *p_lvl;
    uint32_t *p_exp, *food, *quiet, *pack_gold, *dlevel;
    uint32_t *steps, *flags;
    float *reward;
    uint8_t *done;
    uint32_t *rng;
    uint64_t *seed_lo, *seed_hi;
    uint8_t *reseed;
    uint32_t *build_ctr;
    const uint32_t *init_draws;
    uint64_t *range_lo, *range_span;
    uint32_t *room_rect;
    uint8_t *room_meta;
    uint32_t *mon_w0;
    int32_t *mon_hp;
    uint32_t *mon_exp;
    uint32_t *mon_cnt;
    uint32_t *gold_pos, *gold_amt;
    uint32_t *edge_a, *edge_b;
    uint16_t *maze_stack;
    int32_t maze_cap;
    uint16_t *dc_map;
    uint16_t *dc_key;
    uint8_t *dc_head, *dc_len;
    uint16_t *dc_part, *dc_own;
    uint32_t *dc_walk;
    int keep_spares;
    int full_bfs;
    unsigned long long *prof;
    uint32_t *sp_ready;
    int32_t sp_slots;
    int32_t *status;
    uint32_t *obs_rec;
    uint16_t *ovl;
    float *bound_gray;
    const float *gray_lut;
    int32_t *obs_list;
    uint32_t *obs_cnt;
    int32_t obs_par;
    uint8_t *klog;
    uint32_t *klog_len;
    uint8_t *klog_cur;
    int32_t klog_cap;
    unsigned long long *stats;
    uint8_t *stair_mark;
    int32_t *stair_list;
    uint32_t *stair_cnt;
    int32_t stair_gen;
    uint32_t *launch_mark;
    uint8_t *on_stairs;
    uint32_t *nx_state;
    uint32_t *nx_rng;
    const struct RgNext *nx;
    const int32_t *ext;
    uint32_t *err_any;
    int32_t n_keys;
    float stair_reward;
};
```

Baseline: 757.7 million env-steps/s.

## Fuse gray observation encoding into step kernel tail, leave redraws to separate pass

When step and gray observation are requested together under simple conditions, the w32 step kernel now encodes each wave's screen rows into the float observation buffer at the end of the step, using an LDS gray LUT. A new redraw-only variant of the streaming obs kernel then handles only envs flagged for redraw, with a larger run per block, instead of re-reading every screen. This removes a full separate pass over screens and its launch cost from the common path, at the cost of extra register and LDS pressure in the step kernel. The gray LUT is now built once at creation rather than lazily.

Result: slower. 648.7 million env-steps/s (-14.4%).

```diff
diff --git a/rogue-gym_amd/csrc/rg_api.cpp b/rogue-gym_amd/csrc/rg_api.cpp
--- a/rogue-gym_amd/csrc/rg_api.cpp
+++ b/rogue-gym_amd/csrc/rg_api.cpp
@@ -31,6 +31,8 @@
 void rgk_export(const RgState *S, uint32_t *err_any, void *o_screen, void *o_hist, void *o_status, void *o_flags, uint32_t *o_err, hipStream_t st);
 int rgk_regen_lanes_supported(const RgConfig *c, int maze_cap);
 int rgk_step_bound_capable(const RgConfig *c);
+int rgk_step_obs_capable(const RgConfig *c);
+int rgk_obs_streams(const RgState *S, const RgConfig *c);
 int rgk_regen_lanes(const RgState *SP, const RgConfig *c, uint32_t *q, int32_t *list, int bulk, int waves, int slots, hipStream_t st, hipEvent_t ev0, hipEvent_t ev1);
 void rgk_debug_descend(const RgState *S, const RgConfig *c, hipStream_t st);
 void rgk_render(const RgState *S, const RgConfig *c, hipStream_t st);
@@ -39,7 +41,7 @@
 void rgk_pack(const RgState *S, int with_hist, uint8_t *out, hipStream_t st);
 void rgk_scatter_rows(const void *src, void *dst, const int32_t *ext, int n, int row_bytes, hipStream_t st);
 void rgk_gather_keys(const uint8_t *keys, const int32_t *ext, uint8_t *dst, int n, hipStream_t st);
-int rgk_obs(const RgState *S, const RgConfig *c, uint32_t sflag, int with_hist, int kind, float *out, uint32_t *err_any, int planes_sym, int bound, hipStream_t st, hipEvent_t ev0, hipEvent_t ev1);
+int rgk_obs(const RgState *S, const RgConfig *c, uint32_t sflag, int with_hist, int kind, float *out, uint32_t *err_any, int planes_sym, int bound, int redraw_only, hipStream_t st, hipEvent_t ev0, hipEvent_t ev1);
 int rgk_redraw(const RgState *S, const RgConfig *c, hipStream_t st);
 int rgk_obs_typed(const RgState *S, const RgConfig *c, int kind, int dtype, uint32_t sflag, int with_hist, int planes_sym, void *out, uint32_t *err_any, hipStream_t st, hipEvent_t ev0,
                   hipEvent_t ev1);
@@ -163,6 +165,7 @@
     h->allocs.clear();
 }
 
+static uint32_t host_tile_to_sym(uint32_t t);
 static int flush_render(rg_handle *h) {
     if (h->render_pending) {
         { TimedLaunch t(h, 1); rgk_render(&h->S, &h->cfg, h->stream); }
@@ -256,6 +259,13 @@
               dev_alloc(h, &S.dc_head, n) && dev_alloc(h, &S.dc_len, n) && dev_alloc(h, &S.dc_part, n) && dev_alloc(h, &S.dc_own, n) && dev_alloc(h, &S.status, n * 10) &&
               dev_alloc(h, &h->d_err, 4) && dev_alloc(h, &h->d_keys, n);
     if (ok && nr <= RG_OBS_MAX_ROOMS) ok = dev_alloc(h, &S.obs_rec, n * (size_t)RG_OBS_REC_WORDS(nr));
+    if (ok) {
+        float lut[128];
+        for (uint32_t g = 0; g < 128; g++) lut[g] = (float)(uint8_t)host_tile_to_sym(g) / (float)(uint8_t)h->cfg.symbols;
+        ok = dev_alloc(h, &h->gray_lut_mem, 128) && hipMemcpy(h->gray_lut_mem, lut, sizeof lut, hipMemcpyHostToDevice) == hipSuccess;
+        if (!ok && h->err.empty()) h->err = "hipMemcpy failed";
+        S.gray_lut = h->gray_lut_mem;
+    }
     if (ok && nr <= RG_OVL_MAX && getenv("ROGUE_GYM_HIP_NO_MIRROR_UPDATE") == nullptr)
         ok = dev_alloc(h, &S.ovl, (nr + 1) * n) && hipMemset(S.ovl, 0xff, (nr + 1) * n * 2) == hipSuccess;
     h->spares = auto_reset != 0 && getenv("ROGUE_GYM_HIP_NO_SPARES") == nullptr;
@@ -531,10 +541,21 @@
     return 0;
 }
 
-static int obs_common(rg_t *h, uint32_t status_flag, int with_hist, int kind, float *out_dev);
+static int obs_common(rg_t *h, uint32_t status_flag, int with_hist, int kind, float *out_dev, bool redraw_only = false);
 int rg_step(rg_t *h, const uint8_t *keys, int keys_on_device) { return rg_step_prefix(h, keys, h->S.n, keys_on_device); }
+static bool step_obs_fusable(rg_handle *h, uint32_t status_flag, int with_hist, float *out_dev) {
+#ifdef RG_DEV_KNOBS
+    if (const char *ev = getenv("RG_STEP_OBS_FUSE")) if (atoi(ev) == 0) return false;
+#endif
+    return h->sub.empty() && out_dev && (status_flag & 0x1ffu) == 0 && !with_hist && !h->S.ext && !h->S.obs_list && rgk_step_obs_capable(&h->cfg) &&
+           rgk_obs_streams(&h->S, &h->cfg);
+}
 int rg_step_obs_gray(rg_t *h, const uint8_t *keys, int keys_on_device, uint32_t status_flag, int with_hist, float *out_dev) {
-    return rg_step_prefix(h, keys, h->S.n, keys_on_device) ? 1 : obs_common(h, status_flag, with_hist, 0, out_dev);
+    const bool fused = step_obs_fusable(h, status_flag, with_hist, out_dev);
+    h->S.fused_gray = fused ? out_dev : nullptr;
+    const int rc = rg_step_prefix(h, keys, h->S.n, keys_on_device);
+    h->S.fused_gray = nullptr;
+    return rc ? 1 : obs_common(h, status_flag, with_hist, 0, out_dev, fused);
 }
 
 int rg_step_prefix(rg_t *h, const uint8_t *keys, int n_keys, int keys_on_device) {
@@ -644,7 +665,7 @@
     return (symbol ? h->planes_sym : 1) + __builtin_popcount(status_flag & 0x1ffu) + (with_hist ? 1 : 0);
 }
 
-static int obs_common(rg_t *h, uint32_t status_flag, int with_hist, int kind, float *out_dev) {
+static int obs_common(rg_t *h, uint32_t status_flag, int with_hist, int kind, float *out_dev, bool redraw_only) {
     if (refuse_mixed(h, kind ? "rg_obs_symbol" : "rg_obs_gray")) return 1;
     HIPCHK(h, hipSetDevice(h->device));
     if (!h->sub.empty()) {
@@ -661,7 +682,7 @@
     {
         TimedLaunch t(h, 2, true);
         const bool bound = h->bound_out && out_dev == h->bound_out && kind == h->bound_kind && (status_flag & 0x1ffu) == 0 && !with_hist;
-        if (rgk_obs(&h->S, &h->cfg, status_flag & 0x1ffu, with_hist ? 1 : 0, kind, out_dev, h->d_err, h->planes_sym, bound && h->S.obs_list && h->bound_valid && h->bound_steps == 1, h->stream, t.start_ev(), t.stop_ev())) {
+        if (rgk_obs(&h->S, &h->cfg, status_flag & 0x1ffu, with_hist ? 1 : 0, kind, out_dev, h->d_err, h->planes_sym, bound && h->S.obs_list && h->bound_valid && h->bound_steps == 1, redraw_only ? 1 : 0, h->stream, t.start_ev(), t.stop_ev())) {
             HIPCHK(h, hipGetLastError());
             h->render_pending = false;
             h->bound_valid = bound;
@@ -700,13 +721,6 @@
     if (out_dev) HIPCHK(h, hipMemsetAsync(h->obs_cnt_mem, 0, 8, h->stream));
     h->S.obs_list = out_dev ? h->obs_list_mem : nullptr; h->S.obs_cnt = out_dev ? h->obs_cnt_mem : nullptr;
     h->S.bound_gray = (out_dev && kind == 0) ? out_dev : nullptr;
-    if (h->S.bound_gray && !h->gray_lut_mem) {
-        float lut[128];
-        for (uint32_t g = 0; g < 128; g++) lut[g] = (float)(uint8_t)host_tile_to_sym(g) / (float)(uint8_t)h->cfg.symbols;
-        if (!dev_alloc(h, &h->gray_lut_mem, 128)) return 1;
-        HIPCHK(h, hipMemcpy(h->gray_lut_mem, lut, sizeof lut, hipMemcpyHostToDevice));
-    }
-    h->S.gray_lut = h->gray_lut_mem;
     h->bound_out = out_dev; h->bound_kind = kind; h->bound_valid = false; h->bound_steps = 0;
     return 0;
 }
diff --git a/rogue-gym_amd/csrc/rg_kernels.hip b/rogue-gym_amd/csrc/rg_kernels.hip
--- a/rogue-gym_amd/csrc/rg_kernels.hip
+++ b/rogue-gym_amd/csrc/rg_kernels.hip
@@ -1,6 +1,7 @@
 
 
 #include "rg_device.h"
+#include "rg_obs_run.h"
 
 
 #include "rg_gen.h"
@@ -2208,7 +2209,35 @@
     if (taken && !(S.keep_spares && S.reseed[e] == 0)) __hip_atomic_store(&S.sp_ready[es], 0u, __ATOMIC_RELAXED, __HIP_MEMORY_SCOPE_AGENT);
 }
 
-template <int BW, int GM, bool BND = false>
+#ifndef STEP_OBS_RUN
+#define STEP_OBS_RUN OBS_RUN
+#endif
+__device__ __forceinline__ void obs_tail(const RgState &S, int et, bool enc) {
+    const uint64_t em = __ballot(enc);
+    if (!em) return;
+    asm volatile("s_waitcnt vmcnt(0)" ::: "memory");
+    int ln = threadIdx.x;
+    asm volatile("" : "+v"(ln));
+    const int e0 = __builtin_amdgcn_readfirstlane(et);
+    const int Q4 = S.hw >> 2;
+    const uint32_t *mir = reinterpret_cast<const uint32_t *>(S.screen) + (size_t)e0 * Q4;
+    float4 *img = reinterpret_cast<float4 *>(S.fused_gray) + (size_t)e0 * Q4;
+    const __attribute__((address_space(3))) float *lutg = (const __attribute__((address_space(3))) float *)(g_smem + STEP_LDS_LUT);
+    const int top = 64 - __builtin_clzll(em);
+    constexpr uint32_t RM = (1u << STEP_OBS_RUN) - 1u;
+    ObsRun<STEP_OBS_RUN> cur;
+    obs_run_load(mir, Q4, ln, (uint32_t)em & RM, cur);
+#pragma nounroll
+    for (int r = 0; r < top; r += STEP_OBS_RUN) {
+        ObsRun<STEP_OBS_RUN> nxt;
+        const uint32_t mn = r + STEP_OBS_RUN < 64 ? (uint32_t)(em >> (r + STEP_OBS_RUN)) & RM : 0u;
+        obs_run_load(mir + (size_t)(r + STEP_OBS_RUN) * Q4, Q4, ln, mn, nxt);
+        obs_run_store(img + (size_t)r * Q4, Q4, ln, (uint32_t)(em >> r) & RM, cur, lutg);
+        cur = nxt;
+    }
+}
+
+template <int BW, int GM, bool BND = false, bool OBS = false>
 __device__ __forceinline__ void step_wave(const RgState &S, const RgState *__restrict__ SPd, const RgConfig &c, const uint8_t *__restrict__ keys, int use_spares, int stage_off,
                                           const int e, const bool valid_in, const int stair_role) {
     uint16_t *lds_grid = reinterpret_cast<uint16_t *>(g_smem + stage_off);
@@ -2271,7 +2300,7 @@
     w.v = (lds_u16 *)(g_smem + STEP_LDS_WIN) + lane;
     lds_u32 *ovl_l = (lds_u32 *)(g_smem + STEP_LDS_OVL) + lane;
     ovl_l[0] = 0;
-    if (BND && S.bound_gray) {
+    if ((BND && S.bound_gray) || OBS) {
         typedef const __attribute__((address_space(1))) void *gptr;
         typedef __attribute__((address_space(3))) void *lptr;
         __builtin_amdgcn_global_load_lds((gptr)(S.gray_lut + lane), (lptr)(g_smem + STEP_LDS_LUT), 4, 0, 0);
@@ -2470,7 +2499,9 @@
             if (mine) atomicAdd(&S.stats[(size_t)blockIdx.x * RG_STAT_COLS + ln], (unsigned long long)mine);
         }
     }
+    uint32_t fin = old_flags;
     if (valid && err) {
+        if (OBS) fin = (old_flags & ~RG_FLAG_ERR_MASK) | err;
         S.flags[et] = (old_flags & ~RG_FLAG_ERR_MASK) | err;
         S.reward[et] = 0.f;
         S.done[et] = (old_flags & RG_FLAG_TERMINAL) ? 1 : 0;
@@ -2493,6 +2524,7 @@
         if (!taken) store_env(S, E);
         S.steps[et] = steps;
         S.flags[et] = flags;
+        if (OBS) fin = flags;
         S.done[et] = terminal ? 1 : 0;
         if (S.ovl && !taken && !inc_done && ((react & R_REDRAW) || descends || (terminal && c.auto_reset))) {
             for (int s0 = 0; s0 < nrooms_k; s0++) {
@@ -2545,12 +2577,16 @@
     take_spares(S, SPd, c, lane, et, taken, on_next);
     stair_publish(S, lane, et, valid, on_next);
     pf.mark(7);
+    if constexpr (OBS) {
+        obs_tail(S, et, valid && !(fin & RG_FLAG_REDRAW));
+        pf.mark(31);
+    }
     pf.finish();
 }
 
 #define STAIR_BLOCKS 256
 
-#define RG_STEP_BLOCK_BODY(BWV, GMV, BNDV) \
+#define RG_STEP_BLOCK_BODY(BWV, GMV, BNDV, OBSV) \
     __builtin_amdgcn_s_setprio(3); \
     const int lane = threadIdx.x; \
     if (blockIdx.x == 0 && lane == 0) { \
@@ -2567,7 +2603,7 @@
         bool v; int e; \
         if (stair) { e = list[i0]; v = lane == 0 && e < S.n_keys && keys[e] == '>'; } \
         else { v = lane < epw && i0 + lane < items; e = v ? i0 + lane : 0; } \
-        if (!stair || __any(v)) step_wave<BWV, GMV, BNDV>(S, SPd, c, keys, use_spares, stage_off, e, v, parity >= 0 ? (stair ? 1 : 2) : 0); \
+        if (!stair || __any(v)) step_wave<BWV, GMV, BNDV, OBSV>(S, SPd, c, keys, use_spares, stage_off, e, v, parity >= 0 ? (stair ? 1 : 2) : 0); \
         if (!stair || items <= STAIR_BLOCKS) break; \
         __syncthreads(); \
         uint32_t t = 0; \
@@ -2577,16 +2613,16 @@
 template <int BW, bool BND = false>
 __global__ void __launch_bounds__(WAVE) k_step(RgState S, const RgState *__restrict__ SPd, RgConfig c, const uint8_t *__restrict__ keys, int use_spares, int stage_off, int epw,
                                                int parity) {
-    RG_STEP_BLOCK_BODY(BW, (BW != 0 ? 1 : 0), BND)
-}
-template <bool BND>
+    RG_STEP_BLOCK_BODY(BW, (BW != 0 ? 1 : 0), BND, false)
+}
+template <bool BND, bool OBS = false>
 __global__ void __launch_bounds__(WAVE) __attribute__((amdgpu_waves_per_eu(2, 2)))
 k_step_w32(RgState S, const RgState *__restrict__ SPd, RgConfig c, const uint8_t *__restrict__ keys, int use_spares, int stage_off, int epw, int parity) {
-    RG_STEP_BLOCK_BODY(0, 0, BND)
+    RG_STEP_BLOCK_BODY(0, 0, BND, OBS)
 }
 __global__ void __launch_bounds__(WAVE) k_step_huge(RgState S, const RgState *__restrict__ SPd, RgConfig c, const uint8_t *__restrict__ keys, int use_spares, int stage_off,
                                                     int epw, int parity) {
-    RG_STEP_BLOCK_BODY(4, 2, false)
+    RG_STEP_BLOCK_BODY(4, 2, false, false)
 }
 #undef RG_STEP_BLOCK_BODY
 
@@ -2622,6 +2658,7 @@
     return (size_t)stage_off + stage;
 }
 size_t rgk_step_lds_per_cu(const RgConfig *c) { return step_lds(c, nullptr) * ((c->width <= 32 && gen_mode_of(c) == 0) ? 8 : 4); }
+int rgk_step_obs_capable(const RgConfig *c) { return (c->width <= 32 && gen_mode_of(c) == 0) ? 1 : 0; }
 int rgk_step_bound_capable(const RgConfig *c) {
     const int hw = c->width * c->height;
     if (gen_mode_of(c) == 2) return 0;
@@ -2647,7 +2684,7 @@
             if (hipFuncSetAttribute(reinterpret_cast<const void *>(k_step_huge), hipFuncAttributeMaxDynamicSharedMemorySize, (int)smem) == hipSuccess && dev >= 0 && dev < 64) raised[dev] = smem;
         }
         RG_LAUNCH_STEP(k_step_huge);
-    } else if (c->width <= 32 && gen_mode_of(c) == 0) { if (bnd) RG_LAUNCH_STEP(k_step_w32<true>); else RG_LAUNCH_STEP(k_step_w32<false>); }
+    } else if (c->width <= 32 && gen_mode_of(c) == 0) { if (bnd) RG_LAUNCH_STEP(k_step_w32<true>); else if (S->fused_gray) RG_LAUNCH_STEP((k_step_w32<false, true>)); else RG_LAUNCH_STEP(k_step_w32<false>); }
     else if (n32 && c->width <= 64) RG_LAUNCH_STEP(k_step<1>);
     else if (n32) { if (bnd) RG_LAUNCH_STEP((k_step<2, true>)); else RG_LAUNCH_STEP(k_step<2>); }
     else if (c->width <= 128) RG_LAUNCH_STEP(k_step<3>);
diff --git a/rogue-gym_amd/csrc/rg_obs.hip b/rogue-gym_amd/csrc/rg_obs.hip
--- a/rogue-gym_amd/csrc/rg_obs.hip
+++ b/rogue-gym_amd/csrc/rg_obs.hip
@@ -1,5 +1,6 @@
 #include <cstdlib>
 #include "rg_device.h"
+#include "rg_obs_run.h"
 
 #define RENDER_THREADS 256
 __device__ __forceinline__ bool in_same_room(const RgState &S, const RgConfig &c, int e, int ax, int ay, int bx, int by) {
@@ -145,15 +146,6 @@
 }
 
 #define OBS_THREADS 256
-__device__ __forceinline__ void store_obs(float4 *p, float4 v) {
-    typedef float f4v __attribute__((ext_vector_type(4)));
-    f4v nv = {v.x, v.y, v.z, v.w};
-#ifdef RG_EXP_OBS_PLAIN_STORES
-    *reinterpret_cast<f4v *>(p) = nv;
-#else
-    __builtin_nontemporal_store(nv, reinterpret_cast<f4v *>(p));
-#endif
-}
 struct ObsTabs { uint32_t w[RG_OBS_REC_WORDS(RG_OBS_MAX_ROOMS)]; };
 #define OBS_ENV_BYTES(hw) ((((size_t)(hw) + sizeof(ObsTabs)) + 15) & ~(size_t)15)
 
@@ -382,13 +374,14 @@
     }
 }
 
-#ifndef OBS_RUN
-#define OBS_RUN 4
+#ifndef OBS_RUN_REDRAW
+#define OBS_RUN_REDRAW 16
 #endif
 #ifndef OBS_STREAM_WAVES
 #define OBS_STREAM_WAVES 16384
 #endif
-__global__ void __launch_bounds__(WAVE) k_obs_stream(RgState S, RgConfig c, float *__restrict__ out, int hi_prio) {
+template <bool redraw_only>
+__device__ __forceinline__ void obs_stream_body(const RgState &S, const RgConfig &c, float *__restrict__ out, int hi_prio) {
     if (hi_prio) __builtin_amdgcn_s_setprio(3);
     __shared__ float lutf[128];
     __shared__ uint8_t mtile[RG_MAX_ENEMY_KINDS + 6];
@@ -399,15 +392,16 @@
     for (int g = lane; g < 128; g += WAVE) lutf[g] = (float)(uint8_t)tile_to_sym((uint32_t)g) / (float)(uint8_t)c.symbols;
     for (int g = lane; g < RG_MAX_ENEMY_KINDS + 6; g += WAVE) mtile[g] = c.mon[g].tile;
     lds_barrier();
-    auto gray4 = [&](uint32_t w) {
-        w &= 0x7f7f7f7fu;
-        float4 v; v.x = lutf[w & 0xff]; v.y = lutf[(w >> 8) & 0xff]; v.z = lutf[(w >> 16) & 0xff]; v.w = lutf[w >> 24];
-        return v;
-    };
+    auto gray4 = [&](uint32_t w) { return obs_gray4(lutf, w); };
+    constexpr int run = redraw_only ? OBS_RUN_REDRAW : OBS_RUN;
     struct Run { uint32_t fl, w0[OBS_RUN], w1[OBS_RUN]; };
     auto load_run = [&](int r, Run &R) {
-        const int base = r * OBS_RUN, cnt = n - base;
-        R.fl = lane < cnt && lane < OBS_RUN ? S.flags[base + lane] : 0u;
+        const int base = r * run, cnt = n - base;
+        R.fl = lane < cnt && lane < run ? S.flags[base + lane] : 0u;
+        if constexpr (redraw_only) {
+            for (int i = 0; i < OBS_RUN; i++) R.w0[i] = R.w1[i] = 0u;
+            return;
+        }
         const uint32_t *m = reinterpret_cast<const uint32_t *>(S.screen) + (size_t)base * Q4;
 #pragma unroll
         for (int i = 0; i < OBS_RUN; i++) {
@@ -415,11 +409,11 @@
             R.w1[i] = i < cnt && lane + WAVE < Q4 ? m[i * Q4 + lane + WAVE] : 0u;
         }
     };
-    const int nruns = (n + OBS_RUN - 1) / OBS_RUN;
+    const int nruns = (n + run - 1) / run;
     Run cur;
     load_run(blockIdx.x, cur);
     for (int r = blockIdx.x; r < nruns; r += gridDim.x) {
-        const int base = r * OBS_RUN, cnt = n - base < OBS_RUN ? n - base : OBS_RUN;
+        const int base = r * run, cnt = n - base < run ? n - base : run;
         Run nxt;
         load_run(r + gridDim.x, nxt);
         const uint32_t fl = cur.fl;
@@ -435,12 +429,14 @@
         uint4 tv = make_uint4(0, 0, 0, 0);
         uint32_t trec = 0;
         if (rmask) load_tiles(base + __builtin_ctzll(rmask), tv, trec);
-        float4 *o = reinterpret_cast<float4 *>(out) + (size_t)base * Q4;
-#pragma unroll
-        for (int i = 0; i < OBS_RUN; i++) {
-            if (i >= cnt || ((rmask >> i) & 1)) continue;
-            if (lane < Q4) store_obs(&o[i * Q4 + lane], gray4(cur.w0[i]));
-            if (lane + WAVE < Q4) store_obs(&o[i * Q4 + lane + WAVE], gray4(cur.w1[i]));
+        if constexpr (!redraw_only) {
+            float4 *o = reinterpret_cast<float4 *>(out) + (size_t)base * Q4;
+#pragma unroll
+            for (int i = 0; i < OBS_RUN; i++) {
+                if (i >= cnt || ((rmask >> i) & 1)) continue;
+                if (lane < Q4) store_obs(&o[i * Q4 + lane], gray4(cur.w0[i]));
+                if (lane + WAVE < Q4) store_obs(&o[i * Q4 + lane + WAVE], gray4(cur.w1[i]));
+            }
         }
         while (rmask) {
             const int i = __builtin_ctzll(rmask);
@@ -487,6 +483,8 @@
         cur = nxt;
     }
 }
+__global__ void __launch_bounds__(WAVE) k_obs_stream(RgState S, RgConfig c, float *__restrict__ out, int hi_prio) { obs_stream_body<false>(S, c, out, hi_prio); }
+__global__ void __launch_bounds__(WAVE) k_obs_redraws(RgState S, RgConfig c, float *__restrict__ out, int hi_prio) { obs_stream_body<true>(S, c, out, hi_prio); }
 
 #define RG_PUBLIC_FLAGS (RG_FLAG_TERMINAL | RG_FLAG_DEAD | RG_FLAG_MSG_MASK | RG_FLAG_ERR_MASK)
 __global__ void __launch_bounds__(256) k_pack(const uint8_t *__restrict__ screen, const uint8_t *__restrict__ hist, const int32_t *__restrict__ status,
@@ -903,7 +901,15 @@
     int blocks = S->n < 8192 ? S->n : 8192;
     hipLaunchKernelGGL(k_render, dim3(blocks), dim3(RENDER_THREADS), 0, st, *S, *c);
 }
-int rgk_obs(const RgState *S, const RgConfig *c, uint32_t sflag, int with_hist, int kind, float *out, uint32_t *err_any, int planes_sym, int bound, hipStream_t st, hipEvent_t ev0, hipEvent_t ev1) {
+int rgk_obs_streams(const RgState *S, const RgConfig *c) {
+    const int hw = c->width * c->height, nr = c->room_num_x * c->room_num_y;
+    if ((hw & 7) || nr > RG_OBS_MAX_ROOMS || !S->obs_rec || hw > 8 * WAVE || RG_OBS_REC_WORDS(nr) > WAVE || S->ext) return 0;
+#ifdef RG_DEV_KNOBS
+    if (const char *ev = getenv("RG_OBS_STREAM")) if (atoi(ev) == 0) return 0;
+#endif
+    return 1;
+}
+int rgk_obs(const RgState *S, const RgConfig *c, uint32_t sflag, int with_hist, int kind, float *out, uint32_t *err_any, int planes_sym, int bound, int redraw_only, hipStream_t st, hipEvent_t ev0, hipEvent_t ev1) {
     int hw = c->width * c->height;
     if (hw & 7) return 0;
     if (c->room_num_x * c->room_num_y > RG_OBS_MAX_ROOMS || !S->obs_rec) return 0;
@@ -927,13 +933,18 @@
 #ifdef RG_DEV_KNOBS
     if (const char *ev = getenv("RG_OBS_STREAM")) stream = stream && atoi(ev) != 0;
 #endif
+    if (redraw_only && !stream) return 0;
     if (stream) {
-        int sblocks = (S->n + OBS_RUN - 1) / OBS_RUN, cap = OBS_STREAM_WAVES;
+        const int srun = redraw_only ? OBS_RUN_REDRAW : OBS_RUN;
+        int sblocks = (S->n + srun - 1) / srun, cap = OBS_STREAM_WAVES;
 #ifdef RG_DEV_KNOBS
         if (const char *ev = getenv("RG_OBS_BLOCKS")) if (atoi(ev) > 0) cap = atoi(ev);
 #endif
         if (sblocks > cap) sblocks = cap;
-        if (ev0 || ev1) hipExtLaunchKernelGGL(k_obs_stream, dim3(sblocks), dim3(WAVE), 0, st, ev0, ev1, 0, *S, *c, out, hi_prio);
+        if (redraw_only) {
+            if (ev0 || ev1) hipExtLaunchKernelGGL(k_obs_redraws, dim3(sblocks), dim3(WAVE), 0, st, ev0, ev1, 0, *S, *c, out, hi_prio);
+            else hipLaunchKernelGGL(k_obs_redraws, dim3(sblocks), dim3(WAVE), 0, st, *S, *c, out, hi_prio);
+        } else if (ev0 || ev1) hipExtLaunchKernelGGL(k_obs_stream, dim3(sblocks), dim3(WAVE), 0, st, ev0, ev1, 0, *S, *c, out, hi_prio);
         else hipLaunchKernelGGL(k_obs_stream, dim3(sblocks), dim3(WAVE), 0, st, *S, *c, out, hi_prio);
         return 1;
     }
diff --git a/rogue-gym_amd/csrc/rg_obs_run.h b/rogue-gym_amd/csrc/rg_obs_run.h
--- /dev/null
+++ b/rogue-gym_amd/csrc/rg_obs_run.h
@@ -0,0 +1,41 @@
+#pragma once
+#include "rg_device.h"
+
+#ifndef OBS_RUN
+#define OBS_RUN 4
+#endif
+
+__device__ __forceinline__ void store_obs(float4 *p, float4 v) {
+    typedef float f4v __attribute__((ext_vector_type(4)));
+    f4v nv = {v.x, v.y, v.z, v.w};
+#ifdef RG_EXP_OBS_PLAIN_STORES
+    *reinterpret_cast<f4v *>(p) = nv;
+#else
+    __builtin_nontemporal_store(nv, reinterpret_cast<f4v *>(p));
+#endif
+}
+template <typename LUT>
+__device__ __forceinline__ float4 obs_gray4(LUT lutf, uint32_t w) {
+    w &= 0x7f7f7f7fu;
+    float4 v; v.x = lutf[w & 0xff]; v.y = lutf[(w >> 8) & 0xff]; v.z = lutf[(w >> 16) & 0xff]; v.w = lutf[w >> 24];
+    return v;
+}
+template <int R> struct ObsRun { uint32_t w0[R], w1[R]; };
+template <int R>
+__device__ __forceinline__ void obs_run_load(const uint32_t *__restrict__ m, int Q4, int lane, uint32_t mask, ObsRun<R> &run) {
+#pragma unroll
+    for (int i = 0; i < R; i++) {
+        const bool on = (mask >> i) & 1u;
+        run.w0[i] = on && lane < Q4 ? m[i * Q4 + lane] : 0u;
+        run.w1[i] = on && lane + WAVE < Q4 ? m[i * Q4 + lane + WAVE] : 0u;
+    }
+}
+template <int R, typename LUT>
+__device__ __forceinline__ void obs_run_store(float4 *__restrict__ o, int Q4, int lane, uint32_t mask, const ObsRun<R> &run, LUT lutf) {
+#pragma unroll
+    for (int i = 0; i < R; i++) {
+        if (!((mask >> i) & 1u)) continue;
+        if (lane < Q4) store_obs(&o[i * Q4 + lane], obs_gray4(lutf, run.w0[i]));
+        if (lane + WAVE < Q4) store_obs(&o[i * Q4 + lane + WAVE], obs_gray4(lutf, run.w1[i]));
+    }
+}
diff --git a/rogue-gym_amd/csrc/rg_state.h b/rogue-gym_amd/csrc/rg_state.h
--- a/rogue-gym_amd/csrc/rg_state.h
+++ b/rogue-gym_amd/csrc/rg_state.h
@@ -93,6 +93,7 @@
     uint16_t *ovl;
     float *bound_gray;
     const float *gray_lut;
+    float *fused_gray;
     int32_t *obs_list;
     uint32_t *obs_cnt;
     int32_t obs_par;
```
